# modelstreaming/ams

Measured on AMD Instinct MI355X. Metric: frames/sec student infer (DeeplabV3+MobileNetV2, 512x1024) + distill-steps/sec, higher is better.
Workload: dtype f32 (2xfp16 split products)

## Files before the change

### ams_amd/csrc/api.hip

```cpp
#include "engine.hpp"

using namespace ams;

extern "C" {

const char* ams_last_error(void) { return ams::last_error(); }
int ams_abi_version(void) { return AMS_ABI_VERSION; }

int ams_device_info(char* name_out, size_t name_cap, int32_t* n_cu, int64_t* hbm_bytes) {
    int dev = 0;
    AMS_CHECK_HIP(hipGetDevice(&dev));
    hipDeviceProp_t p;
    AMS_CHECK_HIP(hipGetDeviceProperties(&p, dev));
    if (name_out && name_cap) { snprintf(name_out, name_cap, "%s (%s)", p.name, p.gcnArchName); }
    if (n_cu) *n_cu = p.multiProcessorCount;
    if (hbm_bytes) *hbm_bytes = (int64_t)p.totalGlobalMem;
    return AMS_OK;
}

int ams_student_arena_bytes(const ams_student_config* cfg, const ams_layer_desc* layers, size_t* bytes_out) {
    AMS_REQUIRE(bytes_out, "arena_bytes: null output");
    ams_student tmp;
    int rc = student_build(&tmp, cfg, layers);
    if (rc) return rc;
// ... 263 lines not shown
                                   int32_t Ws, uint8_t* labels_out_dev, int64_t out_stride, void* stream) {
    return launch_teacher_labels_from_logits(logits_dev, slot_stride, n, lh, lw, num_classes, Hs, Ws, labels_out_dev, out_stride, (hipStream_t)stream);
}

size_t ams_render_table_bytes(void) { return AMS_RENDER_TABLE_BYTES; }

int ams_render_views(const uint8_t* frames_dev, const void* student_dev, int32_t student_dtype, const uint8_t* teacher_dev, int32_t batch, int32_t H,
                     int32_t W, int32_t K, const uint8_t* tables_dev, const ams_render_out* out, void* stream) {
    return launch_render_views(frames_dev, student_dev, student_dtype, teacher_dev, batch, H, W, K, tables_dev, out, (hipStream_t)stream);
}

int ams_student_train_step_dp(ams_student* s, const void* frames_dev, int32_t frames_dtype, const uint8_t* teacher_dev,
                              int32_t batch, int32_t global_batch, float lr, const uint8_t* mask_dev, double* loss_dev,
                              ams_allreduce_cb cb, void* user, void* stream) {
    return train_step_impl(s, frames_dev, frames_dtype, teacher_dev, batch, global_batch, lr, mask_dev, loss_dev, cb, user, nullptr, stream);
}

int ams_student_train_step_rccl(ams_student* s, const void* frames_dev, int32_t frames_dtype, const uint8_t* teacher_dev,
                                int32_t batch, int32_t global_batch, float lr, const uint8_t* mask_dev, double* loss_dev,
                                ams_comm* comm, void* stream) {
    AMS_REQUIRE(comm, "train_step_rccl: null communicator");
    return train_step_impl(s, frames_dev, frames_dtype, teacher_dev, batch, global_batch, lr, mask_dev, loss_dev, nullptr, nullptr, comm, stream);
}

int ams_student_train_step(ams_student* s, const void* frames_dev, int32_t frames_dtype, const uint8_t* teacher_dev, int32_t batch,
                           float lr, const uint8_t* mask_dev, double* loss_dev, void* stream) {
    return train_step_impl(s, frames_dev, frames_dtype, teacher_dev, batch, batch, lr, mask_dev, loss_dev, nullptr, nullptr, nullptr, stream);
}

int ams_student_f16_fallback_layers(const ams_student* s, int32_t* n_layers) {
    AMS_REQUIRE(s && n_layers, "f16_fallback_layers: null pointer");
    *n_layers = s->f16_fallback_layers;
    return AMS_OK;
}

int ams_student_feed_teacher_logits_layout(ams_student* s, const float* teacher_logits_dev, int32_t th, int32_t tw, int32_t layout) {
    AMS_REQUIRE(s, "feed_teacher_logits: null student");
    AMS_REQUIRE(layout == AMS_TLOGITS_FULL || layout == AMS_TLOGITS_SELECTED, "feed_teacher_logits: unknown teacher-logit layout %d", layout);
    if (!teacher_logits_dev) { s->teacher_logits = nullptr; s->teacher_th = s->teacher_tw = 0; s->teacher_layout = AMS_TLOGITS_FULL; return AMS_OK; }
    AMS_REQUIRE(th >= 1 && tw >= 1 && th <= s->cfg.height && tw <= s->cfg.width, "feed_teacher_logits: %d x %d teacher logits for %d x %d labels", th, tw,
                s->cfg.height, s->cfg.width);
    s->teacher_logits = teacher_logits_dev; s->teacher_th = th; s->teacher_tw = tw; s->teacher_layout = layout;
    return AMS_OK;
}

int ams_student_feed_teacher_logits(ams_student* s, const float* teacher_logits_dev, int32_t th, int32_t tw) {
    return ams_student_feed_teacher_logits_layout(s, teacher_logits_dev, th, tw, AMS_TLOGITS_FULL);
}

int ams_student_set_regularizer(ams_student* s, const uint8_t* reg_mask_dev, int32_t n_vars, float coef) {
    AMS_REQUIRE(s, "set_regularizer: null student");
    if (!reg_mask_dev) { s->reg_mask = nullptr; s->reg_nvars = 0; s->reg_coef = 0.f; return AMS_OK; }
    AMS_REQUIRE(s->cfg.trainable, "set_regularizer: this student was created frozen");
    AMS_REQUIRE(n_vars > 0 && coef >= 0.f, "set_regularizer: n_vars=%d coef=%g", n_vars, (double)coef);
    s->reg_mask = reg_mask_dev; s->reg_nvars = n_vars; s->reg_coef = coef;
    return AMS_OK;
}

int ams_student_set_option(ams_student* s, int32_t option, int32_t value) {
    AMS_REQUIRE(s, "set_option: null student");
    s->dual_choice.clear();
    if (option == AMS_OPT_MATMUL) {
        AMS_REQUIRE(value == AMS_MATMUL_F32 || value == AMS_MATMUL_SPLIT_BF16 || value == AMS_MATMUL_SPLIT_BF16_X6 || value == AMS_MATMUL_BF16 ||
                        value == AMS_MATMUL_SPLIT_F16,
                    "set_option: unknown matmul mode %d", value);
        s->matmul_mode = value;
        return AMS_OK;
    }
    if (option == AMS_OPT_DUAL_AUTOTUNE) {
        s->dual_autotune = value != 0;
        return AMS_OK;
    }
    if (option == AMS_OPT_DUAL_PARTS) {
        AMS_REQUIRE(value >= 2 && value <= 4, "set_option: AMS_OPT_DUAL_PARTS must be 2 .. 4");
        s->dual_parts = value;
        return AMS_OK;
    }
    if (option == AMS_OPT_FUSE_FIRST_BLOCK) {
        s->fuse_first_block = value < 0 ? 0 : (value > 2 ? 2 : value);
        return AMS_OK;
    }
    if (option == AMS_OPT_FUSE_DW_PROJECT) {
        s->fuse_dw_project = value != 0;
        return AMS_OK;
    }
    if (option == AMS_OPT_FUSE_EXPAND_DW_STREAM) {
        s->fuse_expand_dw_stream = value < 0 ? 0 : (value > 2 ? 2 : value);
        return AMS_OK;
    }
    if (option == AMS_OPT_BLOCK_X6) {
        s->block_x6 = value != 0;
        return AMS_OK;
    }
    if (option == AMS_OPT_LATE_SUBBATCH) {
        s->late_subbatch = value < 0 ? 0 : value;
        return AMS_OK;
    }
    if (option == AMS_OPT_DUAL_STREAM) {
        s->dual_stream = value < 0 ? 0 : value;
        s->dual_choice.clear();
        return AMS_OK;
    }
    if (option == AMS_OPT_FUSE_BLOCK) {
        s->fuse_block = value != 0;
        return AMS_OK;
    }
    if (option == AMS_OPT_FUSE_EXPAND_DW) {
        s->fuse_expand_dw = value < 0 ? 0 : (value > 2 ? 2 : value);
        return AMS_OK;
    }
    if (option == AMS_OPT_EMULATE_BF16_STORAGE) {
        s->emulate_bf16_storage = value != 0;
        return AMS_OK;
    }
    if (option == AMS_OPT_FUSE_DGRAD_BN) {
        s->fuse_dgrad_bn = value < 0 ? 0 : (value > 3 ? 3 : value);
        return AMS_OK;
    }
    if (option == AMS_OPT_FUSE_GEMM_RED) {
        s->fuse_gemm_red = value & 3;
        return AMS_OK;
    }
    if (option == AMS_OPT_TRAIN_RECOMPUTE) {
        s->train_recompute = value < 0 ? 0 : (value > 2 ? 2 : value);
        return AMS_OK;
    }
    if (option == AMS_OPT_FUSE_OPERAND_BN) {
        s->fuse_operand_bn = value & 1;
        return AMS_OK;
    }
    if (option == AMS_OPT_WGRAD_FORK_EVERY) {
        AMS_REQUIRE(value >= 1 && value <= 64, "set_option: AMS_OPT_WGRAD_FORK_EVERY must be in 1 .. 64");
        s->wgrad_fork_every = value;
        return AMS_OK;
    }
    if (option == AMS_OPT_TRAIN_FWD_F16) {
        s->train_fwd_f16 = value != 0;
        return AMS_OK;
    }
    if (option == AMS_OPT_SOFT_TEACHER) {
        s->soft_teacher = value != 0;
        return AMS_OK;
    }
    if (option == AMS_OPT_NAN_GRADS) {
        s->nan_grads = value != 0;
        return AMS_OK;
    }
    if (option == AMS_OPT_OVERLAP_WGRAD) {
        s->overlap_wgrad = value < 0 ? 0 : (value > 3 ? 3 : value);
        return AMS_OK;
    }
    if (option == AMS_OPT_OVERLAP_HEAD) {
        s->overlap_head = value != 0;
        return AMS_OK;
    }
    if (option == AMS_OPT_STREAM_MIN_ROWS) {
        AMS_REQUIRE(value >= 0, "set_option: AMS_OPT_STREAM_MIN_ROWS must be >= 0");
        s->stream_min_rows = value;
        return AMS_OK;
    }
    set_error("set_option: unknown option %d", option);
    return AMS_E_INVALID;
}

int ams_student_profile(ams_student* s, int32_t enable) {
    AMS_REQUIRE(s, "profile: null student");
    AMS_CHECK_HIP(hipDeviceSynchronize());
    s->prof.clear();
    s->prof.on = enable != 0;
    return AMS_OK;
}

int ams_student_profile_read(ams_student* s, char* buf, size_t cap, size_t* needed) {
    AMS_REQUIRE(s && needed, "profile_read: null pointer");
    AMS_CHECK_HIP(hipDeviceSynchronize());
    std::string out;
    char line[256];
    for (auto& r : s->prof.recs) {
        float ms = 0.f;
        AMS_CHECK_HIP(hipEventElapsedTime(&ms, r.e0, r.e1));
        snprintf(line, sizeof(line), "%s\t%d\t%.6f\t%.0f\t%.0f\t%.0f\n", r.name.c_str(), r.layer, ms, r.bytes, r.flops, r.flops_x6);
        out += line;
    }
    *needed = out.size() + 1;
    if (buf && cap >= out.size() + 1) memcpy(buf, out.c_str(), out.size() + 1);
    return AMS_OK;
}

int ams_student_get_adam_step(const ams_student* s, int64_t* t) {
    AMS_REQUIRE(s && t, "get_adam_step: null pointer");
    *t = s->adam_t;
    return AMS_OK;
}
int ams_student_set_adam_step(ams_student* s, int64_t t) {
    AMS_REQUIRE(s && t >= 0, "set_adam_step: bad argument");
    s->adam_t = t;
    return AMS_OK;
}

size_t ams_pack_masked_fp16_scratch(int64_t n) { return n > 0 ? pack_fp16_scratch(n) : 0; }

int ams_pack_masked_fp16(const float* params_dev, const uint8_t* mask_dev, int64_t n, uint16_t* out_half_dev, int64_t* n_out_dev,
                         int64_t* scratch_dev, size_t scratch_elems, void* stream) {
    AMS_REQUIRE(params_dev && out_half_dev && n_out_dev && n > 0, "pack_masked_fp16: bad argument");
    AMS_REQUIRE(scratch_dev && scratch_elems >= pack_fp16_scratch(n), "pack_masked_fp16: scratch too small (need %zu int64)",
                pack_fp16_scratch(n));
    return launch_pack_fp16(params_dev, mask_dev, n, out_half_dev, n_out_dev, scratch_dev, (hipStream_t)stream);
}

static int64_t delta_mask_bytes(const ams_student* s, const ams_delta_var* vars, int32_t n_vars, const char* what = "apply_delta") {
    if (!vars || n_vars < 1 || n_vars > AMS_DELTA_MAX_VARS) { set_error("%s: %d variables (1 .. %d)", what, n_vars, AMS_DELTA_MAX_VARS); return -1; }
    int64_t mask = 0;
    for (int32_t i = 0; i < n_vars; ++i) {
        const ams_delta_var& d = vars[i];
        const int64_t n_region = d.region == AMS_REGION_PARAMS ? (int64_t)s->cfg.n_trainable : d.region == AMS_REGION_STATS ? (int64_t)s->cfg.n_stats : -1;
        if (n_region < 0) { set_error("%s: variable %d: region %d is neither params nor stats", what, i, d.region); return -1; }
        if (d.offset < 0 || d.count < 0 || d.offset > n_region - d.count) {
            set_error("%s: variable %d: elements [%lld, +%lld) outside its region of %lld", what, i, (long long)d.offset, (long long)d.count,
                      (long long)n_region);
            return -1;
        }
        if (d.mask_offset != mask) {
            set_error("%s: variable %d: mask at byte %lld, the masks before it end at %lld", what, i, (long long)d.mask_offset, (long long)mask);
            return -1;
        }
        mask += (d.count + 7) / 8;
    }
    return mask;
}

size_t ams_student_apply_delta_scratch(const ams_delta_var* vars_host, int32_t n_vars) {
    if (!vars_host || n_vars < 1 || n_vars > AMS_DELTA_MAX_VARS) return 0;
    int64_t mask = 0;
    for (int32_t i = 0; i < n_vars; ++i) mask += vars_host[i].count > 0 ? (vars_host[i].count + 7) / 8 : 0;
    return (size_t)(4 * (int64_t)n_vars + delta_segments(mask));
}

int ams_student_apply_delta(ams_student* s, const uint8_t* payload_dev, int64_t payload_bytes, const ams_delta_var* vars_host,
                            int32_t n_vars, int64_t* n_applied_dev, int32_t* status_dev, int64_t* scratch_dev, size_t scratch_elems,
                            void* stream) {
    AMS_REQUIRE(s && n_applied_dev && status_dev && scratch_dev, "apply_delta: null pointer");
    AMS_REQUIRE(payload_bytes >= 0 && (payload_dev || payload_bytes == 0), "apply_delta: %lld payload bytes at %p", (long long)payload_bytes,
                (const void*)payload_dev);
    static_assert(sizeof(ams_delta_var) == 4 * sizeof(int64_t), "ams_delta_var: four int64 words");
    const int64_t mask_bytes = delta_mask_bytes(s, vars_host, n_vars);
    if (mask_bytes < 0) return AMS_E_INVALID;
    const size_t need = 4 * (size_t)n_vars + (size_t)delta_segments(mask_bytes);
    AMS_REQUIRE(scratch_elems >= need, "apply_delta: scratch too small (need %zu int64)", need);
    hipStream_t st = (hipStream_t)stream;
    if (s->ev_delta) AMS_CHECK_HIP(hipEventSynchronize(s->ev_delta));
    else RUN(create_sync_event(&s->ev_delta));
    s->delta_vars.assign(vars_host, vars_host + n_vars);
    ams_delta_var* vars_dev = reinterpret_cast<ams_delta_var*>(scratch_dev);
    AMS_CHECK_HIP(hipMemcpyAsync(vars_dev, s->delta_vars.data(), n_vars * sizeof(ams_delta_var), hipMemcpyHostToDevice, st));
    AMS_CHECK_HIP(hipEventRecord(s->ev_delta, st));
    return launch_apply_delta(payload_dev, payload_bytes, vars_dev, n_vars, mask_bytes, s->params, (int64_t)s->cfg.n_trainable, s->stats,
                              (int64_t)s->cfg.n_stats, scratch_dev + 4 * n_vars, n_applied_dev, status_dev, st);
}

size_t ams_select_changed_scratch(int64_t n) { return n > 0 ? select_scratch() : 0; }

int ams_select_changed(const float* after_dev, const float* before_dev, int64_t n, int64_t k, ams_select_result* result_dev,
                       int64_t* scratch_dev, size_t scratch_elems, void* stream) {
    AMS_REQUIRE(after_dev && before_dev && result_dev && scratch_dev, "select_changed: null pointer");
    AMS_REQUIRE(n > 0 && n < ((int64_t)1 << 31) && k >= 0 && k < n, "select_changed: rank %lld of %lld elements (0 <= k < n < 2^31)", (long long)k,
                (long long)n);
    AMS_REQUIRE(((uintptr_t)result_dev & 7) == 0 && ((uintptr_t)after_dev & 3) == 0 && ((uintptr_t)before_dev & 3) == 0, "select_changed: misaligned pointer");
    AMS_REQUIRE(scratch_elems >= select_scratch(), "select_changed: scratch too small (need %zu int64)", select_scratch());
    return launch_select_changed(after_dev, before_dev, n, k, result_dev, scratch_dev, (hipStream_t)stream);
}

int ams_select_apply(float* params_dev, const float* before_dev, int64_t n, float cut, uint8_t* mask_dev, int64_t* n_kept_dev, void* stream) {
    AMS_REQUIRE(params_dev && before_dev && mask_dev && n_kept_dev && n > 0, "select_apply: bad argument");
    AMS_REQUIRE(((uintptr_t)n_kept_dev & 7) == 0 && ((uintptr_t)params_dev & 3) == 0 && ((uintptr_t)before_dev & 3) == 0, "select_apply: misaligned pointer");
    return launch_select_apply(params_dev, before_dev, n, cut, mask_dev, n_kept_dev, (hipStream_t)stream);
}

size_t ams_student_encode_delta_scratch(const ams_delta_var* vars_host, int32_t n_vars) {
    if (!vars_host || n_vars < 1 || n_vars > AMS_DELTA_MAX_VARS) return 0;
    int64_t mask = 0;
    for (int32_t i = 0; i < n_vars; ++i) mask += vars_host[i].count > 0 ? (vars_host[i].count + 7) / 8 : 0;
    return (size_t)(5 * (int64_t)n_vars + 2 + encode_segments(mask));
}

int ams_student_encode_delta(ams_student* s, const uint8_t* mask_dev, const ams_delta_var* vars_host, int32_t n_vars, uint8_t* payload_dev,
                             int64_t payload_cap, int64_t* payload_bytes_dev, int64_t* scratch_dev, size_t scratch_elems, void* stream) {
    AMS_REQUIRE(s && payload_dev && payload_bytes_dev && scratch_dev, "encode_delta: null pointer");
    const int64_t mask_bytes = delta_mask_bytes(s, vars_host, n_vars, "encode_delta");
    if (mask_bytes < 0) return AMS_E_INVALID;
    AMS_REQUIRE(payload_cap >= mask_bytes, "encode_delta: room for %lld bytes, the mask section alone has %lld", (long long)payload_cap,
                (long long)mask_bytes);
    const size_t table = 5 * (size_t)n_vars + 1;
    const size_t need = table + 1 + (size_t)encode_segments(mask_bytes);
    AMS_REQUIRE(scratch_elems >= need, "encode_delta: scratch too small (need %zu int64)", need);
    hipStream_t st = (hipStream_t)stream;
    if (s->ev_encode) AMS_CHECK_HIP(hipEventSynchronize(s->ev_encode));
    else RUN(create_sync_event(&s->ev_encode));
    s->encode_table.resize(table);
    memcpy(s->encode_table.data(), vars_host, n_vars * sizeof(ams_delta_var));
    int64_t first = 0;
    for (int32_t i = 0; i < n_vars; ++i) { s->encode_table[4 * (size_t)n_vars + i] = first; first += vars_host[i].count; }
    s->encode_table[table - 1] = first;
    AMS_CHECK_HIP(hipMemcpyAsync(scratch_dev, s->encode_table.data(), table * sizeof(int64_t), hipMemcpyHostToDevice, st));
    AMS_CHECK_HIP(hipEventRecord(s->ev_encode, st));
    return launch_encode_delta(mask_dev, scratch_dev, n_vars, mask_bytes, s->params, s->stats, scratch_dev + table, payload_dev, payload_cap,
                               payload_bytes_dev, st);
// ... 484 lines not shown
```

### ams_amd/csrc/engine.hpp

```cpp
#pragma once
#include <math.h>
#include <stdarg.h>

#include <string>
#include <map>
#include <vector>

#include "kernels.hpp"

namespace ams {

const char* last_error();

struct ProfRec { std::string name; int layer; double bytes, flops, flops_x6; hipEvent_t e0, e1; };
struct Profiler {
    bool on = false;
    std::vector<ProfRec> recs;
    std::vector<hipEvent_t> pool;
    hipEvent_t get() {
        if (!pool.empty()) { hipEvent_t e = pool.back(); pool.pop_back(); return e; }
        hipEvent_t e = nullptr;
        (void)hipEventCreate(&e);
        return e;
    }
    void clear() {
        for (auto& r : recs) { pool.push_back(r.e0); pool.push_back(r.e1); }
        recs.clear();
    }
    ~Profiler() {
        clear();
        for (auto e : pool) if (e) (void)hipEventDestroy(e);
    }
};

struct LayerRt {
    ams_layer_desc d;
    int Hin = 0, Win = 0, Hout = 0, Wout = 0;
    int64_t px_in = 0, px_out = 0;
    float *fscale = nullptr, *fshift = nullptr;
    float *scale = nullptr, *shift = nullptr, *mean = nullptr, *rstd = nullptr, *cA = nullptr, *cB = nullptr, *cC = nullptr;
    double *fsums = nullptr, *bsums = nullptr;
    float *z = nullptr, *a = nullptr, *da = nullptr;
    float* dzp = nullptr;
    float* dw_rows = nullptr; size_t dw_rows_floats = 0;
    uint16_t *whi = nullptr, *wlo = nullptr, *wlo3 = nullptr;
    uint16_t* whf_mem = nullptr;
    uint16_t* whf = nullptr;
    int Kp = 0, split_k0 = 0;
    float* blk_vecs = nullptr;
    double* xx64 = nullptr;
    float* xx_g0 = nullptr;
};

struct Carver {
    char* base;
    size_t off = 0;
    explicit Carver(void* b) : base((char*)b) {}
    template <typename T>
    T* take(size_t n) {
        off = (off + 255) & ~(size_t)255;
        T* p = base ? (T*)(base + off) : nullptr;
        off += n * sizeof(T);
        return p;
    }
};

}

struct ams_student {
    ams_student_config cfg;
    std::vector<ams::LayerRt> L;
    char* arena = nullptr;
    size_t arena_bytes = 0;
    int h = 0, w = 0;
    int n_backbone = 0;
    int iPool = 0, iAspp = 0, iProj = 0, iLogits = 0;
    float *params = nullptr, *stats = nullptr, *grads = nullptr, *adam_m = nullptr, *adam_v = nullptr;
    float *fparams = nullptr, *fstats = nullptr;
    double* bn_sync = nullptr; size_t bn_sync_doubles = 0;
    float* logits = nullptr;
    uint16_t* xsplit = nullptr; size_t xsplit_plane = 0;
    uint16_t* panel_scratch = nullptr; size_t panel_elems = 0;
    std::vector<ams::SplitJob> tp_jobs;
    std::map<std::pair<const float*, int>, int> tp_index;
    ams::SplitJob* tp_jobs_dev = nullptr;
    uint16_t* tp_panels = nullptr; size_t tp_elems = 0;
    int64_t tp_blocks = 0;
    bool tp_fresh = false;
    bool tp_wait = false;
    hipEvent_t ev_tp = nullptr;
    std::vector<ams_delta_var> delta_vars;
    hipEvent_t ev_delta = nullptr;
    std::vector<int64_t> encode_table;
    hipEvent_t ev_encode = nullptr;
    float* dlogits = nullptr;
    float* ce_scratch = nullptr;
    int emulate_bf16_storage = 0;
    int fuse_gemm_red = 3;
    int fuse_operand_bn = 1;
    int fuse_dgrad_bn = 3;
    int train_recompute = 2;
    double* xx_scratch = nullptr; size_t xx_scratch_doubles = 0;
    float* xt_scratch = nullptr; size_t xt_floats = 0;
    float *vec_ones = nullptr, *vec_zeros = nullptr;
    float* vec_inv_hw = nullptr;
    float* act[4] = {nullptr, nullptr, nullptr, nullptr};
    size_t act_elems = 0;
    float *pooled = nullptr, *pool_a = nullptr, *img_bias = nullptr;
    float *d_img_bias = nullptr, *d_pool_a = nullptr, *d_pool_z = nullptr, *d_pooled = nullptr;
    float* im2col = nullptr;
    float* scratch2 = nullptr;
    float* scratch3 = nullptr;
    hipStream_t side2 = nullptr;
    hipEvent_t ev_xt = nullptr;
    hipStream_t side = nullptr;
    hipEvent_t ev_fork = nullptr, ev_head = nullptr;
    int dual_stream = 1;
    int dual_parts = 2;
    int dual_autotune = 0;
    hipStream_t part_stream[3] = {nullptr, nullptr, nullptr};
    hipEvent_t part_done[3] = {nullptr, nullptr, nullptr};
    hipEvent_t ev_fork_dual = nullptr;
    std::map<int, int> dual_choice;
    int overlap_head = 0;
    int overlap_wgrad = 1;
    int wgrad_fork_every = 1;
    int train_fwd_f16 = 0;
    int f16_fallback_layers = 0;
    int soft_teacher = 0;
    const float* teacher_logits = nullptr; int teacher_th = 0, teacher_tw = 0, teacher_layout = AMS_TLOGITS_FULL;
    const uint8_t* reg_mask = nullptr; int reg_nvars = 0; float reg_coef = 0.f;
    int nan_grads = 0;
    ~ams_student() {
        if (ev_fork) (void)hipEventDestroy(ev_fork);
        if (ev_head) (void)hipEventDestroy(ev_head);
        for (auto& e : part_done) if (e) (void)hipEventDestroy(e);
        for (auto& t : part_stream) if (t) (void)hipStreamDestroy(t);
        if (ev_fork_dual) (void)hipEventDestroy(ev_fork_dual);
        if (side) (void)hipStreamDestroy(side);
        if (side2) (void)hipStreamDestroy(side2);
        if (ev_xt) (void)hipEventDestroy(ev_xt);
        if (ev_tp) (void)hipEventDestroy(ev_tp);
        if (ev_delta) (void)hipEventDestroy(ev_delta);
        if (ev_encode) (void)hipEventDestroy(ev_encode);
    }
    float* scratch = nullptr; size_t scratch_floats = 0;
    float* tmp_c = nullptr;
    double* loss_buf = nullptr;
    int64_t* conf_buf = nullptr;
    int64_t adam_t = 0;
    bool frozen_ready = false;
    int matmul_mode = AMS_MATMUL_SPLIT_F16;
    int fuse_dw_project = 0;
    int fuse_first_block = 1;
    int64_t stream_min_rows = 4096;
    int fuse_expand_dw_stream = 1;
    int block_x6 = 1;
    int late_subbatch = 0;
    int fuse_block = 1;
    int fuse_expand_dw = 1;
    ams::Profiler prof;
    hipEvent_t prof_e0 = nullptr;
    double prof_flops = 0.0;
    double prof_flops_x6 = 0.0;
};

namespace ams {

int student_build(ams_student* s, const ams_student_config* cfg, const ams_layer_desc* layers);
int student_layout(ams_student* s, void* arena, size_t* bytes_out);
void prof_begin(ams_student* s, hipStream_t st);
void prof_end(ams_student* s, hipStream_t st, int layer, double bytes);

static inline PwArgs pw_args(const float* x, int64_t M, int K, int ldx, const float* w, int N, float* y, int ldy) {
    PwArgs a;
    memset(&a, 0, sizeof(a));
    a.x = x; a.M = M; a.K = K; a.Kw = K; a.ldx = ldx; a.w = w; a.w_sk = N; a.w_sn = 1; a.N = N;
    a.rows_per_img = 1; a.act = AMS_ACT_NONE; a.y = y; a.ldy = ldy;
    return a;
}

#define RUN(expr) do { int _rc = (expr); if (_rc) return _rc; } while (0)

#define RUNK(LAYER, BYTES, expr)                                   \
    do {                                                           \
        prof_begin(s, st);                                         \
        int _rc = (expr);                                          \
        prof_end(s, st, (LAYER), (double)(BYTES));                 \
        if (_rc) return _rc;                                       \
    } while (0)

static inline double pw_bytes(const PwArgs& a) {
    return 4.0 * ((double)a.M * (a.K + a.N + (a.res ? a.N : 0)) + (double)a.Kw * a.N) + (a.ysplit ? 2.0 * a.ysplit_np * (double)a.M * a.N : 0.0);
}
static inline double dw_bytes(const LayerRt& l, int B) { return 4.0 * ((double)B * (l.px_in + l.px_out) * l.d.cin + 9.0 * l.d.cin); }

struct SyncCtx { ams_allreduce_cb cb; void* user; ams_student* s; ams_comm* comm; };

static inline int comm_as_cb(void*, size_t, size_t, int32_t) { return 0; }

static inline int sync_any(const SyncCtx* sc, void* p, size_t n, int dtype, hipStream_t st) {
    if (!sc || !sc->cb) return AMS_OK;
    if (sc->comm) return comm_allreduce(sc->comm, p, n, dtype, st);
    const int rc = sc->cb(sc->user, (size_t)((char*)p - sc->s->arena), n, dtype);
    if (rc) { set_error("all-reduce callback failed (%d)", rc); return AMS_E_STATE; }
    return AMS_OK;
}
static inline int sync_doubles(const SyncCtx* sc, double* p, size_t n, hipStream_t st) { return sync_any(sc, p, n, AMS_DT_F64, st); }

bool split_pays(const PwArgs& a);
int live_pointwise(ams_student* s, const PwArgs& a, hipStream_t st);
bool train_recompute_block(const ams_student* s, int i);
bool dw_fused_train(const ams_student* s, int i, int B);
bool stem_fused_train(const ams_student* s);
bool dw_fused_train_fwd(const ams_student* s, int i, int B);
bool operand_bn_act(const ams_student* s, int i);
size_t red_rows_bound(int64_t M);
int check_call(const ams_student* s, const void* frames, int dtype, int batch);
int run_forward(ams_student* s, const void* frames, int dtype, int batch, int mode, hipStream_t st);
int forward_live(ams_student* s, const void* frames, int dtype, int B, int global_B, bool update_ema, const SyncCtx* sc, hipStream_t st);

int loss_forward(ams_student* s, const uint8_t* teacher, int B, int32_t* labels, hipStream_t st);
int backward(ams_student* s, const void* frames, int dtype, const uint8_t* teacher, int B, int global_B, const SyncCtx* sc, hipStream_t st);
int train_step_impl(ams_student* s, const void* frames_dev, int32_t frames_dtype, const uint8_t* teacher_dev, int32_t batch, int32_t global_batch,
                    float lr, const uint8_t* mask_dev, double* loss_dev, ams_allreduce_cb cb, void* user, ams_comm* comm, void* stream);

}
```

### ams_amd/csrc/engine_forward.hip

```cpp
#include "engine.hpp"

namespace ams {

bool split_pays(const PwArgs& a) {
    if (a.K < 32 || a.K % 8 != 0 || a.M < 256) return false;
    return a.M < 32768 || !pointwise_stream_applies(a) || (int64_t)a.K * a.N >= 40 * (int64_t)(a.K + a.N);
}

int live_pointwise(ams_student* s, const PwArgs& a, hipStream_t st) {
    const bool split = s->matmul_mode != AMS_MATMUL_F32 && s->panel_scratch && split_pays(a) && a.Kw == a.K && a.ldx % 4 == 0;
    if (!split) return launch_pointwise(a, st);
    const int Kp = (a.K + 31) / 32 * 32;
    const size_t plane = (size_t)a.N * Kp;
    if (s->tp_fresh) {
        auto it = s->tp_index.find({a.w, a.w_sk == 1 ? 1 : 0});
        if (it != s->tp_index.end()) {
            const SplitJob& j = s->tp_jobs[it->second];
            if (j.K == a.K && j.N == a.N && j.sk == a.w_sk && j.sn == a.w_sn) {
                if (s->tp_wait) { AMS_CHECK_HIP(hipStreamWaitEvent(st, s->ev_tp, 0)); s->tp_wait = false; }
                if (s->matmul_mode == AMS_MATMUL_SPLIT_F16 && s->train_fwd_f16 && j.f16 && pointwise_f16_applies(a))
                    return launch_pointwise_split_f16(a, j.p0 + 3 * j.plane, j.plane, j.Kp, st);
                return launch_pointwise_split3(a, j.p0, j.p0 + j.plane, j.p0 + 2 * j.plane, j.Kp, st);
            }
        }
    }
    AMS_REQUIRE(3 * plane <= s->panel_elems, "live_pointwise: panel scratch too small");
    uint16_t* p0 = s->panel_scratch;
    int rc = launch_split_weights3(a.w, a.w_sk, a.w_sn, a.K, a.N, Kp, p0, p0 + plane, p0 + 2 * plane, st);
    if (rc) return rc;
    return launch_pointwise_split3(a, p0, p0 + plane, p0 + 2 * plane, Kp, st);
}

struct FrozenView {
    float* act[4];
    uint16_t* xsplit; size_t xsplit_plane;
    float *pooled, *pool_a, *img_bias, *logits, *scratch;
    const void* frames; int B;
    int reserved;
};
static FrozenView view_whole(const ams_student* s, const void* frames, int B) {
    return {{s->act[0], s->act[1], s->act[2], s->act[3]}, s->xsplit, s->xsplit_plane, s->pooled, s->pool_a, s->img_bias, s->logits, s->scratch, frames, B, -1};
}
static FrozenView view_late(const ams_student* s, FrozenView v, int b0, int bp, int input_i) {
    v.pooled += (size_t)b0 * s->L[s->iPool].d.cin;
    v.pool_a += (size_t)b0 * s->L[s->iPool].d.cout;
    v.img_bias += (size_t)b0 * s->L[s->iProj].d.cout;
    v.logits += (size_t)b0 * s->h * s->w * 32;
    v.B = bp; v.reserved = input_i;
    return v;
}
static FrozenView view_slice(const ams_student* s, const void* frames, int dtype, int b0, int bp) {
    const ams_student_config& c = s->cfg;
    FrozenView v = view_late(s, view_whole(s, (const char*)frames + (size_t)b0 * c.height * c.width * 3 * (dtype == AMS_DT_U8 ? 1 : 4), bp), b0, bp, -1);
    for (int k = 0; k < 4; ++k) v.act[k] += (size_t)b0 * (s->act_elems / c.max_batch);
    if (v.xsplit) { v.xsplit += 3 * (s->xsplit_plane / c.max_batch) * b0; v.xsplit_plane = (s->xsplit_plane / c.max_batch) * bp; }
    v.scratch += image_colsum_scratch(b0, s->L[s->iPool].d.cin);
    return v;
}

struct PartsFmt { int np = 0, fmt = 0; };
struct Cursor { int i; const float* cur; int cur_i; PartsFmt parts; };

static int other(const FrozenView& v, int avoid0, int avoid1) {
    for (int k = 0; k < 4; ++k) if (k != avoid0 && k != avoid1 && k != v.reserved) return k;
    return -1;
}

enum PwForm { PW_F32, PW_BF16_1, PW_BF16_2, PW_BF16_3, PW_F16 };
enum BlockForm { BLOCK_WHOLE,
                 BLOCK_TILED,
                 BLOCK_STREAM, BLOCK_WREG,
                 BLOCK_LAYERS };
struct BlockPlan {
    BlockForm form = BLOCK_LAYERS;
    bool expand = false;
    bool h16 = false, x6 = false;
    int np = 0; const uint16_t* wparts = nullptr; int64_t wplane = 0;
    PartsFmt in;
    PwForm expand_form = PW_F32;
    bool dw_project = false;
    bool d_h2i = false;
    PwForm project_form = PW_F32;
    PartsFmt out;
};

static PwArgs layer_args(const ams_student* s, int layer, int B, const float* x, float* y, const float* res) {
    const LayerRt& l = s->L[layer];
    PwArgs a = pw_args(x, (int64_t)B * l.px_in, l.d.cin, l.d.cin, s->fparams + l.d.w_off, l.d.cout, y, l.d.cout);
    a.scale = l.fscale; a.shift = l.fshift; a.act = l.d.act;
    if (l.d.role == AMS_ROLE_PROJECT && l.d.residual_from) { a.res = res; a.ldr = l.d.cout; }
    return a;
}

static PwForm pointwise_form(const ams_student* s, int layer, const PwArgs& a, bool streamable) {
    const LayerRt& l = s->L[layer];
    if (s->matmul_mode == AMS_MATMUL_F32 || !l.whi || !(split_pays(a) || (streamable && a.K % 8 == 0 && a.K >= 32))) return PW_F32;
    switch (s->matmul_mode) {
        case AMS_MATMUL_SPLIT_F16: return l.whf && pointwise_f16_applies(a) ? PW_F16 : PW_BF16_3;
        case AMS_MATMUL_SPLIT_BF16_X6: return PW_BF16_3;
        case AMS_MATMUL_BF16: return PW_BF16_1;
        default: return PW_BF16_2;
    }
}

static bool stream_ok(const ams_student* s, int B, int k) {
    if (!(s->fuse_expand_dw_stream && k + 1 <= s->n_backbone && s->L[k].d.role == AMS_ROLE_EXPAND && s->L[k + 1].d.role == AMS_ROLE_DEPTHWISE &&
          (int64_t)B * s->L[k].px_in >= s->stream_min_rows && (int64_t)s->L[k + 1].px_out * s->L[k + 1].d.cout * 4 < 0x7fffffffLL &&
          expand_dw_stream_supported(s->L[k].d.cin, s->L[k].d.cout, s->L[k + 1].d.stride, s->L[k + 1].d.rate)))
        return false;
    if (s->L[k + 1].d.stride != 1 && s->fuse_expand_dw_stream < 2) return false;
    if (s->L[k].d.cin <= 32) return true;
    return s->matmul_mode != AMS_MATMUL_F32 && s->L[k].whi && s->L[k].Kp == s->L[k].d.cin;
}
static int stream_np(const ams_student* s, int k) {
    if (s->matmul_mode == AMS_MATMUL_SPLIT_F16 && s->L[k].whf && s->L[k].d.cin > 32) return AMS_NP_F16;
    return s->matmul_mode == AMS_MATMUL_SPLIT_BF16_X6 || s->matmul_mode == AMS_MATMUL_SPLIT_F16 ? 3 : s->matmul_mode == AMS_MATMUL_BF16 ? 1 : 2;
}
static PartsFmt stream_parts(const ams_student* s, int k) {
    PartsFmt f;
    const int np = stream_np(s, k);
    if (np == AMS_NP_F16) { f.np = 2; f.fmt = 1; }
    else if (s->matmul_mode != AMS_MATMUL_SPLIT_F16) f.np = np;
    return f;
}

static BlockPlan plan_block(const ams_student* s, const FrozenView& v, int i, PartsFmt in) {
    BlockPlan p;
    const int B = v.B, nb = s->n_backbone;
    const auto role = [&](int k) { return k <= nb ? s->L[k].d.role : -1; };
    p.expand = role(i) == AMS_ROLE_EXPAND;
    const int id = i + (p.expand ? 1 : 0), ij = id + 1;
    const LayerRt& le = s->L[i];
    const LayerRt& ld = s->L[id];
    const LayerRt& lj = s->L[ij];
    if (s->fuse_block && p.expand && role(id) == AMS_ROLE_DEPTHWISE && role(ij) == AMS_ROLE_PROJECT &&
        (!lj.d.residual_from || lj.d.residual_from == i - 1) &&
        block_fused_supported(le.d.cin, le.d.cout, lj.d.cout, ld.d.stride, ld.d.rate, lj.d.residual_from != 0)) {
        p.form = BLOCK_WHOLE;
        p.h16 = s->block_x6 && s->matmul_mode == AMS_MATMUL_SPLIT_F16 && le.whf && lj.whf && le.Kp == 32;
        p.x6 = !p.h16 && s->block_x6 && s->matmul_mode != AMS_MATMUL_F32 && le.whi && le.Kp == 32 && le.d.cin > 16;
        return p;
    }
    if (stream_ok(s, B, i) && (le.d.cin <= 96 || in.np || s->fuse_expand_dw_stream >= 2)) {
        p.form = le.d.cin > 96 && in.np ? BLOCK_WREG : BLOCK_STREAM;
        p.in = in;
        p.np = stream_np(s, i);
        p.h16 = p.np == AMS_NP_F16;
        p.wparts = p.h16 ? le.whf : le.whi;
        p.wplane = p.h16 ? (int64_t)le.d.cout * le.Kp : (int64_t)(le.wlo - le.whi);
    } else if (s->fuse_expand_dw && p.expand && role(id) == AMS_ROLE_DEPTHWISE &&
               expand_dw_supported(le.d.cin, le.d.cout, ld.d.stride, ld.d.rate) &&
               (s->fuse_expand_dw >= 2 || le.d.cin <= 24 || ld.d.stride == 2)) {
        p.form = BLOCK_TILED;
    } else {
        if (p.expand) {
            const bool streamable = role(id) == AMS_ROLE_DEPTHWISE && le.Kp == le.d.cin && le.d.cin >= 64 &&
                                    expand_dw_stream_supported(le.d.cin, le.d.cout, ld.d.stride, ld.d.rate);
            p.expand_form = pointwise_form(s, i, layer_args(s, i, B, nullptr, nullptr, nullptr), streamable);
        }
        if (s->fuse_dw_project && s->matmul_mode == AMS_MATMUL_SPLIT_BF16 &&    role(id) == AMS_ROLE_DEPTHWISE &&
            role(ij) == AMS_ROLE_PROJECT && lj.whi && (int64_t)B * ld.px_out < 32768 && (int64_t)B * ld.px_out >= 256 &&
            lj.Kp == ld.d.cin && dw_project_supported(ld.d.cin, lj.d.cout, ld.d.stride, ld.d.rate)) {
            p.dw_project = true;
            return p;
        }
    }
    if (role(ij) != AMS_ROLE_PROJECT) return p;
    const PwArgs a = layer_args(s, ij, B, nullptr, nullptr, s->fparams);
    p.project_form = pointwise_form(s, ij, a, false);
    p.d_h2i = (p.form == BLOCK_STREAM || p.form == BLOCK_WREG) && p.h16 && p.project_form == PW_F16 && ld.d.cout % 8 == 0 && !s->emulate_bf16_storage;
    if (stream_ok(s, B, ij + 1) && v.xsplit && (size_t)a.M * a.N <= v.xsplit_plane && p.project_form != PW_F32 && pointwise_split_writes_parts(a) &&
        !(s->emulate_bf16_storage && lj.px_out == (int64_t)s->h * s->w))
        p.out = stream_parts(s, ij + 1);
    return p;
}

static int frozen_pointwise(ams_student* s, int layer, const PwArgs& a, PwForm form, hipStream_t st) {
    const LayerRt& l = s->L[layer];
    if (a.x_fmt != 0 && form != PW_F16) { set_error("frozen_pointwise: layer %d was handed fp16 pairs but does not run the fp16 product", layer); return AMS_E_STATE; }
    switch (form) {
        case PW_F16: RUNK(layer, pw_bytes(a), launch_pointwise_split_f16(a, l.whf, (int64_t)l.d.cout * l.Kp, l.Kp, st)); break;
        case PW_BF16_3: RUNK(layer, pw_bytes(a), launch_pointwise_split3(a, l.whi, l.wlo, l.wlo3, l.Kp, st)); break;
        case PW_BF16_2: RUNK(layer, pw_bytes(a), launch_pointwise_split(a, l.whi, l.wlo, l.Kp, st)); break;
        case PW_BF16_1: RUNK(layer, pw_bytes(a), launch_pointwise_split1(a, l.whi, l.Kp, st)); break;
        case PW_F32: RUNK(layer, pw_bytes(a), launch_pointwise(a, st)); break;
    }
    return AMS_OK;
}

static int run_first_block(ams_student* s, const FrozenView& v, int dtype, Cursor& c, hipStream_t st) {
    const ams_student_config& cf = s->cfg;
    const float* P = s->fparams;
    const int B = v.B;
    float* y = v.act[0];
    const LayerRt& l = s->L[1];
    const LayerRt& ld = s->L[2];
    const LayerRt& lj = s->L[3];
    const double in_bytes = (double)B * cf.height * cf.width * 3 * (dtype == AMS_DT_U8 ? 1 : 4);
    c.i = 2;
    if (s->fuse_first_block && s->n_backbone >= 3 && l.d.cout == 32 && ld.d.role == AMS_ROLE_DEPTHWISE && ld.d.cin == 32 &&
        ld.d.stride == 1 && ld.d.rate == 1 && lj.d.role == AMS_ROLE_PROJECT && lj.d.cin == 32 && lj.d.cout == 16 &&
        !lj.d.residual_from) {
        const double bytes = in_bytes + 4.0 * B * lj.px_out * lj.d.cout + 4.0 * (27 * 32 + 9 * 32 + 32 * 16);
        if (s->fuse_first_block >= 2)
            RUNK(3, bytes, launch_first_block_tiles(v.frames, dtype, B, cf.height, cf.width, cf.pixel_scale, P + l.d.w_off, l.fscale, l.fshift,
                                                    l.d.act, P + ld.d.w_off, ld.fscale, ld.fshift, ld.d.act, P + lj.d.w_off, lj.fscale,
                                                    lj.fshift, lj.d.act, y, st, l.blk_vecs));
        else {
            const bool h16 = s->block_x6 && s->matmul_mode == AMS_MATMUL_SPLIT_F16 && l.whf && lj.whf && lj.Kp == 32;
            const bool x6 = !h16 && s->block_x6 && s->matmul_mode != AMS_MATMUL_F32 && l.whi;
            RUNK(3, bytes, launch_first_block(v.frames, dtype, B, cf.height, cf.width, cf.pixel_scale, P + l.d.w_off, l.fscale, l.fshift,
                                              l.d.act, P + ld.d.w_off, ld.fscale, ld.fshift, ld.d.act, P + lj.d.w_off, lj.fscale,
                                              lj.fshift, lj.d.act, y, st, x6 ? l.whi : nullptr, 32 * 32, h16 ? l.whf : nullptr, 32 * 32,
                                              h16 ? lj.whf : nullptr, (int64_t)lj.d.cout * lj.Kp));
        }
        c.i = 4;
    } else {
        const double bytes = in_bytes + 4.0 * B * l.px_out * l.d.cout;
        RUNK(1, bytes, launch_stem(v.frames, dtype, B, cf.height, cf.width, P + l.d.w_off, l.d.cout, l.fscale, l.fshift, l.d.act,
                                   cf.pixel_scale, y, st));
    }
    c.cur = y; c.cur_i = 0; c.parts = PartsFmt();
    return AMS_OK;
}

static int run_project(ams_student* s, const FrozenView& v, Cursor& c, const BlockPlan& p, int ij, const float* d, int d_i, hipStream_t st) {
    const LayerRt& l = s->L[ij];
    AMS_REQUIRE(l.d.role == AMS_ROLE_PROJECT, "engine: expected project at layer %d", ij);
    const int o = other(v, c.cur_i, d_i);
    PwArgs a = layer_args(s, ij, v.B, d, v.act[o], c.cur);
    a.x_fmt = p.d_h2i ? 1 : 0;
    if (p.out.np) { a.ysplit = v.xsplit; a.ysplit_plane = a.M * a.N; a.ysplit_np = p.out.np; a.ysplit_fmt = p.out.fmt; }
    RUN(frozen_pointwise(s, ij, a, p.project_form, st));
    if (s->emulate_bf16_storage && l.px_out == (int64_t)s->h * s->w)
        RUN(launch_round_bf16(v.act[o], (int64_t)v.B * l.px_out * l.d.cout, st));
    c.cur = v.act[o]; c.cur_i = o; c.i = ij + 1; c.parts = p.out;
    return AMS_OK;
}

static int run_block_whole(ams_student* s, const FrozenView& v, Cursor& c, const BlockPlan& p, hipStream_t st) {
    const float* P = s->fparams;
    const int B = v.B, i = c.i;
    const LayerRt& le = s->L[i];
    const LayerRt& ld = s->L[i + 1];
    const LayerRt& lj = s->L[i + 2];
    const int o = other(v, c.cur_i, -1);
    const bool res = lj.d.residual_from != 0;
    const double bytes = 4.0 * ((double)B * (le.px_in * le.d.cin * (res ? 2 : 1) + lj.px_out * lj.d.cout) + (double)le.d.cin * le.d.cout +
                                9.0 * ld.d.cin + (double)lj.d.cin * lj.d.cout);
    const double fl_e = 2.0 * B * (double)le.px_in * le.d.cin * le.d.cout, fl_p = 2.0 * B * (double)lj.px_out * lj.d.cin * lj.d.cout;
    s->prof_flops = 2.0 * B * (double)ld.px_out * 9.0 * ld.d.cin + (p.h16 ? 0.0 : fl_p) + (p.x6 || p.h16 ? 0.0 : fl_e);
    s->prof_flops_x6 = p.h16 ? fl_e + fl_p : p.x6 ? fl_e : 0.0;
    RUNK(i + 2, bytes, launch_block_fused(c.cur, B, le.Hin, le.Win, le.d.cin, P + le.d.w_off, le.fscale, le.fshift, le.d.act, le.d.cout,
                                          P + ld.d.w_off, ld.d.stride, ld.fscale, ld.fshift, ld.d.act, P + lj.d.w_off, lj.fscale, lj.fshift,
                                          lj.d.act, lj.d.cout, res, v.act[o], st, le.blk_vecs, p.x6 ? le.whi : nullptr,
                                          (int64_t)(le.wlo - le.whi), p.h16 ? le.whf : nullptr, (int64_t)le.d.cout * le.Kp, p.h16 ? lj.whf : nullptr,
                                          (int64_t)lj.d.cout * lj.Kp, lj.Kp));
    c.cur = v.act[o]; c.cur_i = o; c.i = i + 3; c.parts = PartsFmt();
    return AMS_OK;
}

static int run_block_expand_dw(ams_student* s, const FrozenView& v, Cursor& c, const BlockPlan& p, hipStream_t st) {
    const float* P = s->fparams;
    const int B = v.B, i = c.i;
    const LayerRt& le = s->L[i];
    const LayerRt& ld = s->L[i + 1];
    const int o = other(v, c.cur_i, -1);
    const double bytes = 4.0 * ((double)B * (le.px_in * le.d.cin + ld.px_out * ld.d.cout) + (double)le.d.cin * le.d.cout + 9.0 * ld.d.cin);
    const uint16_t* x_parts = p.in.np ? v.xsplit : nullptr;
    const int64_t xplane = (int64_t)B * le.px_in * le.d.cin;
    if (p.form == BLOCK_TILED)
        RUNK(i + 1, bytes, launch_expand_dw(c.cur, B, le.Hin, le.Win, le.d.cin, P + le.d.w_off, le.fscale, le.fshift, le.d.act, le.d.cout,
                                            P + ld.d.w_off, ld.d.stride, ld.d.rate, ld.fscale, ld.fshift, ld.d.act, v.act[o], st));
    else if (p.form == BLOCK_WREG)
        RUNK(i + 1, bytes, launch_expand_dw_wreg(x_parts, xplane, B, le.Hin, le.Win, le.d.cin, p.wparts, p.wplane, p.np, le.fscale,
                                                 le.fshift, le.d.act, le.d.cout, P + ld.d.w_off, ld.d.rate, ld.fscale, ld.fshift, ld.d.act,
                                                 v.act[o], st, p.d_h2i ? 1 : 0));
    else
        RUNK(i + 1, bytes, launch_expand_dw_stream(c.cur, x_parts, xplane, B, le.Hin, le.Win, le.d.cin, P + le.d.w_off, p.wparts, p.wplane, p.np, le.fscale,
                                                   le.fshift, le.d.act, le.d.cout, P + ld.d.w_off, ld.d.stride, ld.d.rate, ld.fscale, ld.fshift, ld.d.act,
                                                   v.act[o], st, p.d_h2i ? 1 : 0));
    if (p.form != BLOCK_TILED && s->emulate_bf16_storage && ld.px_out == (int64_t)s->h * s->w)
        RUN(launch_round_bf16(v.act[o], (int64_t)B * ld.px_out * ld.d.cout, st));
    return run_project(s, v, c, p, i + 2, v.act[o], o, st);
}

static int run_block_layers(ams_student* s, const FrozenView& v, Cursor& c, const BlockPlan& p, hipStream_t st) {
    const float* P = s->fparams;
    const int B = v.B;
    int i = c.i;
    const float* x = c.cur;
    int x_i = c.cur_i;
    if (p.expand) {
        const int o = other(v, c.cur_i, -1);
        RUN(frozen_pointwise(s, i, layer_args(s, i, B, x, v.act[o], nullptr), p.expand_form, st));
        x = v.act[o]; x_i = o; ++i;
    }
    const LayerRt& l = s->L[i];
    AMS_REQUIRE(l.d.role == AMS_ROLE_DEPTHWISE, "engine: expected depthwise at layer %d", i);
    const int o = other(v, c.cur_i, x_i);
    if (p.dw_project) {
        const LayerRt& lpj = s->L[i + 1];
        const PwArgs a = layer_args(s, i + 1, B, nullptr, v.act[o], c.cur);
        const double bytes = 4.0 * ((double)B * (l.px_in * l.d.cin + lpj.px_out * lpj.d.cout * (a.res ? 2 : 1)) +
                                    (double)lpj.d.cin * lpj.d.cout + 9.0 * l.d.cin);
        RUNK(i + 1, bytes, launch_dw_project(x, B, l.Hin, l.Win, l.d.cin, P + l.d.w_off, l.d.rate, l.fscale, l.fshift, l.d.act, a,
                                             lpj.whi, lpj.wlo, lpj.Kp, st));
        c.cur = v.act[o]; c.cur_i = o; c.i = i + 2; c.parts = PartsFmt();
        return AMS_OK;
    }
    RUNK(i, dw_bytes(l, B), launch_depthwise(x, B, l.Hin, l.Win, l.d.cin, P + l.d.w_off, l.d.stride, l.d.rate, l.fscale,
                                             l.fshift, l.d.act, v.act[o], st));
    if (s->emulate_bf16_storage && l.px_out == (int64_t)s->h * s->w)
        RUN(launch_round_bf16(v.act[o], (int64_t)B * l.px_out * l.d.cout, st));
    return run_project(s, v, c, p, i + 1, v.act[o], o, st);
}

static int run_blocks(ams_student* s, const FrozenView& v, Cursor& c, int i_stop, hipStream_t st) {
    while (c.i <= s->n_backbone && c.i < i_stop) {
        const BlockPlan p = plan_block(s, v, c.i, c.parts);
        switch (p.form) {
            case BLOCK_WHOLE: RUN(run_block_whole(s, v, c, p, st)); break;
            case BLOCK_TILED: case BLOCK_STREAM: case BLOCK_WREG: RUN(run_block_expand_dw(s, v, c, p, st)); break;
            case BLOCK_LAYERS: RUN(run_block_layers(s, v, c, p, st)); break;
        }
    }
    return AMS_OK;
}

static int run_head(ams_student* s, const FrozenView& v, const Cursor& c, hipStream_t st) {
    const float* P = s->fparams;
    const LayerRt& lp = s->L[s->iPool]; const LayerRt& la = s->L[s->iAspp]; const LayerRt& lc = s->L[s->iProj]; const LayerRt& ll = s->L[s->iLogits];
    const int B = v.B;
    const int64_t HW = (int64_t)s->h * s->w, M = (int64_t)B * HW;
    const bool fork = s->overlap_head && !s->prof.on;
    hipStream_t ps = st;
    if (fork) {
        if (!s->side) RUN(create_side_stream(&s->side));
        if (!s->ev_fork) RUN(create_sync_event(&s->ev_fork));
        if (!s->ev_head) RUN(create_sync_event(&s->ev_head));
        AMS_CHECK_HIP(hipEventRecord(s->ev_fork, st));
        AMS_CHECK_HIP(hipStreamWaitEvent(s->side, s->ev_fork, 0));
        ps = s->side;
    }
    RUNK(s->iPool, 4.0 * M * lp.d.cin, launch_global_mean(c.cur, B, HW, lp.d.cin, v.pooled, v.scratch, ps));
    {
        PwArgs a = pw_args(v.pooled, B, lp.d.cin, lp.d.cin, P + lp.d.w_off, lp.d.cout, v.pool_a, lp.d.cout);
        a.scale = lp.fscale; a.shift = lp.fshift; a.act = lp.d.act;
        RUNK(s->iPool, pw_bytes(a), launch_pointwise(a, ps));
        PwArgs b = pw_args(v.pool_a, B, lp.d.cout, lp.d.cout, P + lc.d.w_off, lc.d.cout, v.img_bias, lc.d.cout);
        RUNK(s->iProj, pw_bytes(b), launch_pointwise(b, ps));
    }
    if (fork) AMS_CHECK_HIP(hipEventRecord(s->ev_head, s->side));
    const int o1 = other(v, c.cur_i, -1), o2 = other(v, c.cur_i, o1);
    PwArgs a = pw_args(c.cur, M, la.d.cin, la.d.cin, P + la.d.w_off, la.d.cout, v.act[o1], la.d.cout);
    a.scale = la.fscale; a.shift = la.fshift; a.act = la.d.act;
    RUN(frozen_pointwise(s, s->iAspp, a, pointwise_form(s, s->iAspp, a, false), st));
    if (fork) AMS_CHECK_HIP(hipStreamWaitEvent(st, s->ev_head, 0));
    PwArgs b = pw_args(v.act[o1], M, la.d.cout, la.d.cout, P + lc.d.w_off + (int64_t)lp.d.cout * lc.d.cout, lc.d.cout,
                       v.act[o2], lc.d.cout);
    b.img_bias = v.img_bias; b.rows_per_img = HW; b.scale = lc.fscale; b.shift = lc.fshift; b.act = lc.d.act;
    RUN(frozen_pointwise(s, s->iProj, b, pointwise_form(s, s->iProj, b, false), st));
    PwArgs d = pw_args(v.act[o2], M, lc.d.cout, lc.d.cout, P + ll.d.w_off, ll.d.cout, v.logits, 32);
    d.shift = P + ll.d.gamma_off;
    RUN(frozen_pointwise(s, s->iLogits, d, pointwise_form(s, s->iLogits, d, false), st));
    return AMS_OK;
}

static int forward_frozen(ams_student* s, const FrozenView& v, int dtype, hipStream_t st) {
    Cursor c;
    RUN(run_first_block(s, v, dtype, c, st));
    int i_late = s->n_backbone + 1;
    for (int k = 2; k <= s->n_backbone; ++k)
        if (s->L[k].d.role == AMS_ROLE_EXPAND && s->L[k].px_in == (int64_t)s->h * s->w) { i_late = k; break; }
    if (!(s->late_subbatch > 0 && v.B > s->late_subbatch && i_late <= s->n_backbone)) {
        RUN(run_blocks(s, v, c, s->n_backbone + 1, st));
        return run_head(s, v, c, st);
    }
    RUN(run_blocks(s, v, c, i_late, st));
    const int64_t late_in_frame = s->L[i_late].px_in * s->L[i_late].d.cin;
    for (int b0 = 0; b0 < v.B; b0 += s->late_subbatch) {
        const int bp = v.B - b0 < s->late_subbatch ? v.B - b0 : s->late_subbatch;
        const FrozenView lv = view_late(s, v, b0, bp, c.cur_i);
        Cursor lc = {i_late, c.cur + (int64_t)b0 * late_in_frame, c.cur_i, PartsFmt()};
        RUN(run_blocks(s, lv, lc, s->n_backbone + 1, st));
        RUN(run_head(s, lv, lc, st));
    }
    return AMS_OK;
}

bool train_recompute_block(const ams_student* s, int i) {
    if (!s->train_recompute || !s->xt_scratch || i < 2 || i + 1 > s->n_backbone) return false;
    const LayerRt& l = s->L[i];
    const LayerRt& ld = s->L[i + 1];
    return l.xx_g0 && l.d.role == AMS_ROLE_EXPAND && ld.d.role == AMS_ROLE_DEPTHWISE && xdw_train_supported(l.d.cin, l.d.cout, ld.d.stride, ld.d.rate) &&
           expand_dw_supported(l.d.cin, l.d.cout, ld.d.stride, ld.d.rate) && l.d.cout <= 1024 &&
           xdw_train_scratch(s->cfg.max_batch, l.Hin, l.Win, l.d.cin, l.d.cout) != (size_t)-1 &&
           xdw_train_scratch(s->cfg.max_batch, l.Hin, l.Win, l.d.cin, l.d.cout) <= s->xt_floats;
}

bool dw_fused_train(const ams_student* s, int i, int B) {
    if (i < 3 || i > s->n_backbone || !s->fuse_dgrad_bn || train_recompute_block(s, i - 1)) return false;
    const LayerRt& l = s->L[i];
    const LayerRt& prev = s->L[i - 1];
    return l.d.role == AMS_ROLE_DEPTHWISE && l.d.stride == 1 && prev.d.role == AMS_ROLE_EXPAND && prev.d.cout == l.d.cin && l.d.cin <= 1024 &&
           depthwise_dgrad_bn_scratch(B, l.Hin, l.Win, l.d.cin) <= s->scratch_floats;
}
bool stem_fused_train(const ams_student* s) {
    const ams_student_config& c = s->cfg;
    return s->n_backbone >= 2 && s->train_recompute && s->L[1].d.role == AMS_ROLE_STEM && s->L[1].d.cout == 32 && s->L[2].d.role == AMS_ROLE_DEPTHWISE &&
           s->L[2].d.stride == 1 && s->L[2].d.rate == 1 && s->xt_scratch && xdw_stem_scratch(c.max_batch, c.height, c.width) != (size_t)-1 &&
           xdw_stem_scratch(c.max_batch, c.height, c.width) <= s->xt_floats;
}
bool dw_fused_train_fwd(const ams_student* s, int i, int B) {
    if (s->fuse_dgrad_bn < 2 || i < 2 || i > s->n_backbone) return false;
    if (!(i == 2 ? stem_fused_train(s) : dw_fused_train(s, i, B))) return false;
    return depthwise_fwd_bn_scratch(B, s->L[i].Hin, s->L[i].Win, s->L[i].d.cin, s->L[i].d.rate) <= s->scratch_floats;
}

bool operand_bn_act(const ams_student* s, int i) {
    if (!(s->fuse_operand_bn & 1) || i < 2 || i + 1 > s->n_backbone) return false;
    const LayerRt& l = s->L[i];
    const LayerRt& lj = s->L[i + 1];
    return l.d.role == AMS_ROLE_DEPTHWISE && lj.d.role == AMS_ROLE_PROJECT && lj.d.cin == l.d.cout && l.d.cout % 4 == 0 && l.d.cout <= 1024;
}

size_t red_rows_bound(int64_t M) {
    const size_t tiled = (size_t)(M / 64 + 8), streaming = M >= 32768 ? 8 * 512 : 0;
    return tiled > streaming ? tiled : streaming;
}

struct BnEma { const float* center; float omd; float *mm, *mv; };
static BnEma bn_ema(const ams_student* s, const LayerRt& l, bool update_ema) {
    return {s->stats + l.d.mean_off, 1.0f - s->cfg.bn_decay, update_ema ? s->stats + l.d.mean_off : nullptr, update_ema ? s->stats + l.d.var_off : nullptr};
}
static int bn_from_partials(ams_student* s, LayerRt& l, const BnEma& e, const float* part, int rows, int64_t stride, double n_global,
                            const SyncCtx* sc, hipStream_t st) {
    const float *gamma = s->params + l.d.gamma_off, *beta = s->params + l.d.beta_off;
    if (!sc || !sc->cb)
        return launch_bn_fwd_finalize_partials(part, rows, stride, l.d.cout, l.fsums, n_global, e.center, gamma, beta, l.d.bn_eps, e.omd, e.mm, e.mv,
                                               l.scale, l.shift, l.mean, l.rstd, st);
    RUN(launch_partials_to_sums(part, rows, stride, l.d.cout, l.fsums, st));
    RUN(sync_doubles(sc, l.fsums, 2 * (size_t)l.d.cout, st));
    return launch_bn_finalize(l.fsums, n_global, l.d.cout, e.center, gamma, beta, l.d.bn_eps, e.omd, e.mm, e.mv, l.scale, l.shift, l.mean, l.rstd, st);
}

static int bn_train(ams_student* s, LayerRt& l, int64_t M_local, double n_global, bool update_ema, const SyncCtx* sc,
                    const float* res, hipStream_t st, int pre_rows = 0, bool act_pass = true) {
    const BnEma e = bn_ema(s, l, update_ema);
    if (pre_rows > 0) {
        RUN(bn_from_partials(s, l, e, s->scratch, pre_rows, 2 * (int64_t)l.d.cout, n_global, sc, st));
    } else if (!sc || !sc->cb) {
        RUNK(0, 4.0 * M_local * l.d.cout,
             launch_colstats_bn(l.z, M_local, l.d.cout, e.center, l.fsums, s->scratch, n_global, s->params + l.d.gamma_off,
                                s->params + l.d.beta_off, l.d.bn_eps, e.omd, e.mm, e.mv, l.scale, l.shift, l.mean, l.rstd, st));
    } else {
        RUNK(0, 4.0 * M_local * l.d.cout, launch_colstats(l.z, M_local, l.d.cout, e.center, l.fsums, s->scratch, st));
        RUN(sync_doubles(sc, l.fsums, 2 * (size_t)l.d.cout, st));
        RUN(launch_bn_finalize(l.fsums, n_global, l.d.cout, e.center, s->params + l.d.gamma_off, s->params + l.d.beta_off, l.d.bn_eps, e.omd,
                               e.mm, e.mv, l.scale, l.shift, l.mean, l.rstd, st));
    }
    if (!act_pass) return AMS_OK;
    RUNK(0, 4.0 * M_local * l.d.cout * (res ? 3 : 2), launch_bn_act(l.z, M_local, l.d.cout, l.scale, l.shift, l.d.act, res, l.a, st));
    return AMS_OK;
}

int forward_live(ams_student* s, const void* frames, int dtype, int B, int global_B, bool update_ema, const SyncCtx* sc,
                        hipStream_t st) {
    const ams_student_config& c = s->cfg;
    AMS_REQUIRE(c.trainable, "live forward needs a trainable student (activations are not allocated)");
    const float* P = s->params;
    s->tp_fresh = false;
    s->tp_wait = false;
    if (s->matmul_mode != AMS_MATMUL_F32 && !s->tp_jobs.empty()) {
        hipStream_t ts = st;
        if (s->overlap_wgrad && !s->prof.on && s->scratch2) {
            if (!s->side) RUN(create_side_stream(&s->side));
            if (!s->ev_fork) RUN(create_sync_event(&s->ev_fork));
            if (!s->ev_tp) RUN(create_sync_event(&s->ev_tp));
            AMS_CHECK_HIP(hipEventRecord(s->ev_fork, st));
            AMS_CHECK_HIP(hipStreamWaitEvent(s->side, s->ev_fork, 0));
            ts = s->side;
        }
        RUNK(0, 0.0, launch_split_batch(s->tp_jobs_dev, (int)s->tp_jobs.size(), s->tp_blocks, ts,
                                        s->train_fwd_f16 && s->matmul_mode == AMS_MATMUL_SPLIT_F16));
        if (ts != st) { AMS_CHECK_HIP(hipEventRecord(s->ev_tp, ts)); s->tp_wait = true; }
        s->tp_fresh = true;
    }
    {
        LayerRt& l = s->L[1];
        RUN(launch_stem(frames, dtype, B, c.height, c.width, P + l.d.w_off, l.d.cout, nullptr, nullptr, AMS_ACT_NONE,
                        c.pixel_scale, l.z, st));
        RUN(bn_train(s, l, (int64_t)B * l.px_out, (double)global_B * l.px_out, update_ema, sc, nullptr, st, 0, !dw_fused_train_fwd(s, 2, B)));
    }
    for (int i = 2; i <= s->n_backbone; ++i) {
        LayerRt& l = s->L[i];
        const float* x = s->L[i - 1].a;
        if (train_recompute_block(s, i)) {
            LayerRt& ld = s->L[i + 1];
            const BnEma e = bn_ema(s, l, update_ema);
            const double n_e = (double)global_B * l.px_out;
            if (s->train_recompute >= 2 && l.xx64 && s->xx_scratch && l.d.cin <= 32 &&
                xx_stats_scratch_doubles((int64_t)B * l.px_in, l.d.cin) <= s->xx_scratch_doubles) {
                const int KP = (l.d.cin + 15) / 16 * 16;
                RUNK(i, 4.0 * B * l.px_in * l.d.cin, launch_xx_gram(x, (int64_t)B * l.px_in, l.d.cin, s->xx_scratch, l.xx64, l.xx_g0, st));
                RUN(sync_doubles(sc, l.xx64, (size_t)KP * KP + KP, st));
                RUN(launch_expand_stats(l.xx64, l.d.cin, P + l.d.w_off, l.d.cout, n_e, e.center, s->params + l.d.gamma_off, s->params + l.d.beta_off,
                                        l.d.bn_eps, e.omd, e.mm, e.mv, l.scale, l.shift, l.mean, l.rstd, l.fsums, st));
            } else {
            int rows = 0;
            int64_t fstride = 0;
            RUNK(i, 4.0 * B * l.px_in * l.d.cin,
                 launch_xdw_fwd_stats(x, B, l.Hin, l.Win, l.d.cin, P + l.d.w_off, l.d.cout, e.center, s->xt_scratch, &rows, &fstride, st));
            {
                const int KP = (l.d.cin + 15) / 16 * 16;
                RUN(launch_reduce_splits(s->xt_scratch + 2 * (int64_t)l.d.cout, rows, (int64_t)KP * KP + KP, l.xx_g0, st, fstride));
            }
            RUN(bn_from_partials(s, l, e, s->xt_scratch, rows, fstride, n_e, sc, st));
            }
            int d_rows = 0;
            const bool d_stats = (s->fuse_gemm_red & 1) && expand_dw_stats_scratch(B, l.Hin, l.Win, l.d.cout, ld.d.stride) <= s->scratch_floats;
            RUNK(i + 1, 4.0 * ((double)B * (l.px_in * l.d.cin + ld.px_out * ld.d.cout)),
                 launch_expand_dw(x, B, l.Hin, l.Win, l.d.cin, P + l.d.w_off, l.scale, l.shift, l.d.act, l.d.cout, P + ld.d.w_off, ld.d.stride,
                                  ld.d.rate, s->vec_ones, s->vec_zeros, AMS_ACT_NONE, ld.z, st, d_stats ? s->stats + ld.d.mean_off : nullptr,
                                  d_stats ? s->scratch : nullptr, d_stats ? &d_rows : nullptr));
            RUN(bn_train(s, ld, (int64_t)B * ld.px_out, (double)global_B * ld.px_out, update_ema, sc, nullptr, st, d_rows, !operand_bn_act(s, i + 1)));
            ++i;
            continue;
        }
        int pre_rows = 0;
        if (l.d.role == AMS_ROLE_DEPTHWISE && dw_fused_train_fwd(s, i, B)) {
            const LayerRt& le = s->L[i - 1];
            if (s->fuse_dgrad_bn >= 3 && l.d.cin % 64 == 0 && depthwise_fwd_bn2_scratch(B, l.Hin, l.Win, l.d.cin, l.d.rate) <= s->scratch_floats)
                RUNK(i, dw_bytes(l, B), launch_depthwise_fwd_bn2(le.z, B, l.Hin, l.Win, l.d.cin, P + l.d.w_off, l.d.rate, le.scale, le.shift, le.d.act,
                                                                 s->stats + l.d.mean_off, l.z, s->scratch, &pre_rows, st));
            else
// ... 149 lines not shown
```

### ams_amd/csrc/kernels.hpp

```cpp
#pragma once
#include <vector>

#include "common.hpp"

struct ams_comm;

namespace ams {

int func_allow_lds(const void* fn, size_t lds);
int func_blocks_per_cu(const void* fn, int threads, size_t lds, int* per_cu);
int device_cus(int* cus);
bool launch_table_needs_attr(int device, const void* fn, size_t lds);
struct Knobs {
    int blk_th = 0, blk_tw = 0;
    int fb_walk = -1;
    int fb_abl = 0;
    int xwr_timed = 0;
    int blk_timed = 0;
    int blk_hp = -1;
    char pw_force = 0; int pw_rm = 0, pw_nt = 0;
    int pw_percu = 0;
    bool pwx_no_tail = false;
    int pwx_rm = 0, pwx_nt = 0;
    int xwr_abl = 0;
    int pwh_abl = 0;
    bool pwh_set = false; int pwh_nw = 4, pwh_d = 2;
    bool xds_set = false; int xds[6] = {0, 0, 0, 0, 0, 0};
    bool xwr_set = false; int xwr[5] = {0, 0, 0, 0, 0};
    bool wg6_eight_waves = false;
    int wg6_split_cap = 0;
    int event_flags = -1;
    unsigned side_cu_mask = 0;
};
const Knobs& knobs();
int blk_phase_cycles(unsigned long long* h);
int xwr_phase_cycles(unsigned long long* h);
int xds_phase_cycles(unsigned long long* h);
int create_side_stream(hipStream_t* out);
int create_sync_event(hipEvent_t* out);

int comm_allreduce(ams_comm* c, void* p, size_t n, int dtype, hipStream_t st);

struct PwArgs {
    const float* x;
    int64_t M;
    int K;
    int Kw;
    int ldx;
    const float* w;
    int64_t w_sk, w_sn;
    int N;
    const float* img_bias;
    int64_t rows_per_img;
    const float* scale;
    const float* shift;
    int act;
    const float* res;
    int ldr;
    float* y;
    int ldy;
    uint16_t* ysplit;
    int64_t ysplit_plane;
    int ysplit_np;
    int ysplit_fmt;
    int x_fmt;
    int red_mode;
    const float* red_center;
    const float* red_z; const float* red_scale; const float* red_shift; const float* red_mean; const float* red_rstd;
    int red_act;
    float* red_part;
    size_t red_part_floats;
    int* red_rows_out;
    const float* red_res; int red_ldr;
    int x_mode; int x_act;
    const float* x_v0; const float* x_v1; const float* x_v2; const float* x2;
    float* x_tmp;
};
int launch_pointwise(const PwArgs& a, hipStream_t st);
int pointwise_materialize_x(const PwArgs& a, PwArgs* b, hipStream_t st);
bool pointwise_stream_applies(const PwArgs& a);
bool pointwise_transforms_on_load(const PwArgs& a);
bool pointwise_split3_transforms_on_load(const PwArgs& a);

int launch_split_weights(const float* w, int64_t sk, int64_t sn, int K, int N, int Kp, uint16_t* hi, uint16_t* lo, hipStream_t st);
int launch_pointwise_split(const PwArgs& a, const uint16_t* whi, const uint16_t* wlo, int Kp, hipStream_t st);
int launch_split_weights3(const float* w, int64_t sk, int64_t sn, int K, int N, int Kp, uint16_t* hi, uint16_t* mid, uint16_t* lo,
                          hipStream_t st);
int launch_pointwise_split3(const PwArgs& a, const uint16_t* whi, const uint16_t* wmid, const uint16_t* wlo, int Kp, hipStream_t st);
struct SplitJob { const float* w; int64_t sk, sn; int K, N, Kp; uint16_t* p0; int64_t plane; int64_t first_block; int f16; };
int launch_split_batch(const SplitJob* jobs_dev, int njobs, int64_t total_blocks, hipStream_t st, int write_f16);
int launch_pointwise_split1(const PwArgs& a, const uint16_t* whi, int Kp, hipStream_t st);
int launch_split_weights_f16(const float* w, int64_t sk, int64_t sn, int K, int N, int Kp, uint16_t* hi, uint16_t* lo, hipStream_t st);
bool pointwise_f16_applies(const PwArgs& a);
int launch_pointwise_split_f16(const PwArgs& a, const uint16_t* whi, int64_t plane, int Kp, hipStream_t st);
int launch_pack_h2i(const float* x, int64_t M, int C, float* out, hipStream_t st);
bool pointwise_split_writes_parts(const PwArgs& a);

struct WgArgs {
    const float* x;  int ldx;  int K;
    const float* dy; int ldy;  int N;
    int64_t M;
    float* dw;
    float* scratch; size_t scratch_floats;
    int allow_split;
    int x_mode = 0, x_act = 0; const float* x_v0 = nullptr; const float* x_v1 = nullptr;
    int dy_mode = 0; const float* dy_v0 = nullptr; const float* dy_v1 = nullptr; const float* dy_v2 = nullptr; const float* dy2 = nullptr;
};
bool dw_project_supported(int C, int N, int stride, int rate);
int launch_dw_project(const float* e, int B, int H, int W, int C, const float* w_dw, int rate, const float* sc_d, const float* sh_d,
                      int act_d, const PwArgs& p, const uint16_t* whi, const uint16_t* wlo, int Kp, hipStream_t st);
bool pointwise_wgrad_x6_applies(int64_t M, int K, int N, int ldx, int ldy);
int wgrad_x6_splits(int64_t M, int K, int N);
int launch_pointwise_wgrad_x6(const WgArgs& a, int splits, hipStream_t st);
size_t pointwise_wgrad_scratch(int64_t M, int K, int N);
int launch_pointwise_wgrad(const WgArgs& a, hipStream_t st);

int launch_first_block(const void* frames, int dtype, int B, int H, int W, float pixel_scale, const float* w_stem,
                       const float* sc_s, const float* sh_s, int act_s, const float* w_dw, const float* sc_d, const float* sh_d,
                       int act_d, const float* w_pj, const float* sc_p, const float* sh_p, int act_p, float* y, hipStream_t st,
                       const uint16_t* w_parts = nullptr, int64_t w_plane = 0, const uint16_t* h_stem = nullptr, int64_t h_stem_plane = 0,
                       const uint16_t* h_pj = nullptr, int64_t h_pj_plane = 0);

int launch_resize_u8(const uint8_t* src, int Hs, int Ws, int C, int mode, int swap_rb, uint8_t* dst, int H, int W, hipStream_t st);

int launch_stem(const void* frames, int dtype, int B, int H, int W, const float* w, int cout, const float* scale,
                const float* shift, int act, float pixel_scale, float* y, hipStream_t st);
int launch_stem_im2col(const void* frames, int dtype, int B, int H, int W, float pixel_scale, float* out, hipStream_t st);
int launch_depthwise(const float* x, int B, int H, int W, int C, const float* w, int stride, int rate,
                     const float* scale, const float* shift, int act, float* y, hipStream_t st);
int launch_depthwise_dgrad(const float* dy, int B, int H, int W, int C, const float* w, int stride, int rate,
                           float* dx, hipStream_t st);
size_t depthwise_fwd_bn_scratch(int B, int H, int W, int C, int rate);
int launch_depthwise_fwd_bn(const float* ze, int B, int H, int W, int C, const float* w, int rate, const float* scale, const float* shift, int act,
                            const float* center, float* zd, float* scratch, int* rows_out, hipStream_t st);
size_t depthwise_dgrad_bn_scratch(int B, int H, int W, int C);
int launch_depthwise_dgrad_bn(const float* dy, int B, int H, int W, int C, const float* w, int rate, const float* z, const float* scale,
                              const float* shift, int act, const float* mean, const float* rstd, float* out, float* scratch, int* rows_out,
                              hipStream_t st);
size_t depthwise_dgrad_bn2_scratch(int B, int H, int W, int C, int rate);
int launch_depthwise_dgrad_bn2(const float* dy, const float* zd, const float* cA, const float* cB, const float* cC, int B, int H, int W, int C,
                               const float* w, int rate, const float* ze, const float* scale, const float* shift, int act, const float* mean,
                               const float* rstd, float* out, float* scratch, int* rows_out, hipStream_t st);
size_t depthwise_fwd_bn2_scratch(int B, int H, int W, int C, int rate);
int launch_depthwise_fwd_bn2(const float* ze, int B, int H, int W, int C, const float* w, int rate, const float* scale, const float* shift, int act,
                             const float* center, float* zd, float* scratch, int* rows_out, hipStream_t st);
size_t depthwise_wgrad_scratch(int B, int H, int W, int C, int stride, int rate);
int launch_depthwise_wgrad(const float* x, const float* dy, int B, int H, int W, int C, int stride, int rate,
                           float* dw, float* scratch, size_t scratch_floats, hipStream_t st);

bool expand_dw_supported(int Cin, int Cexp, int stride, int rate);
size_t expand_dw_stats_scratch(int B, int H, int W, int Cexp, int stride);
int launch_expand_dw(const float* x, int B, int H, int W, int Cin, const float* w_exp, const float* sc_e, const float* sh_e, int act_e,
                     int Cexp, const float* w_dw, int stride, int rate, const float* sc_d, const float* sh_d, int act_d, float* y,
                     hipStream_t st, const float* stats_center = nullptr, float* stats_part = nullptr, int* stats_rows = nullptr);

bool xdw_train_supported(int Cin, int Cexp, int stride, int rate);
size_t xdw_train_scratch(int B, int H, int W, int Cin, int Cexp);
int xdw_train_blocks(int B, int H, int W, int Cexp);
int launch_xdw_fwd_stats(const float* x, int B, int H, int W, int Cin, const float* w_exp, int Cexp, const float* center, float* scratch,
                         int* rows_out, int64_t* stride_out, hipStream_t st);
int launch_xdw_bwd_reduce(const float* x, int B, int H, int W, int Cin, const float* w_exp, int Cexp, const float* sc_e, const float* sh_e,
                          const float* mean_e, const float* rstd_e, int act_e, const float* w_dw, int stride, const float* dz_d, float* scratch,
                          int* rows_out, int64_t* stride_out, hipStream_t st);
size_t xdw_stem_scratch(int B, int fH, int fW);
int launch_xdw_bwd_reduce_stem(const void* frames, int dtype, int B, int fH, int fW, float pixel_scale, const float* w_stem, const float* sc_e,
                               const float* sh_e, const float* mean_e, const float* rstd_e, int act_e, const float* w_dw, const float* dz_d,
                               float* scratch, int* rows_out, int64_t* stride_out, hipStream_t st);
int launch_xdw_bwd_dx(const float* x, int B, int H, int W, int Cin, const float* w_exp, int Cexp, const float* sc_e, const float* sh_e,
                      int act_e, const float* w_dw, int stride, const float* dz_d, const float* cA, const float* cB, const float* cC,
                      const float* res, float* dx, hipStream_t st, const float* red_z = nullptr, const float* red_mean = nullptr,
                      const float* red_rstd = nullptr, float* red_part = nullptr, int* red_rows_out = nullptr);
int launch_xdw_dwe(const float* G1, const float* xx_g0, int Cin, int Cexp, const float* w_exp, const float* cA, const float* cB, const float* cC,
                   float* dw, hipStream_t st);

int xx_stats_blocks(int64_t M);
size_t xx_stats_scratch_doubles(int64_t M, int Cin);
int launch_xx_gram(const float* x, int64_t M, int Cin, double* scratch, double* xx64, float* xx32, hipStream_t st);
int launch_expand_stats(const double* xx64, int Cin, const float* w_exp, int Cexp, double n, const float* center, const float* gamma,
                        const float* beta, float eps, float one_minus_decay, float* moving_mean, float* moving_var, float* scale, float* shift,
                        float* save_mean, float* save_rstd, double* sums, hipStream_t st);

bool block_fused_supported(int Cin, int Cexp, int Cout, int stride, int rate, bool residual);
int launch_block_fused(const float* x, int B, int H, int W, int Cin, const float* w_exp, const float* sc_e, const float* sh_e, int act_e, int Cexp,
                       const float* w_dw, int stride, const float* sc_d, const float* sh_d, int act_d, const float* w_pj, const float* sc_p,
                       const float* sh_p, int act_p, int Cout, bool residual, float* y, hipStream_t st, const float* vecs = nullptr,
                       const uint16_t* wparts = nullptr, int64_t wplane = 0, const uint16_t* h_exp = nullptr, int64_t h_exp_plane = 0,
                       const uint16_t* h_pj = nullptr, int64_t h_pj_plane = 0, int h_pj_kp = 0);
int launch_first_block_tiles(const void* frames, int dtype, int B, int H, int W, float pixel_scale, const float* w_stem, const float* sc_s,
                             const float* sh_s, int act_s, const float* w_dw, const float* sc_d, const float* sh_d, int act_d, const float* w_pj,
                             const float* sc_p, const float* sh_p, int act_p, float* y, hipStream_t st, const float* vecs = nullptr);
int launch_block_pack(const float* sc_e, const float* sh_e, const float* sc_d, const float* sh_d, const float* w_dw, int Cexp, float* out, hipStream_t st);

constexpr int AMS_NP_F16 = 4;
bool expand_dw_stream_supported(int Cin, int Cexp, int stride, int rate);
int launch_expand_dw_stream(const float* x, const uint16_t* x_parts, int64_t x_plane, int B, int H, int W, int Cin, const float* w_f32,
                            const uint16_t* w_parts, int64_t plane, int np,
                            const float* sc_e, const float* sh_e, int act_e, int Cexp, const float* w_dw, int stride, int rate, const float* sc_d,
                            const float* sh_d, int act_d, float* y, hipStream_t st, int y_fmt = 0);

int launch_expand_dw_wreg(const uint16_t* x_parts, int64_t x_plane, int B, int H, int W, int Cin, const uint16_t* w_parts, int64_t plane,
                          int np, const float* sc_e, const float* sh_e, int act_e, int Cexp, const float* w_dw, int rate, const float* sc_d,
                          const float* sh_d, int act_d, float* y, hipStream_t st, int y_fmt = 0);


size_t image_colsum_scratch(int B, int C);
int launch_global_mean(const float* x, int B, int64_t HW, int C, float* y, float* scratch, hipStream_t st);
int launch_image_colsum(const float* x, int B, int64_t HW, int C, int ldx, float* out, float* scratch, hipStream_t st);

size_t colstats_scratch(int64_t M, int C);
int launch_colstats(const float* z, int64_t M, int C, const float* center, double* sums , float* scratch,
                    hipStream_t st);
int launch_bn_finalize(const double* sums, double n, int C, const float* center, const float* gamma, const float* beta,
                       float eps, float one_minus_decay, float* moving_mean, float* moving_var, float* scale,
                       float* shift, float* save_mean, float* save_rstd, hipStream_t st);
int launch_bn_fold(const float* gamma, const float* beta, const float* mean, const float* var, float eps, int C,
                   float* scale, float* shift, hipStream_t st);
int launch_bn_act(const float* z, int64_t M, int C, const float* scale, const float* shift, int act, const float* res,
                  float* a, hipStream_t st);
int launch_bn_bwd_reduce(const float* da, const float* z, int64_t M, int C, const float* scale, const float* shift,
                         int act, const float* mean, const float* rstd, double* sums, float* scratch, hipStream_t st);
int launch_bn_bwd_coef(const double* sums, double n, int C, const float* gamma, const float* mean, const float* rstd,
                       float* coefA, float* coefB, float* coefC, float* dgamma, float* dbeta, hipStream_t st);
int launch_bn_param_grads(const double* sums, int C, float* dgamma, float* dbeta, hipStream_t st);
int launch_colstats_bn(const float* z, int64_t M, int C, const float* center, double* sums, float* scratch, double n,
                       const float* gamma, const float* beta, float eps, float one_minus_decay, float* moving_mean,
                       float* moving_var, float* scale, float* shift, float* save_mean, float* save_rstd, hipStream_t st);
int launch_bn_bwd_reduce_coef(const float* da, const float* z, int64_t M, int C, const float* scale, const float* shift, int act,
                              const float* mean, const float* rstd, double* sums, float* scratch, double n, const float* gamma,
                              float* coefA, float* coefB, float* coefC, float* dgamma, float* dbeta, hipStream_t st);
int launch_bn_bwd_apply(const float* da, const float* z, int64_t M, int C, const float* scale, const float* shift, int act,
                        const float* coefA, const float* coefB, const float* coefC, float* dz, hipStream_t st);
int launch_colsum(const float* x, int64_t M, int C, int ldx, float* out, float* scratch, hipStream_t st);
int launch_adam(float* p, const float* g, float* m, float* v, const uint8_t* mask, int64_t n, float lr_t, float b1,
                float b2, float eps, hipStream_t st);
struct ReduceJobs {
    static constexpr int kMax = 32;
    int n = 0;
    const float* part[kMax]; float* out[kMax]; int splits[kMax]; int64_t count[kMax]; int64_t stride[kMax]; int first_block[kMax];
    bool add(const float* p, int splits_, int64_t count_, float* o, int64_t stride_) {
        if (n >= kMax) return false;
        part[n] = p; splits[n] = splits_; count[n] = count_; out[n] = o; stride[n] = stride_ > 0 ? stride_ : count_; ++n;
        return true;
    }
};
int launch_reduce_batch(ReduceJobs& jobs, hipStream_t st);
int launch_reduce_splits(const float* part, int splits, int64_t n, float* out, hipStream_t st, int64_t stride = 0);
int launch_bn_fwd_finalize_partials(const float* part, int rows, int64_t row_stride, int C, double* sums, double n, const float* center,
                                    const float* gamma, const float* beta, float eps, float one_minus_decay, float* moving_mean,
                                    float* moving_var, float* scale, float* shift, float* save_mean, float* save_rstd, hipStream_t st);
// ... 72 lines not shown
```

### ams_amd/csrc/pw_common.hpp

```cpp
#pragma once
#include <stdlib.h>

#include <string>

#include "kernels.hpp"
#include "split_bf16.hpp"

namespace ams {

template <int NT>
__device__ __forceinline__ void pw_stage_affine(const PwArgs& a, float* sSc, float* sSh, int n0, int tid, int nthreads) {
    for (int e = tid; e < 16 * NT; e += nthreads) {
        const int n = n0 + e;
        sSc[e] = (a.scale && n < a.N) ? a.scale[n] : 1.f;
        sSh[e] = (a.shift && n < a.N) ? a.shift[n] : 0.f;
    }
}

template <int RM, int NT>
__device__ __forceinline__ void pw_epilogue(const PwArgs& a, f32x4 (&acc)[RM][NT], int64_t m_base, int n0, int l15, int q,
                                            const float* sSc, const float* sSh, int nrg = RM) {
    const bool y_vec = (a.ldy & 3) == 0, r_vec = (a.ldr & 3) == 0, n_vec = (a.N & 3) == 0;
#pragma unroll
    for (int r = 0; r < RM; ++r) {
        const int64_t m = m_base + r * 16 + l15;
        if (m >= a.M || r >= nrg) continue;
        float4 add[NT];
        bool has_add = false;
        if (a.res || a.img_bias) {
            has_add = true;
            const float* rp = a.res ? a.res + m * a.ldr : nullptr;
            const float* bp = a.img_bias ? a.img_bias + (m / a.rows_per_img) * a.N : nullptr;
#pragma unroll
            for (int t = 0; t < NT; ++t) {
                const int n4 = n0 + 16 * t + 4 * q;
                float4 rv = make_float4(0.f, 0.f, 0.f, 0.f), bv = rv;
                if (n4 + 3 < a.N) {
                    if (rp) rv = r_vec ? ld4(rp + n4) : make_float4(rp[n4], rp[n4 + 1], rp[n4 + 2], rp[n4 + 3]);
                    if (bp) bv = n_vec ? ld4(bp + n4) : make_float4(bp[n4], bp[n4 + 1], bp[n4 + 2], bp[n4 + 3]);
                } else if (n4 < a.N) {
                    float tr[4] = {0.f, 0.f, 0.f, 0.f}, tb[4] = {0.f, 0.f, 0.f, 0.f};
#pragma unroll
                    for (int i = 0; i < 4; ++i)
                        if (n4 + i < a.N) { if (rp) tr[i] = rp[n4 + i]; if (bp) tb[i] = bp[n4 + i]; }
                    rv = make_float4(tr[0], tr[1], tr[2], tr[3]);
                    bv = make_float4(tb[0], tb[1], tb[2], tb[3]);
                }
                add[t] = rv;
                acc[r][t][0] += bv.x; acc[r][t][1] += bv.y; acc[r][t][2] += bv.z; acc[r][t][3] += bv.w;
            }
        }
#pragma unroll
        for (int t = 0; t < NT; ++t) {
            const int c4 = 16 * t + 4 * q, n4 = n0 + c4;
            if (n4 >= a.N) continue;
            const float4 sc = ld4(sSc + c4), sh = ld4(sSh + c4);
            float4 v;
            const float4 bn = muladd4_pk(make_float4(acc[r][t][0], acc[r][t][1], acc[r][t][2], acc[r][t][3]), sc, sh);
            v.x = apply_act(bn.x, a.act); v.y = apply_act(bn.y, a.act);
            v.z = apply_act(bn.z, a.act); v.w = apply_act(bn.w, a.act);
            if (has_add && a.res) { v.x += add[t].x; v.y += add[t].y; v.z += add[t].z; v.w += add[t].w; }
            float* yp = a.y + m * a.ldy + n4;
            if (n4 + 3 < a.N && y_vec) st4(yp, v);
            else {
                const float o[4] = {v.x, v.y, v.z, v.w};
#pragma unroll
                for (int i = 0; i < 4; ++i) if (n4 + i < a.N) yp[i] = o[i];
            }
        }
    }
}

enum { EPI_PLAIN = 0, EPI_RES = 1, EPI_BIAS = 2, EPI_GENERIC = 3 };

template <int RM, int NT, int EPI, bool SPLIT_OUT = false>
__device__ __forceinline__ void pw_epilogue_t(const PwArgs& a, f32x4 (&acc)[RM][NT], int64_t m_base, int n0, int lane,
                                              const float* sSc, const float* sSh, float* sOut, int nrg = RM) {
    constexpr int OP = 16 * NT + 4;
    constexpr int V4 = 4 * NT;
    const int l15 = lane & 15, q = lane >> 4;
#pragma unroll
    for (int r = 0; r < RM; ++r) {
        if (r >= nrg) break;
        const int64_t m0 = m_base + r * 16;
        if (EPI == EPI_BIAS) {
            int64_t m = m0 + l15;
            if (m > a.M - 1) m = a.M - 1;
            const float* bp = a.img_bias + (m / a.rows_per_img) * a.N;
            float4 bv[NT];
#pragma unroll
            for (int t = 0; t < NT; ++t) {
                int n4 = n0 + 16 * t + 4 * q;
                if (n4 > a.N - 4) n4 = a.N - 4;
                bv[t] = ld4(bp + n4);
            }
#pragma unroll
            for (int t = 0; t < NT; ++t) { acc[r][t][0] += bv[t].x; acc[r][t][1] += bv[t].y; acc[r][t][2] += bv[t].z; acc[r][t][3] += bv[t].w; }
        }
        const bool ident = !a.scale && !a.shift && a.act == AMS_ACT_NONE;
#pragma unroll
        for (int t = 0; t < NT; ++t) {
            const int c4 = 16 * t + 4 * q;
            float4 v = make_float4(acc[r][t][0], acc[r][t][1], acc[r][t][2], acc[r][t][3]);
            if (!ident) {
                const float4 sc = ld4(sSc + c4), sh = ld4(sSh + c4);
                const float4 bn = muladd4_pk(v, sc, sh);
                v.x = apply_act(bn.x, a.act); v.y = apply_act(bn.y, a.act);
                v.z = apply_act(bn.z, a.act); v.w = apply_act(bn.w, a.act);
            }
            st4(sOut + l15 * OP + c4, v);
        }
        __builtin_amdgcn_fence(__ATOMIC_RELEASE, "wavefront");
        __builtin_amdgcn_wave_barrier();
        __builtin_amdgcn_fence(__ATOMIC_ACQUIRE, "wavefront");
        constexpr int UG = NT > 6 ? (NT + 1) / 2 : NT;
#pragma unroll
        for (int u0 = 0; u0 < NT; u0 += UG) {
        float4 rv[UG];
        if (EPI == EPI_RES) {
#pragma unroll
            for (int uu = 0; uu < UG; ++uu) {
                const int u = u0 + uu < NT ? u0 + uu : NT - 1;
                const int f = lane + 64 * u;
                const int row = f / V4;
                int col = n0 + (f - row * V4) * 4;
                int64_t m = m0 + row;
                if (m > a.M - 1) m = a.M - 1;
                if (col > a.N - 4) col = a.N - 4;
                rv[uu] = ld4(a.res + m * a.ldr + col);
            }
        }
#pragma unroll
        for (int uu = 0; uu < UG; ++uu) {
            const int u = u0 + uu;
            if (u >= NT) break;
            const int f = lane + 64 * u;
            const int row = f / V4, c4 = (f - row * V4) * 4;
            const int64_t m = m0 + row;
            float4 v = ld4(sOut + row * OP + c4);
            if (EPI == EPI_RES) { v.x += rv[uu].x; v.y += rv[uu].y; v.z += rv[uu].z; v.w += rv[uu].w; }
            if (m < a.M && n0 + c4 < a.N) {
                if (SPLIT_OUT && a.ysplit) __builtin_nontemporal_store((f32x4){v.x, v.y, v.z, v.w}, reinterpret_cast<f32x4*>(a.y + m * a.ldy + n0 + c4));
                else st4(a.y + m * a.ldy + n0 + c4, v);
            }
            if (SPLIT_OUT && a.ysplit && a.ysplit_fmt == 1 && m < a.M && n0 + c4 < a.N) {
                unsigned h[2], l[2];
                split4_f16(v, h, l);
                uint16_t* sp = a.ysplit + m * (int64_t)a.N + n0 + c4;
                *reinterpret_cast<uint2*>(sp) = make_uint2(h[0], h[1]);
                *reinterpret_cast<uint2*>(sp + a.ysplit_plane) = make_uint2(l[0], l[1]);
            } else if (SPLIT_OUT && a.ysplit && m < a.M && n0 + c4 < a.N) {
                const float f[4] = {v.x, v.y, v.z, v.w};
                typedef __bf16 bf16x4 __attribute__((ext_vector_type(4)));
                bf16x4 p0, p1, p2;
#pragma unroll
                for (int j = 0; j < 4; ++j) {
                    const __bf16 h = (__bf16)f[j];
                    const float r1 = f[j] - (float)h;
                    const __bf16 md = (__bf16)r1;
                    p0[j] = h; p1[j] = md; p2[j] = (__bf16)(r1 - (float)md);
                }
                uint16_t* sp = a.ysplit + m * (int64_t)a.N + n0 + c4;
                *reinterpret_cast<bf16x4*>(sp) = p0;
                if (a.ysplit_np >= 2) *reinterpret_cast<bf16x4*>(sp + a.ysplit_plane) = p1;
                if (a.ysplit_np == 3) *reinterpret_cast<bf16x4*>(sp + 2 * a.ysplit_plane) = p2;
            }
        }
        }
        __builtin_amdgcn_fence(__ATOMIC_RELEASE, "wavefront");
        __builtin_amdgcn_wave_barrier();
        __builtin_amdgcn_fence(__ATOMIC_ACQUIRE, "wavefront");
    }
}

template <int NT>
__device__ __forceinline__ void pw_red_stage(const PwArgs& a, float* sRedVec, int n0, int tid, int nthreads) {
    for (int e = tid; e < 4 * 16 * NT; e += nthreads) {
        const int which = e / (16 * NT), n = n0 + e - which * (16 * NT);
        float v = which == 0 ? 1.f : 0.f;
        if (n < a.N) {
            if (a.red_mode == 2) v = (which == 0 ? a.red_scale : which == 1 ? a.red_shift : which == 2 ? a.red_mean : a.red_rstd)[n];
            else v = (which == 0 && a.red_center) ? a.red_center[n] : 0.f;
        }
        sRedVec[e] = v;
    }
}

template <int RM, int NT>
__device__ __forceinline__ void pw_red_rowgroups(const PwArgs& a, f32x4 (&acc)[RM][NT], int64_t m_base, int n0, int l15, int q,
                                                 const float* sRedVec, float4 (&s1)[NT], float4 (&s2)[NT], int nrg = RM) {
    const float lo = a.red_act == AMS_ACT_NONE ? -__builtin_huge_valf() : 0.f, hi = a.red_act == AMS_ACT_RELU6 ? 6.f : __builtin_huge_valf();
#pragma unroll
    for (int r = 0; r < RM; ++r) {
        if (r >= nrg) break;
        int64_t m = m_base + r * 16 + l15;
        const float w = m < a.M ? 1.f : 0.f;
        const bool whole = m_base + r * 16 + 16 <= a.M;
        if (m > a.M - 1) m = a.M - 1;
        if (a.red_mode == 2) {
            float4 zv[NT];
#pragma unroll
            for (int t = 0; t < NT; ++t) {
                int n4 = n0 + 16 * t + 4 * q;
                if (n4 > a.N - 4) n4 = a.N - 4;
                zv[t] = ld4(a.red_z + m * a.ldy + n4);
            }
            if (a.red_res) {
#pragma unroll
                for (int t = 0; t < NT; ++t) {
                    int n4 = n0 + 16 * t + 4 * q;
                    if (n4 > a.N - 4) n4 = a.N - 4;
                    const float4 rv = ld4(a.red_res + m * a.red_ldr + n4);
                    acc[r][t][0] += rv.x; acc[r][t][1] += rv.y; acc[r][t][2] += rv.z; acc[r][t][3] += rv.w;
                }
            }
#pragma unroll
            for (int t = 0; t < NT; ++t) {
                const int c4 = 16 * t + 4 * q;
                const float4 sc = ld4(sRedVec + c4), sh = ld4(sRedVec + 16 * NT + c4), mu = ld4(sRedVec + 32 * NT + c4), rs = ld4(sRedVec + 48 * NT + c4);
                const float4 y = muladd4_pk(zv[t], sc, sh);
                float4 d;
                d.x = (y.x > lo && y.x < hi) ? acc[r][t][0] : 0.f; d.y = (y.y > lo && y.y < hi) ? acc[r][t][1] : 0.f;
                d.z = (y.z > lo && y.z < hi) ? acc[r][t][2] : 0.f; d.w = (y.w > lo && y.w < hi) ? acc[r][t][3] : 0.f;
                acc[r][t][0] = d.x; acc[r][t][1] = d.y; acc[r][t][2] = d.z; acc[r][t][3] = d.w;
                if (n0 + c4 < a.N) {
                    const float4 dw = whole ? d : make_float4(d.x * w, d.y * w, d.z * w, d.w * w);
                    s1[t] = add4_pk(s1[t], dw);
                    s2[t] = add4_pk(s2[t], mul4_pk(mul4_pk(dw, sub4_pk(zv[t], mu)), rs));
                }
            }
        } else {
#pragma unroll
            for (int t = 0; t < NT; ++t) {
                const int c4 = 16 * t + 4 * q;
                if (n0 + c4 >= a.N) continue;
                const float4 ctr = ld4(sRedVec + c4);
                float4 d = sub4_pk(make_float4(acc[r][t][0], acc[r][t][1], acc[r][t][2], acc[r][t][3]), ctr);
                if (!whole) d = make_float4(d.x * w, d.y * w, d.z * w, d.w * w);
                s1[t] = add4_pk(s1[t], d);
                s2[t] = add4_pk(s2[t], mul4_pk(d, d));
            }
        }
    }
}

template <int NT>
__device__ __forceinline__ void pw_red_finish(const PwArgs& a, float4 (&s1)[NT], float4 (&s2)[NT], int lane, int wave, int nwaves, float* sRed,
                                              int64_t row, int n0, int tid, int nthreads) {
    const int l15 = lane & 15, q = lane >> 4;
#pragma unroll
    for (int t = 0; t < NT; ++t) {
        float4 u = s1[t], v = s2[t];
#pragma unroll
        for (int off = 8; off > 0; off >>= 1) {
            u.x += __shfl_xor(u.x, off, 64); u.y += __shfl_xor(u.y, off, 64); u.z += __shfl_xor(u.z, off, 64); u.w += __shfl_xor(u.w, off, 64);
            v.x += __shfl_xor(v.x, off, 64); v.y += __shfl_xor(v.y, off, 64); v.z += __shfl_xor(v.z, off, 64); v.w += __shfl_xor(v.w, off, 64);
        }
        if (l15 == 0) {
            st4(sRed + (wave * 2 + 0) * 16 * NT + 16 * t + 4 * q, u);
            st4(sRed + (wave * 2 + 1) * 16 * NT + 16 * t + 4 * q, v);
        }
    }
    __syncthreads();
    float* out = a.red_part + row * 2 * (int64_t)a.N;
    for (int e = tid; e < 2 * 16 * NT; e += nthreads) {
        const int which = e / (16 * NT), c = e - which * (16 * NT);
        if (n0 + c >= a.N) continue;
        float s = 0.f;
        for (int wv = 0; wv < nwaves; ++wv) s += sRed[(wv * 2 + which) * 16 * NT + c];
        out[(int64_t)which * a.N + n0 + c] = s;
    }
}

static inline bool pw_red_ok(const PwArgs& a, int64_t rows) {
    return a.red_mode != 0 && a.red_part && (size_t)rows * 2 * (size_t)a.N <= a.red_part_floats && !a.scale && !a.shift && !a.img_bias && !a.res && a.act == AMS_ACT_NONE && a.N % 4 == 0 && a.ldy % 4 == 0 &&
           a.N >= 4;
}

static inline int pw_pick_epi(const PwArgs& a) {
    const bool vec_ok = a.N >= 4 && (a.N & 3) == 0 && (a.ldy & 3) == 0 && (!a.res || (a.ldr & 3) == 0);
    if (!vec_ok || (a.res && a.img_bias)) return EPI_GENERIC;
    return a.res ? EPI_RES : a.img_bias ? EPI_BIAS : EPI_PLAIN;
}

static inline void pw_pick_tile(int64_t M, int N, int* rm_out, int* nt_out) {
    int nt;
    if (N % 64 == 0) nt = 4;
    else if (N % 80 == 0) nt = 5;
    else if (N % 48 == 0) nt = 3;
    else if (N % 32 == 0) nt = 2;
    else nt = N <= 16 ? 1 : N <= 32 ? 2 : N <= 48 ? 3 : 4;
    const int tiles_n = cdiv(N, 16 * nt);
    *rm_out = (cdiv64(M, 128) * tiles_n >= 512) ? 2 : 1;
    *nt_out = nt;
}
// ... 88 lines not shown
```

### ams_amd/engine.py

```python
from __future__ import annotations

import ctypes as C
import os
from typing import Dict, Optional, Sequence

import numpy as np
import torch

from . import coord_masks, hip
from .spec import (BN_DECAY, BN_EPS_FROZEN, PIXEL_SCALE, Layer, StudentSpec, build_spec)
from . import weights as W

_ACT = {"none": hip.ACT_NONE, "relu": hip.ACT_RELU, "relu6": hip.ACT_RELU6}

_ENV_OPTIONS = {
    "AMS_DUAL_STREAM": hip.OPT_DUAL_STREAM, "AMS_DUAL_PARTS": hip.OPT_DUAL_PARTS, "AMS_DUAL_AUTOTUNE": hip.OPT_DUAL_AUTOTUNE,
    "AMS_BLOCK_X6": hip.OPT_BLOCK_X6, "AMS_LATE_SUB": hip.OPT_LATE_SUBBATCH, "AMS_STREAM_MIN_ROWS": hip.OPT_STREAM_MIN_ROWS,
    "AMS_OVERLAP_HEAD": hip.OPT_OVERLAP_HEAD, "AMS_FUSE_BLOCK": hip.OPT_FUSE_BLOCK, "AMS_FUSE_XDS": hip.OPT_FUSE_EXPAND_DW_STREAM,
    "AMS_OVERLAP_WGRAD": hip.OPT_OVERLAP_WGRAD, "AMS_FUSE_DGRAD_BN": hip.OPT_FUSE_DGRAD_BN, "AMS_FUSE_GEMM_RED": hip.OPT_FUSE_GEMM_RED,
    "AMS_TRAIN_RECOMPUTE": hip.OPT_TRAIN_RECOMPUTE, "AMS_NAN_GRADS": hip.OPT_NAN_GRADS, "AMS_FUSE_OPERAND_BN": hip.OPT_FUSE_OPERAND_BN,
    "AMS_WGRAD_FORK_EVERY": hip.OPT_WGRAD_FORK_EVERY, "AMS_TRAIN_FWD_F16": hip.OPT_TRAIN_FWD_F16,
}


def _role(layer: Layer) -> int:
    s = layer.scope
    if s == "MobilenetV2/Conv":
        return hip.ROLE_STEM
    if s.endswith("/expand"):
        return hip.ROLE_EXPAND
    if s.endswith("/depthwise"):
        return hip.ROLE_DEPTHWISE
    if s.endswith("/project"):
        return hip.ROLE_PROJECT
    return {"image_pooling": hip.ROLE_POOL_CONV, "aspp0": hip.ROLE_ASPP, "concat_projection": hip.ROLE_CONCAT_PROJ,
            "logits/semantic": hip.ROLE_LOGITS}[s]


def layer_table(spec: StudentSpec):
    arr = (hip.LayerDesc * len(spec.layers))()
    for i, l in enumerate(spec.layers):
        d = arr[i]
        d.role = _role(l)
        d.cin, d.cout, d.stride, d.rate = l.cin, l.cout, l.stride, l.rate
        d.act = _ACT[l.act]
        d.residual_from = l.residual_from or 0
        d.w_off = spec.by_name[l.weight_name].offset
        if l.bn_eps is not None:
            d.bn_eps = l.bn_eps
            d.gamma_off = spec.by_name[l.scope + "/BatchNorm/gamma:0"].offset
            d.beta_off = spec.by_name[l.scope + "/BatchNorm/beta:0"].offset
            d.mean_off = spec.by_name[l.scope + "/BatchNorm/moving_mean:0"].offset
            d.var_off = spec.by_name[l.scope + "/BatchNorm/moving_variance:0"].offset
        else:
            d.bn_eps = -1.0
            d.gamma_off = spec.by_name[l.scope + "/biases:0"].offset
            d.beta_off = d.mean_off = d.var_off = 0
    return arr


class StudentEngine:

    def __init__(self, class_indices: Sequence[int], height: int, width: Optional[int] = None, max_batch: int = 1,
                 trainable: bool = False, num_classes: int = 19, device: str | torch.device = "cuda:0"):
        if not torch.cuda.is_available():
            raise hip.AmsHipError("no GPU visible: the AMS student runs only on MI355X (no CPU fallback)")
        self.lib = hip.lib()
        self.device = torch.device(device)
        self.spec = build_spec(num_classes)
        self.height, self.width = int(height), int(width if width is not None else 2 * height)
        self.max_batch = int(max_batch)
        self.trainable = bool(trainable)
        self.num_classes = int(num_classes)
        self.soft_teacher = False
        self._reg_mask = self._teacher_logits_dev = None
        self._frames_b, self._frames_u8, self._frames_metric = 0, False, False
        self.class_indices = [int(c) for c in class_indices]
        self.K = len(self.class_indices)
        cfg = hip.StudentConfig()
        cfg.abi_version = hip.ABI_VERSION
        cfg.height, cfg.width, cfg.max_batch = self.height, self.width, self.max_batch
        cfg.num_classes, cfg.n_selected = num_classes, self.K
        for i, c in enumerate(self.class_indices):
            cfg.class_indices[i] = c
        cfg.n_layers = len(self.spec.layers)
        cfg.trainable = 1 if trainable else 0
        cfg.act_dtype = hip.DT_F32
        cfg.n_trainable, cfg.n_stats = self.spec.n_trainable, self.spec.n_stats
        cfg.bn_decay, cfg.bn_eps_frozen, cfg.pixel_scale = BN_DECAY, BN_EPS_FROZEN, PIXEL_SCALE
        self._cfg = cfg
        self._layers = layer_table(self.spec)
        need = C.c_size_t(0)
        hip.check(self.lib.ams_student_arena_bytes(C.byref(cfg), self._layers, C.byref(need)), "ams_student_arena_bytes")
        self.arena_bytes = int(need.value)
        with torch.cuda.device(self.device):
            self.arena = torch.zeros(self.arena_bytes, dtype=torch.uint8, device=self.device)
            handle = C.c_void_p()
            hip.check(self.lib.ams_student_create(C.byref(cfg), self._layers, C.c_void_p(self.arena.data_ptr()),
                                                  self.arena_bytes, C.byref(handle)), "ams_student_create")
        self._h = handle
        self.params = self._view(hip.REGION_PARAMS, torch.float32)
        self.stats = self._view(hip.REGION_STATS, torch.float32)
        self.frozen_params = self._view(hip.REGION_FROZEN, torch.float32)
        self.logits_lowres = self._view(hip.REGION_LOGITS, torch.float32)
        self.bn_sync = self._view(hip.REGION_BN_SYNC, torch.float64)
        if trainable:
            self.grads = self._view(hip.REGION_GRADS, torch.float32)
            self.adam_m = self._view(hip.REGION_ADAM_M, torch.float32)
            self.adam_v = self._view(hip.REGION_ADAM_V, torch.float32)
        h, w = C.c_int32(), C.c_int32()
        hip.check(self.lib.ams_student_lowres_size(self._h, C.byref(h), C.byref(w)))
        self.lowres = (h.value, w.value)
        self._out_meta = (self.K * self.K + 2) * 8
        nbytes = self._out_meta * self.max_batch + self.max_batch * self.height * self.width * 4
        self._out_dev = torch.zeros(nbytes, dtype=torch.uint8, device=self.device)
        self._out_host = torch.zeros(nbytes, dtype=torch.uint8).pin_memory()
        self._in_frames = torch.zeros(self.max_batch * self.height * self.width * 3, dtype=torch.uint8).pin_memory()
        self._in_labels = torch.zeros(self.max_batch * self.height * self.width, dtype=torch.uint8).pin_memory()
        self._in_free = {}
        self._keepalive = []
        self._delta_host = self._delta_dev = self._delta_scratch = None
        self._delta_words = torch.zeros(2, dtype=torch.int64, device=self.device)
        self._updated_since_freeze = False
        self._fallback_layers = 0
        self._select_scratch = self._encode_scratch = None
        self._select_words = torch.zeros(4, dtype=torch.int64, device=self.device)
        self.generation = 0
        for name, opt in _ENV_OPTIONS.items():
            if name in os.environ:
                hip.check(self.lib.ams_student_set_option(self._h, opt, int(os.environ[name])), "ams_student_set_option(%s)" % name)

    def _view(self, region: int, dtype: torch.dtype) -> torch.Tensor:
        off, n = C.c_size_t(), C.c_size_t()
        hip.check(self.lib.ams_student_region(self._h, region, C.byref(off), C.byref(n)), "ams_student_region")
        item = torch.empty((), dtype=dtype).element_size()
        return self.arena[off.value:off.value + n.value * item].view(dtype)

    def _stream(self) -> C.c_void_p:
        return C.c_void_p(torch.cuda.current_stream(self.device).cuda_stream)

    def close(self) -> None:
        if getattr(self, "_h", None):
            torch.cuda.synchronize(self.device)
            self.lib.ams_student_destroy(self._h)
            self._h = None

    def __del__(self):
        try:
            self.close()
        except Exception:
            pass

    def _frames_to_device(self, frames) -> tuple:
        if isinstance(frames, torch.Tensor):
            t = frames
        else:
            a = np.asarray(frames)
            if a.dtype == np.uint8 and a.ndim == 4 and tuple(a.shape[1:]) == (self.height, self.width, 3) and 0 < a.shape[0] <= self.max_batch:
                return self._staged(a, self._in_frames), hip.DT_U8, int(a.shape[0])
            a = np.ascontiguousarray(a)
            if a.dtype != np.uint8:
                a = a.astype(np.float32, copy=False)
            t = torch.from_numpy(a)
        if t.dtype not in (torch.uint8, torch.float32):
            t = t.to(torch.float32)
        assert t.dim() == 4 and tuple(t.shape[1:]) == (self.height, self.width, 3), \
            "frames must be [B,%d,%d,3], got %s" % (self.height, self.width, tuple(t.shape))
        assert 0 < t.shape[0] <= self.max_batch, "batch %d outside 1..%d" % (t.shape[0], self.max_batch)
        t = t.to(self.device, non_blocking=True).contiguous()
        return t, (hip.DT_U8 if t.dtype == torch.uint8 else hip.DT_F32), int(t.shape[0])

    def _staged(self, a: np.ndarray, block: torch.Tensor) -> torch.Tensor:
        prev = self._in_free.get(id(block))
        if prev is not None:
            prev.synchronize()
        view = block[:a.size].view(a.shape)
        np.copyto(view.numpy(), a)
        t = view.to(self.device, non_blocking=True)
        ev = torch.cuda.Event()
        ev.record(torch.cuda.current_stream(self.device))
        self._in_free[id(block)] = ev
        return t

    def _labels_to_device(self, labels, batch: int) -> torch.Tensor:
        if isinstance(labels, torch.Tensor):
            t = labels
        else:
            a = np.asarray(labels)
            if a.dtype == np.uint8 and tuple(a.shape) == (batch, self.height, self.width) and a.size <= self._in_labels.numel():
                return self._staged(a, self._in_labels)
            if a.dtype != np.uint8:
                ai = a.astype(np.float32).astype(np.int64)
                a = np.where((ai >= 0) & (ai < 255), ai, 255).astype(np.uint8)
            t = torch.from_numpy(np.ascontiguousarray(a))
        if t.dtype != torch.uint8:
            ti = t.to(torch.int64)
            t = torch.where((ti >= 0) & (ti < 255), ti, torch.full_like(ti, 255)).to(torch.uint8)
        assert tuple(t.shape) == (batch, self.height, self.width), "labels must be [B,H,W], got %s" % (tuple(t.shape),)
        return t.to(self.device, non_blocking=True).contiguous()

    def load_variables(self, variables: Dict[str, np.ndarray]) -> None:
        tr = self.params.cpu().numpy()
        st = self.stats.cpu().numpy()
        W.fill_flat(tr, [v for v in self.spec.trainable if v.name in variables], variables)
        W.fill_flat(st, [v for v in self.spec.stats if v.name in variables], variables)
        self.params.copy_(torch.from_numpy(tr))
        self.stats.copy_(torch.from_numpy(st))

    def get_variables(self) -> Dict[str, np.ndarray]:
        return W.unpack(self.spec, self.params.cpu().numpy(), self.stats.cpu().numpy())

    def set_matmul_mode(self, mode: int) -> None:
        hip.check(self.lib.ams_student_set_option(self._h, hip.OPT_MATMUL, int(mode)), "ams_student_set_option")

    def pack_masked_fp16(self, mask: Optional[torch.Tensor] = None) -> torch.Tensor:
        n = self.spec.n_trainable
        if mask is not None:
            assert mask.dtype == torch.uint8 and mask.numel() == n and mask.device == self.arena.device
        out = torch.empty(n, dtype=torch.int16, device=self.device)
        cnt = torch.zeros(1, dtype=torch.int64, device=self.device)
        scratch = torch.empty(int(self.lib.ams_pack_masked_fp16_scratch(n)), dtype=torch.int64, device=self.device)
        hip.check(self.lib.ams_pack_masked_fp16(C.c_void_p(self.params.data_ptr()), C.c_void_p(mask.data_ptr()) if mask is not None else None,
                                                n, C.c_void_p(out.data_ptr()), C.c_void_p(cnt.data_ptr()),
                                                C.c_void_p(scratch.data_ptr()), scratch.numel(), self._stream()),
                  "ams_pack_masked_fp16")
        return out[:int(cnt.item())]

    def set_fuse_operand_bn(self, on: bool) -> None:
        hip.check(self.lib.ams_student_set_option(self._h, hip.OPT_FUSE_OPERAND_BN, int(bool(on))), "ams_student_set_option")

    def set_wgrad_fork_every(self, n: int) -> None:
        hip.check(self.lib.ams_student_set_option(self._h, hip.OPT_WGRAD_FORK_EVERY, int(n)), "ams_student_set_option")

    def set_train_recompute(self, on: bool, fuse_dgrad_bn: Optional[bool] = None, fuse_gemm_red: Optional[int] = None) -> None:
        hip.check(self.lib.ams_student_set_option(self._h, hip.OPT_TRAIN_RECOMPUTE, 2 if on is True else int(on)), "ams_student_set_option")
        if fuse_gemm_red is not None:
            hip.check(self.lib.ams_student_set_option(self._h, hip.OPT_FUSE_GEMM_RED, int(fuse_gemm_red)), "ams_student_set_option")
        if fuse_dgrad_bn is not None:
            hip.check(self.lib.ams_student_set_option(self._h, hip.OPT_FUSE_DGRAD_BN, 2 if fuse_dgrad_bn is True else int(fuse_dgrad_bn)), "ams_student_set_option")

    def set_soft_teacher(self, on: bool) -> None:
        hip.check(self.lib.ams_student_set_option(self._h, hip.OPT_SOFT_TEACHER, int(bool(on))), "ams_student_set_option")
        self.soft_teacher = bool(on)

    def set_regularizer(self, on: bool, biases_only: bool = False, coef: float = 0.01) -> None:
        if not on:
            hip.check(self.lib.ams_student_set_regularizer(self._h, None, 0, 0.0), "ams_student_set_regularizer")
            self._reg_mask = None
            return
        flat = np.zeros(self.spec.n_trainable, dtype=np.uint8)
        tvars = [v for v in self.spec.trainable if not (biases_only and 'weight' in v.name)]
        for part in W.split_flat(flat, tvars):
            part[...] = 1
        n_vars = len(tvars)
        self._reg_mask = torch.from_numpy(flat).to(self.device)
        hip.check(self.lib.ams_student_set_regularizer(self._h, C.c_void_p(self._reg_mask.data_ptr()), n_vars, float(coef)),
                  "ams_student_set_regularizer")

    def teacher_logits_layout(self, channels: int, layout: Optional[str] = None) -> int:
        channels = int(channels)
        if layout is None:
            assert channels in (self.num_classes, self.K), \
                "teacher logits must be [batch, th, tw, %d] (full) or [batch, th, tw, %d] (the selected classes), got %d channels" % (self.num_classes, self.K, channels)
            layout = "full" if channels == self.num_classes else "selected"
        assert layout in hip.TLOGITS_LAYOUTS, "layout is 'full' or 'selected', got %r" % (layout,)
        want = self.num_classes if layout == "full" else self.K
        assert channels == want, "teacher logits in the %s layout must be [batch, th, tw, %d], got %d channels" % (layout, want, channels)
        return hip.TLOGITS_LAYOUTS[layout]

    def _feed_teacher_logits(self, teacher_logits, b: int, layout: Optional[str] = None):
        if teacher_logits is None:
            assert not self.soft_teacher, "soft_teacher is on: teacher_logits must be fed (teacher_labels_logits_pl)"
            return None
        t = teacher_logits if isinstance(teacher_logits, torch.Tensor) else torch.from_numpy(np.ascontiguousarray(teacher_logits, dtype=np.float32))
        assert t.dim() == 4 and t.shape[0] == b, "teacher logits must be [batch, th, tw, %d]" % self.num_classes
        code = self.teacher_logits_layout(t.shape[3], layout)
        assert t.shape[1] <= self.height and t.shape[2] <= self.width
        t = t.to(self.device, dtype=torch.float32, non_blocking=True).contiguous()
        hip.check(self.lib.ams_student_feed_teacher_logits_layout(self._h, C.c_void_p(t.data_ptr()), int(t.shape[1]), int(t.shape[2]), code),
                  "ams_student_feed_teacher_logits_layout")
        return t

    def set_nan_grads(self, on: bool) -> None:
        hip.check(self.lib.ams_student_set_option(self._h, hip.OPT_NAN_GRADS, int(bool(on))), "ams_student_set_option")

    def set_fuse_first_block(self, on: int) -> None:
        hip.check(self.lib.ams_student_set_option(self._h, hip.OPT_FUSE_FIRST_BLOCK, int(on)), "ams_student_set_option")

    def set_fuse_dw_project(self, on: bool) -> None:
        hip.check(self.lib.ams_student_set_option(self._h, hip.OPT_FUSE_DW_PROJECT, int(bool(on))), "ams_student_set_option")

    def set_block_x6(self, on: bool) -> None:
        hip.check(self.lib.ams_student_set_option(self._h, hip.OPT_BLOCK_X6, int(bool(on))), "ams_student_set_option")

    def set_dual_stream(self, mode: int, parts: Optional[int] = None, autotune: Optional[bool] = None) -> None:
        hip.check(self.lib.ams_student_set_option(self._h, hip.OPT_DUAL_STREAM, int(mode)), "ams_student_set_option")
        if parts is not None:
            hip.check(self.lib.ams_student_set_option(self._h, hip.OPT_DUAL_PARTS, int(parts)), "ams_student_set_option")
        if autotune is not None:
            hip.check(self.lib.ams_student_set_option(self._h, hip.OPT_DUAL_AUTOTUNE, int(bool(autotune))), "ams_student_set_option")

    def set_late_subbatch(self, frames: int) -> None:
        hip.check(self.lib.ams_student_set_option(self._h, hip.OPT_LATE_SUBBATCH, int(frames)), "ams_student_set_option")

    def set_fuse_block(self, on: bool) -> None:
        hip.check(self.lib.ams_student_set_option(self._h, hip.OPT_FUSE_BLOCK, int(bool(on))), "ams_student_set_option")

    def set_fuse_expand_dw(self, on: int) -> None:
        hip.check(self.lib.ams_student_set_option(self._h, hip.OPT_FUSE_EXPAND_DW, int(on)), "ams_student_set_option")

    def set_fuse_expand_dw_stream(self, on: int) -> None:
        hip.check(self.lib.ams_student_set_option(self._h, hip.OPT_FUSE_EXPAND_DW_STREAM, int(on)), "ams_student_set_option")

    def freeze(self) -> None:
        hip.check(self.lib.ams_student_freeze(self._h, self._stream()), "ams_student_freeze")
        before, self._fallback_layers = self._fallback_layers, self.f16_fallback_layers()
        if self._updated_since_freeze and (before or self._fallback_layers):
            self.generation += 1
        self._updated_since_freeze = False

    def f16_fallback_layers(self) -> int:
        n = C.c_int32()
        hip.check(self.lib.ams_student_f16_fallback_layers(self._h, C.byref(n)), "ams_student_f16_fallback_layers")
        return int(n.value)

    def apply_delta(self, payload, layout) -> int:
        if isinstance(payload, torch.Tensor):
            assert payload.dtype == torch.uint8 and payload.device == self.arena.device, "payload: a uint8 tensor on the engine's device"
            dev = payload.contiguous().view(-1)
            n = int(dev.numel())
        else:
            a = np.frombuffer(payload, dtype=np.uint8) if isinstance(payload, (bytes, bytearray, memoryview)) else \
                np.ascontiguousarray(payload, dtype=np.uint8).reshape(-1)
            n = int(a.size)
            if n > layout.max_payload_bytes:
                raise hip.AmsHipError("delta payload rejected: %d bytes, the %s layout holds at most %d; the model is unchanged"
                                      % (n, layout.kind, layout.max_payload_bytes))
            if self._delta_host is None or self._delta_host.numel() < layout.max_payload_bytes:
                self._delta_host = torch.empty(layout.max_payload_bytes, dtype=torch.uint8).pin_memory()
                self._delta_dev = torch.empty(layout.max_payload_bytes, dtype=torch.uint8, device=self.device)
            np.copyto(self._delta_host[:n].numpy(), a)
            self._delta_dev[:n].copy_(self._delta_host[:n], non_blocking=True)
            dev = self._delta_dev
        table = layout.table()
        need = int(self.lib.ams_student_apply_delta_scratch(table, len(table)))
        if self._delta_scratch is None or self._delta_scratch.numel() < need:
            self._delta_scratch = torch.empty(need, dtype=torch.int64, device=self.device)
        words = self._delta_words.data_ptr()
        hip.check(self.lib.ams_student_apply_delta(self._h, C.c_void_p(dev.data_ptr()) if n else None, n, table, len(table),
                                                   C.c_void_p(words), C.c_void_p(words + 8), C.c_void_p(self._delta_scratch.data_ptr()),
                                                   self._delta_scratch.numel(), self._stream()), "ams_student_apply_delta")
        w = self._delta_words.cpu().numpy()
        applied, status = int(w[0]), int(w[1:].view(np.int32)[0])
        if status != hip.DELTA_OK:
            why = {hip.DELTA_BAD_SIZE: "its size does not match its mask (%d mask bytes + 2 per set bit): truncated, over-long or corrupted"
                   % layout.mask_bytes, hip.DELTA_BAD_PADDING: "a padding bit after a variable's last element is set"}.get(status, "status %d" % status)
            raise hip.AmsHipError("delta payload rejected (%d bytes, %s layout): %s; the model is unchanged" % (n, layout.kind, why))
        if applied:
            self._updated_since_freeze = True
        return applied

    def snapshot_params(self) -> torch.Tensor:
        return self.params.clone()

    def select_changed(self, before: torch.Tensor, frac: float):
        n = self.spec.n_trainable
        assert before.dtype == torch.float32 and before.numel() == n and before.device == self.arena.device
        q = 100 * (1 - frac)
        k = coord_masks.percentile_rank(n, q)
        if self._select_scratch is None:
            self._select_scratch = torch.empty(int(self.lib.ams_select_changed_scratch(n)), dtype=torch.int64, device=self.device)
        words = self._select_words
        hip.check(self.lib.ams_select_changed(C.c_void_p(self.params.data_ptr()), C.c_void_p(before.data_ptr()), n, k, C.c_void_p(words.data_ptr()),
                                              C.c_void_p(self._select_scratch.data_ptr()), self._select_scratch.numel(), self._stream()),
                  "ams_select_changed")
        w = words[:2].cpu().numpy()
        a, b = w[:1].view(np.float32)
        cut = coord_masks.percentile_cut(a, b, n, q, int(w[1]))
        mask = torch.empty(n, dtype=torch.uint8, device=self.device)
        hip.check(self.lib.ams_select_apply(C.c_void_p(self.params.data_ptr()), C.c_void_p(before.data_ptr()), n, float(cut),
                                            C.c_void_p(mask.data_ptr()), C.c_void_p(words.data_ptr() + 16), self._stream()), "ams_select_apply")
        return mask, words[2:3].clone()

    def encode_delta(self, layout, mask: Optional[torch.Tensor] = None, cap: Optional[int] = None) -> torch.Tensor:
        if mask is not None:
            assert mask.dtype == torch.uint8 and mask.numel() == layout.n_elements and mask.device == self.arena.device
        table = layout.table()
        need = int(self.lib.ams_student_encode_delta_scratch(table, len(table)))
        if self._encode_scratch is None or self._encode_scratch.numel() < need:
            self._encode_scratch = torch.empty(need, dtype=torch.int64, device=self.device)
        cap = layout.max_payload_bytes if cap is None else int(cap)
        out = torch.empty(cap, dtype=torch.uint8, device=self.device)
        size = self._select_words.data_ptr() + 24
        hip.check(self.lib.ams_student_encode_delta(self._h, C.c_void_p(mask.data_ptr()) if mask is not None else None, table, len(table),
                                                    C.c_void_p(out.data_ptr()), cap, C.c_void_p(size), C.c_void_p(self._encode_scratch.data_ptr()),
                                                    self._encode_scratch.numel(), self._stream()), "ams_student_encode_delta")
        nbytes = int(self._select_words[3].item())
        if nbytes > cap:
            raise hip.AmsHipError("encode_delta: the payload has %d bytes, the buffer %d; nothing was written" % (nbytes, cap))
        return out[:nbytes]

    def predict(self, frames, mode: int = hip.MODE_FROZEN) -> torch.Tensor:
        t, dt, b = self._frames_to_device(frames)
        out = torch.empty((b, self.height, self.width), dtype=torch.int32, device=self.device)
        hip.check(self.lib.ams_student_predict(self._h, C.c_void_p(t.data_ptr()), dt, b, mode, C.c_void_p(out.data_ptr()),
                                               self._stream()), "ams_student_predict")
        return out

    def graphed_predict(self, batch: int, mode: int = hip.MODE_FROZEN) -> "GraphedPredict":
        return GraphedPredict(self, batch, mode)

    def predict_with_metric(self, frames, labels_teacher, mode: int = hip.MODE_FROZEN):
        t, dt, b = self._frames_to_device(frames)
        lab = self._labels_to_device(labels_teacher, b)
        out = torch.empty((b, self.height, self.width), dtype=torch.int32, device=self.device)
        conf = torch.empty(self.K * self.K, dtype=torch.int64, device=self.device)
        loss = torch.empty(2, dtype=torch.float64, device=self.device)
        hip.check(self.lib.ams_student_predict_with_metric(
            self._h, C.c_void_p(t.data_ptr()), dt, b, mode, C.c_void_p(lab.data_ptr()), C.c_void_p(out.data_ptr()),
            C.c_void_p(conf.data_ptr()), C.c_void_p(loss.data_ptr()), self._stream()), "ams_student_predict_with_metric")
        return out, conf.view(self.K, self.K), loss

    def predict_host(self, frames, mode: int = hip.MODE_FROZEN) -> np.ndarray:
        self.predict_frames(frames, None, mode, u8=True)
        return self.fetch_frames(labels_only=True)[0]

    def predict_with_metric_host(self, frames, labels_teacher, mode: int = hip.MODE_FROZEN):
        self.predict_frames(frames, labels_teacher, mode, u8=True)
        labels, confs, losses = self.fetch_frames()
        return labels, confs.sum(axis=0), losses.sum(axis=0)

    def predict_frames(self, frames, labels_teacher=None, mode: int = hip.MODE_FROZEN, u8: bool = False):
        t, dt, b = self._frames_to_device(frames)
        lab = self._labels_to_device(labels_teacher, b) if labels_teacher is not None else None
        kk = self.K * self.K
        base = self._out_dev.data_ptr()
        meta = self._out_meta * b
        fn = self.lib.ams_student_predict_frames_u8 if u8 else self.lib.ams_student_predict_frames
        hip.check(fn(self._h, C.c_void_p(t.data_ptr()), dt, b, mode, C.c_void_p(lab.data_ptr()) if lab is not None else None, C.c_void_p(base + meta),
                     C.c_void_p(base), C.c_void_p(base + kk * 8 * b), self._stream()), "ams_student_predict_frames")
        self._keepalive = [t, lab]
        self._frames_b = b
        self._frames_u8 = bool(u8)
        self._frames_metric = lab is not None
        conf = self._out_dev[:kk * 8 * b].view(torch.int64).view(b, self.K, self.K)
        loss = self._out_dev[kk * 8 * b:meta].view(torch.float64).view(b, 2)
        px = b * self.height * self.width
        labels = (self._out_dev[meta:meta + px].view(b, self.height, self.width) if u8 else
                  self._out_dev[meta:meta + px * 4].view(torch.int32).view(b, self.height, self.width))
        return labels, conf, loss

    def last_inputs(self):
        return self._keepalive[0], self._keepalive[1]

    def fetch_frames(self, labels_only: bool = False):
        b = self._frames_b
        kk = self.K * self.K
        meta = self._out_meta * b
        px = b * self.height * self.width
        n = meta + (px if self._frames_u8 else px * 4)
# ... 131 lines not shown
```

### ams_amd/hip.py

```python
from __future__ import annotations

import ctypes as C
import os
from pathlib import Path

_HERE = Path(__file__).resolve().parent
LIB_PATH = _HERE / "libams_hip.so"

ABI_VERSION = 6

ROLE_STEM, ROLE_EXPAND, ROLE_DEPTHWISE, ROLE_PROJECT, ROLE_POOL_CONV, ROLE_ASPP, ROLE_CONCAT_PROJ, ROLE_LOGITS = range(8)
ACT_NONE, ACT_RELU, ACT_RELU6 = 0, 1, 2
DT_F32, DT_U8, DT_I32, DT_F64 = 0, 1, 3, 4
MODE_FROZEN, MODE_LIVE = 0, 1
OPT_MATMUL = 1
RESIZE_NEAREST, RESIZE_LINEAR = 0, 1
OPT_FUSE_EXPAND_DW = 2
OPT_FUSE_DW_PROJECT = 3
OPT_FUSE_FIRST_BLOCK = 4
OPT_FUSE_EXPAND_DW_STREAM = 5
OPT_FUSE_BLOCK = 6
OPT_LATE_SUBBATCH = 7
OPT_BLOCK_X6 = 8
OPT_DUAL_STREAM = 10
OPT_TRAIN_RECOMPUTE = 11
OPT_FUSE_DGRAD_BN = 16
OPT_FUSE_GEMM_RED = 17
OPT_EMULATE_BF16_STORAGE = 15
OPT_DUAL_AUTOTUNE = 12
OPT_DUAL_PARTS = 13
OPT_NAN_GRADS = 18
OPT_TRAIN_FWD_F16 = 24
OPT_SOFT_TEACHER = 25
TLOGITS_FULL, TLOGITS_SELECTED = 0, 1
TLOGITS_LAYOUTS = {"full": TLOGITS_FULL, "selected": TLOGITS_SELECTED}
OPT_OVERLAP_WGRAD = 19
OPT_OVERLAP_HEAD = 20
OPT_STREAM_MIN_ROWS = 21
OPT_FUSE_OPERAND_BN = 22
OPT_WGRAD_FORK_EVERY = 23
MATMUL_F32, MATMUL_SPLIT_BF16, MATMUL_SPLIT_BF16_X6, MATMUL_BF16, MATMUL_SPLIT_F16 = 0, 1, 2, 3, 4
MATMUL_DEFAULT = MATMUL_SPLIT_F16
(REGION_PARAMS, REGION_STATS, REGION_GRADS, REGION_ADAM_M, REGION_ADAM_V, REGION_FROZEN, REGION_BN_SYNC,
 REGION_LOGITS) = range(8)


class LayerDesc(C.Structure):
    _fields_ = [("role", C.c_int32), ("cin", C.c_int32), ("cout", C.c_int32), ("stride", C.c_int32),
                ("rate", C.c_int32), ("act", C.c_int32), ("residual_from", C.c_int32), ("bn_eps", C.c_float),
                ("w_off", C.c_int64), ("gamma_off", C.c_int64), ("beta_off", C.c_int64), ("mean_off", C.c_int64),
                ("var_off", C.c_int64)]


class StudentConfig(C.Structure):
    _fields_ = [("abi_version", C.c_int32), ("height", C.c_int32), ("width", C.c_int32), ("max_batch", C.c_int32),
                ("num_classes", C.c_int32), ("n_selected", C.c_int32), ("class_indices", C.c_int32 * 32),
                ("n_layers", C.c_int32), ("trainable", C.c_int32), ("act_dtype", C.c_int32),
                ("n_trainable", C.c_int64), ("n_stats", C.c_int64), ("bn_decay", C.c_float),
                ("bn_eps_frozen", C.c_float), ("pixel_scale", C.c_float)]


class DeltaVar(C.Structure):
    _fields_ = [("region", C.c_int32), ("reserved", C.c_int32), ("offset", C.c_int64), ("count", C.c_int64), ("mask_offset", C.c_int64)]


class RenderOut(C.Structure):
    _fields_ = [("colour_student", C.c_void_p), ("overlay_student", C.c_void_p), ("colour_teacher", C.c_void_p), ("overlay_teacher", C.c_void_p),
                ("ignore_mask", C.c_void_p), ("cross_mask", C.c_void_p)]


RENDER_VIEWS = tuple(f[0] for f in RenderOut._fields_)
RENDER_TABLE_BYTES = 1120
CONFIDENCE_BINS = 32

DELTA_OK, DELTA_BAD_SIZE, DELTA_BAD_PADDING = 0, 1, 2
DELTA_MAX_VARS = 1024

ALLREDUCE_CB = C.CFUNCTYPE(C.c_int, C.c_void_p, C.c_size_t, C.c_size_t, C.c_int32)

_vp, _i32, _i64, _f32, _sz = C.c_void_p, C.c_int32, C.c_int64, C.c_float, C.c_size_t

SIGNATURES = {
    "ams_last_error": (C.c_char_p, []),
    "ams_abi_version": (C.c_int, []),
    "ams_device_info": (C.c_int, [C.c_char_p, _sz, C.POINTER(_i32), C.POINTER(_i64)]),
    "ams_student_arena_bytes": (C.c_int, [C.POINTER(StudentConfig), C.POINTER(LayerDesc), C.POINTER(_sz)]),
    "ams_student_create": (C.c_int, [C.POINTER(StudentConfig), C.POINTER(LayerDesc), _vp, _sz, C.POINTER(_vp)]),
    "ams_student_destroy": (None, [_vp]),
    "ams_student_region": (C.c_int, [_vp, _i32, C.POINTER(_sz), C.POINTER(_sz)]),
    "ams_student_lowres_size": (C.c_int, [_vp, C.POINTER(_i32), C.POINTER(_i32)]),
    "ams_student_layer_tensor": (C.c_int, [_vp, _i32, _i32, C.POINTER(C.c_size_t), C.POINTER(C.c_size_t)]),
    "ams_student_freeze": (C.c_int, [_vp, _vp]),
    "ams_student_predict": (C.c_int, [_vp, _vp, _i32, _i32, _i32, _vp, _vp]),
    "ams_student_predict_with_metric": (C.c_int, [_vp, _vp, _i32, _i32, _i32, _vp, _vp, _vp, _vp, _vp]),
    "ams_student_predict_frames": (C.c_int, [_vp, _vp, _i32, _i32, _i32, _vp, _vp, _vp, _vp, _vp]),
    "ams_student_predict_frames_u8": (C.c_int, [_vp, _vp, _i32, _i32, _i32, _vp, _vp, _vp, _vp, _vp]),
    "ams_student_confidence": (C.c_int, [_vp, _i32, _vp, _vp, _vp, _vp, _vp]),
    "ams_student_soft_metric": (C.c_int, [_vp, _i32, _vp, _vp, _i32, _i32, _vp, _vp, _vp, _vp]),
    "ams_cross_confusion": (C.c_int, [_vp, _vp, _i64, _vp, _vp]),
    "ams_cross_confusion_pairs": (C.c_int, [_vp, _vp, _i64, _i32, _i64, _vp, _vp, _i32, _vp, _vp]),
    "ams_student_soft_metric_layout": (C.c_int, [_vp, _i32, _vp, _vp, _i32, _i32, _vp, _vp, _vp, _vp, _i32]),
    "ams_replay_pack_logits": (C.c_int, [_vp, _i32, _i32, _i32, C.POINTER(_i32), _i32, _i32, _vp, _vp]),
    "ams_replay_gather": (C.c_int, [_vp, _i64, _vp, _i64, _i32, _i32, _i32, _vp, _vp, _i32, _i32, _i32, _vp, _vp, _vp]),
    "ams_replay_gather_f32": (C.c_int, [_vp, _i64, _i32, _i32, _i32, _i32, _vp, _vp, _i32, _vp, _vp]),
    "ams_replay_gather_logits": (C.c_int, [_vp, _i64, _i32, _i32, _i32, _i32, _vp, _vp, _i32, _i32, _i32, _vp, _vp]),
    "ams_replay_gather_logits_lowres": (C.c_int, [_vp, _i64, _i32, _i32, _i32, _i32, _i32, _i32, _vp, _vp, _i32, _i32, _i32, _vp, _vp]),
    "ams_teacher_labels_from_logits": (C.c_int, [_vp, _i64, _i32, _i32, _i32, _i32, _i32, _i32, _vp, _i64, _vp]),
    "ams_render_table_bytes": (_sz, []),
    "ams_render_views": (C.c_int, [_vp, _vp, _i32, _vp, _i32, _i32, _i32, _i32, _vp, C.POINTER(RenderOut), _vp]),
    "ams_student_train_step": (C.c_int, [_vp, _vp, _i32, _vp, _i32, _f32, _vp, _vp, _vp]),
    "ams_student_train_step_dp": (C.c_int, [_vp, _vp, _i32, _vp, _i32, _i32, _f32, _vp, _vp, ALLREDUCE_CB, _vp, _vp]),
    "ams_comm_unique_id": (C.c_int, [_vp, _sz]),
    "ams_comm_create": (C.c_int, [_vp, _sz, _i32, _i32, C.POINTER(_vp)]),
    "ams_comm_destroy": (None, [_vp]),
    "ams_comm_stats": (C.c_int, [_vp, C.POINTER(_i32), C.POINTER(_i32), C.POINTER(_i64), C.POINTER(_i64)]),
    "ams_comm_set_timing": (C.c_int, [_vp, _i32]),
    "ams_comm_timing_read": (C.c_int, [_vp, C.POINTER(C.c_double), C.POINTER(C.c_double), C.POINTER(_i64)]),
    "ams_comm_allreduce": (C.c_int, [_vp, _vp, _sz, _i32, _vp]),
    "ams_student_train_step_rccl": (C.c_int, [_vp, _vp, _i32, _vp, _i32, _i32, _f32, _vp, _vp, _vp, _vp]),
    "ams_student_set_option": (C.c_int, [_vp, _i32, _i32]),
    "ams_student_feed_teacher_logits": (C.c_int, [_vp, _vp, _i32, _i32]),
    "ams_student_feed_teacher_logits_layout": (C.c_int, [_vp, _vp, _i32, _i32, _i32]),
    "ams_student_f16_fallback_layers": (C.c_int, [_vp, C.POINTER(_i32)]),
    "ams_student_set_regularizer": (C.c_int, [_vp, _vp, _i32, _f32]),
    "ams_student_profile": (C.c_int, [_vp, _i32]),
    "ams_student_profile_read": (C.c_int, [_vp, C.c_char_p, _sz, C.POINTER(_sz)]),
    "ams_student_get_adam_step": (C.c_int, [_vp, C.POINTER(_i64)]),
    "ams_student_set_adam_step": (C.c_int, [_vp, _i64]),
    "ams_pack_masked_fp16": (C.c_int, [_vp, _vp, _i64, _vp, _vp, _vp, _sz, _vp]),
    "ams_pack_masked_fp16_scratch": (_sz, [_i64]),
    "ams_student_apply_delta": (C.c_int, [_vp, _vp, _i64, C.POINTER(DeltaVar), _i32, _vp, _vp, _vp, _sz, _vp]),
    "ams_student_apply_delta_scratch": (_sz, [C.POINTER(DeltaVar), _i32]),
    "ams_select_changed": (C.c_int, [_vp, _vp, _i64, _i64, _vp, _vp, _sz, _vp]),
    "ams_select_changed_scratch": (_sz, [_i64]),
    "ams_select_apply": (C.c_int, [_vp, _vp, _i64, _f32, _vp, _vp, _vp]),
    "ams_student_encode_delta": (C.c_int, [_vp, _vp, C.POINTER(DeltaVar), _i32, _vp, _i64, _vp, _vp, _sz, _vp]),
    "ams_student_encode_delta_scratch": (_sz, [C.POINTER(DeltaVar), _i32]),
    "ams_k_stem_conv": (C.c_int, [_vp, _i32, _i32, _i32, _i32, _vp, _i32, _vp, _vp, _i32, _f32, _vp, _vp]),
    "ams_k_depthwise3x3": (C.c_int, [_vp, _i32, _i32, _i32, _i32, _vp, _i32, _i32, _vp, _vp, _i32, _vp, _vp]),
    "ams_k_pointwise": (C.c_int, [_vp, _i64, _i32, _vp, _i32, _i32, _vp, _i64, _vp, _vp, _i32, _vp, _vp, _vp]),
    "ams_k_pointwise_split": (C.c_int, [_vp, _i64, _i32, _vp, _i32, _vp, _vp, _i32, _vp, _vp, _vp, _sz, _vp]),
    "ams_k_pointwise_split3": (C.c_int, [_vp, _i64, _i32, _vp, _i32, _vp, _vp, _i32, _vp, _vp, _vp, _sz, _vp]),
    "ams_k_pack_h2i": (C.c_int, [_vp, _i64, _i32, _vp, _vp]),
    "ams_k_pointwise_split_f16": (C.c_int, [_vp, _i64, _i32, _vp, _i32, _vp, _vp, _i32, _vp, _vp, _vp, _sz, _vp, _vp, _vp]),
    "ams_k_expand_dw_stream_f16": (C.c_int, [_vp, _i32, _i32, _i32, _i32, _vp, _vp, _vp, _i32, _vp, _i32, _vp, _vp, _vp, _vp, _sz, _i32, _i32, _vp]),
    "ams_ingest_resize_u8": (C.c_int, [_vp, _i32, _i32, _i32, _i32, _i32, _vp, _i32, _i32, _vp]),
    "ams_k_dw_project": (C.c_int, [_vp, _i32, _i32, _i32, _i32, _vp, _i32, _vp, _vp, _vp, _i32, _vp, _vp, _vp, _vp, _vp, _sz, _vp]),
    "ams_k_block_fused": (C.c_int, [_vp, _i32, _i32, _i32, _i32, _vp, _vp, _vp, _i32, _vp, _i32, _vp, _vp, _vp, _i32, _vp, _vp, _i32, _vp, _vp, _sz, _vp]),
    "ams_k_block_fused_f16": (C.c_int, [_vp, _i32, _i32, _i32, _i32, _vp, _vp, _vp, _i32, _vp, _i32, _vp, _vp, _vp, _i32, _vp, _vp, _i32, _vp, _vp, _sz, _vp]),
    "ams_k_expand_dw": (C.c_int, [_vp, _i32, _i32, _i32, _i32, _vp, _vp, _vp, _i32, _vp, _i32, _i32, _vp, _vp, _vp, _vp]),
    "ams_k_expand_dw_stream": (C.c_int, [_vp, _i32, _i32, _i32, _i32, _vp, _vp, _vp, _i32, _vp, _i32, _vp, _vp, _vp, _vp, _sz, _i32, _i32, _vp]),
    "ams_k_global_mean": (C.c_int, [_vp, _i32, _i64, _i32, _vp, _vp, _sz, _vp]),
    "ams_k_global_mean_scratch": (_sz, [_i32, _i32]),
    "ams_k_upsample_argmax": (C.c_int, [_vp, _i32, _i32, _i32, _i32, C.POINTER(_i32), _i32, _i32, _i32, _vp, _vp, _vp,
                                        _vp, _vp]),
    "ams_k_upsample_confidence": (C.c_int, [_vp, _i32, _i32, _i32, _i32, C.POINTER(_i32), _i32, _i32, _i32, _vp, _vp, _vp, _vp, _vp]),
    "ams_confidence_stats_len": (_sz, []),
    "ams_k_upsample_soft_metric": (C.c_int, [_vp, _i32, _i32, _i32, _i32, C.POINTER(_i32), _i32, _i32, _i32, _vp, _vp, _i32, _i32, _vp, _vp, _vp, _vp]),
    "ams_k_upsample_soft_metric_layout": (C.c_int, [_vp, _i32, _i32, _i32, _i32, _i32, C.POINTER(_i32), _i32, _i32, _i32, _vp, _vp, _i32, _i32, _i32, _vp, _vp, _vp, _vp]),
    "ams_soft_metric_stats_len": (_sz, [_i32]),
    "ams_k_ce_grad": (C.c_int, [_vp, _i32, _i32, _i32, _i32, C.POINTER(_i32), _i32, _i32, _i32, _vp, _vp, _vp, _vp]),
    "ams_k_ce_loss_grad": (C.c_int, [_vp, _i32, _i32, _i32, _i32, C.POINTER(_i32), _i32, _i32, _i32, _vp, _vp, _vp, _vp, _sz, _vp]),
    "ams_k_ce_loss_grad_scratch": (_sz, [_i32, _i32, _i32, _i32]),
    "ams_k_ce_loss_grad_soft": (C.c_int, [_vp, _i32, _i32, _i32, _i32, C.POINTER(_i32), _i32, _i32, _i32, _vp, _vp, _i32, _i32, _vp, _vp, _vp, _sz, _vp]),
    "ams_k_ce_loss_grad_soft_layout": (C.c_int, [_vp, _i32, _i32, _i32, _i32, _i32, C.POINTER(_i32), _i32, _i32, _i32, _vp, _vp, _i32, _i32, _i32, _vp, _vp, _vp, _sz, _vp]),
    "ams_debug_launch_table_needs_attr": (C.c_int, [_i32, C.c_uint64, _sz]),
    "ams_debug_reload_knobs": (C.c_int, []),
    "ams_debug_phase_cycles": (C.c_int, [C.c_int32, C.POINTER(C.c_uint64), C.c_int32]),
    "ams_k_pointwise_wgrad": (C.c_int, [_vp, _vp, _i64, _i32, _i32, _vp, _vp, _sz, _vp]),
    "ams_k_pointwise_wgrad_scratch": (_sz, [_i64, _i32, _i32]),
    "ams_k_pointwise_wgrad_split": (C.c_int, [_vp, _vp, _i64, _i32, _i32, _vp, _vp, _sz, _vp]),
    "ams_k_depthwise3x3_dgrad": (C.c_int, [_vp, _i32, _i32, _i32, _i32, _vp, _i32, _i32, _vp, _vp]),
    "ams_k_depthwise3x3_wgrad": (C.c_int, [_vp, _vp, _i32, _i32, _i32, _i32, _i32, _i32, _vp, _vp, _sz, _vp]),
    "ams_k_pointwise_xform": (C.c_int, [_vp, _i64, _i32, _vp, _i32, _i32, _i32, _i32, _i32, _vp, _vp, _vp, _vp, _vp, _vp, _vp, _sz, _vp]),
    "ams_k_pointwise_wgrad_xform": (C.c_int, [_vp, _vp, _i64, _i32, _i32, _i32, _i32, _i32, _vp, _vp, _i32, _vp, _vp, _vp, _vp, _vp, _vp, _sz, _vp]),
    "ams_k_pointwise_red": (C.c_int, [_vp, _i64, _i32, _vp, _i32, _i32, _i32, _i32, _vp, _vp, _vp, _vp, _vp, _vp, _i32, _vp, _vp, _vp, _sz,
                                     C.POINTER(_i32), _vp, _sz, _vp]),
    "ams_k_depthwise3x3_fwd_bn_scratch": (_sz, [_i32, _i32, _i32, _i32, _i32]),
    "ams_k_depthwise3x3_fwd_bn": (C.c_int, [_vp, _i32, _i32, _i32, _i32, _vp, _i32, _vp, _vp, _i32, _vp, _vp, _vp, _sz, C.POINTER(_i32), _vp]),
    "ams_k_depthwise3x3_dgrad_bn_scratch": (_sz, [_i32, _i32, _i32, _i32]),
    "ams_k_depthwise3x3_dgrad_bn": (C.c_int, [_vp, _i32, _i32, _i32, _i32, _vp, _i32, _vp, _vp, _vp, _i32, _vp, _vp, _vp, _vp, _sz,
                                             C.POINTER(_i32), _vp]),
    "ams_k_depthwise3x3_fwd_bn_tiles_scratch": (_sz, [_i32, _i32, _i32, _i32, _i32]),
    "ams_k_depthwise3x3_fwd_bn_tiles": (C.c_int, [_vp, _i32, _i32, _i32, _i32, _vp, _i32, _vp, _vp, _i32, _vp, _vp, _vp, _sz, C.POINTER(_i32), _vp]),
    "ams_k_depthwise3x3_dgrad_bn_apply_scratch": (_sz, [_i32, _i32, _i32, _i32, _i32]),
    "ams_k_depthwise3x3_dgrad_bn_apply": (C.c_int, [_vp, _vp, _vp, _vp, _vp, _i32, _i32, _i32, _i32, _vp, _i32, _vp, _vp, _vp, _i32, _vp, _vp, _vp, _vp, _sz,
# ... 49 lines not shown
```

### include/ams_hip.h

```cpp
#ifndef AMS_HIP_H
#define AMS_HIP_H

#include <stddef.h>
#include <stdint.h>

#ifdef __cplusplus
extern "C" {
#endif

#define AMS_ABI_VERSION 6

enum {
    AMS_OK = 0,
    AMS_E_INVALID = -1,
    AMS_E_HIP = -2,
    AMS_E_STATE = -3,
    AMS_E_NOMEM = -4
};

enum {
    AMS_ROLE_STEM = 0,
    AMS_ROLE_EXPAND = 1,
    AMS_ROLE_DEPTHWISE = 2,
    AMS_ROLE_PROJECT = 3,
    AMS_ROLE_POOL_CONV = 4,
    AMS_ROLE_ASPP = 5,
    AMS_ROLE_CONCAT_PROJ = 6,
    AMS_ROLE_LOGITS = 7
};
enum { AMS_ACT_NONE = 0, AMS_ACT_RELU = 1, AMS_ACT_RELU6 = 2 };
enum { AMS_DT_F32 = 0, AMS_DT_U8 = 1,
       AMS_DT_I32 = 3, AMS_DT_F64 = 4 };
enum {
    AMS_MODE_FROZEN = 0,
    AMS_MODE_LIVE = 1
};

typedef struct ams_layer_desc {
    int32_t role;
    int32_t cin, cout;
    int32_t stride, rate;
    int32_t act;
    int32_t residual_from;
    float bn_eps;
    int64_t w_off;
    int64_t gamma_off;
    int64_t beta_off;
    int64_t mean_off;
    int64_t var_off;
} ams_layer_desc;

typedef struct ams_student_config {
    int32_t abi_version;
    int32_t height, width;
    int32_t max_batch;
    int32_t num_classes;
    int32_t n_selected;
    int32_t class_indices[32];
    int32_t n_layers;
    int32_t trainable;
    int32_t act_dtype;
    int64_t n_trainable;
    int64_t n_stats;
    float bn_decay;
    float bn_eps_frozen;
    float pixel_scale;
} ams_student_config;

typedef struct ams_student ams_student;

enum {
    AMS_REGION_PARAMS = 0,
    AMS_REGION_STATS = 1,
    AMS_REGION_GRADS = 2,
    AMS_REGION_ADAM_M = 3,
    AMS_REGION_ADAM_V = 4,
    AMS_REGION_FROZEN = 5,
    AMS_REGION_BN_SYNC = 6,
    AMS_REGION_LOGITS = 7
};

const char* ams_last_error(void);
int ams_abi_version(void);
int ams_device_info(char* name_out, size_t name_cap, int32_t* n_cu, int64_t* hbm_bytes);

int ams_student_arena_bytes(const ams_student_config* cfg, const ams_layer_desc* layers, size_t* bytes_out);
int ams_student_create(const ams_student_config* cfg, const ams_layer_desc* layers, void* arena_dev,
                       size_t arena_bytes, ams_student** out);
void ams_student_destroy(ams_student* s);
int ams_student_region(const ams_student* s, int32_t region, size_t* offset_bytes, size_t* n_elems);
int ams_student_lowres_size(const ams_student* s, int32_t* h, int32_t* w);
int ams_student_layer_tensor(const ams_student* s, int32_t layer, int32_t which, size_t* offset_bytes, size_t* n_elems);

int ams_student_freeze(ams_student* s, void* stream);

int ams_student_predict(ams_student* s, const void* frames_dev, int32_t frames_dtype, int32_t batch,
                        int32_t mode, int32_t* labels_out_dev, void* stream);

int ams_student_predict_with_metric(ams_student* s, const void* frames_dev, int32_t frames_dtype, int32_t batch,
                                    int32_t mode, const uint8_t* teacher_dev, int32_t* labels_out_dev,
                                    int64_t* conf_mat_dev, double* loss_dev, void* stream);

int ams_student_predict_frames(ams_student* s, const void* frames_dev, int32_t frames_dtype, int32_t batch, int32_t mode,
                               const uint8_t* teacher_dev, int32_t* labels_out_dev, int64_t* conf_mats_dev, double* losses_dev, void* stream);

int ams_student_predict_frames_u8(ams_student* s, const void* frames_dev, int32_t frames_dtype, int32_t batch, int32_t mode,
                                  const uint8_t* teacher_dev, uint8_t* labels_out_dev, int64_t* conf_mats_dev, double* losses_dev, void* stream);

int ams_student_confidence(ams_student* s, int32_t batch, const uint8_t* teacher_dev, uint8_t* conf_u8, float* conf_f32, int64_t* stats,
                           void* stream);

int ams_student_soft_metric(ams_student* s, int32_t batch, const uint8_t* teacher_dev, const float* teacher_logits_dev, int32_t th, int32_t tw,
                            int64_t* stats, float* p_f32, float* ce_f32, void* stream);
int ams_student_soft_metric_layout(ams_student* s, int32_t batch, const uint8_t* teacher_dev, const float* teacher_logits_dev, int32_t th, int32_t tw,
                                   int64_t* stats, float* p_f32, float* ce_f32, void* stream, int32_t layout);

int ams_cross_confusion(const ams_student* s, const uint8_t* labels_dev, int64_t n_pixels, int64_t* conf_mat_dev,
                        void* stream);

int ams_student_train_step(ams_student* s, const void* frames_dev, int32_t frames_dtype, const uint8_t* teacher_dev,
                           int32_t batch, float lr, const uint8_t* mask_dev, double* loss_dev, void* stream);

int ams_student_f16_fallback_layers(const ams_student* s, int32_t* n_layers);

int ams_student_feed_teacher_logits(ams_student* s, const float* teacher_logits_dev, int32_t th, int32_t tw);

enum { AMS_TLOGITS_FULL = 0, AMS_TLOGITS_SELECTED = 1 };

int ams_student_feed_teacher_logits_layout(ams_student* s, const float* teacher_logits_dev, int32_t th, int32_t tw, int32_t layout);
int ams_student_set_regularizer(ams_student* s, const uint8_t* reg_mask_dev, int32_t n_vars, float coef);

typedef int (*ams_allreduce_cb)(void* user, size_t offset_bytes, size_t count, int32_t dtype);
int ams_student_train_step_dp(ams_student* s, const void* frames_dev, int32_t frames_dtype,
                              const uint8_t* teacher_dev, int32_t batch, int32_t global_batch, float lr,
                              const uint8_t* mask_dev, double* loss_dev, ams_allreduce_cb cb, void* user,
                              void* stream);

typedef struct ams_comm ams_comm;
int ams_comm_unique_id(uint8_t* id_out, size_t cap);
int ams_comm_create(const uint8_t* id, size_t id_len, int32_t rank, int32_t world, ams_comm** out);
void ams_comm_destroy(ams_comm* c);
int ams_comm_stats(const ams_comm* c, int32_t* rank, int32_t* world, int64_t* calls, int64_t* bytes);
int ams_comm_set_timing(ams_comm* c, int32_t enable);
int ams_comm_timing_read(ams_comm* c, double* total_ms, double* max_ms, int64_t* spans);
int ams_comm_allreduce(ams_comm* c, void* buf_dev, size_t count, int32_t dtype, void* stream);
int ams_student_train_step_rccl(ams_student* s, const void* frames_dev, int32_t frames_dtype, const uint8_t* teacher_dev,
                                int32_t batch, int32_t global_batch, float lr, const uint8_t* mask_dev, double* loss_dev,
                                ams_comm* comm, void* stream);

enum { AMS_OPT_SOFT_TEACHER = 25 ,
       AMS_OPT_TRAIN_FWD_F16 = 24 ,
       AMS_OPT_WGRAD_FORK_EVERY = 23 ,
       AMS_OPT_FUSE_OPERAND_BN = 22 ,
       AMS_OPT_NAN_GRADS = 18 ,
       AMS_OPT_OVERLAP_WGRAD = 19 ,
       AMS_OPT_OVERLAP_HEAD = 20 ,
       AMS_OPT_STREAM_MIN_ROWS = 21 ,
       AMS_OPT_DUAL_AUTOTUNE = 12 ,
       AMS_OPT_DUAL_PARTS = 13 ,
       AMS_OPT_EMULATE_BF16_STORAGE = 15 ,
       AMS_OPT_FUSE_DGRAD_BN = 16 ,
       AMS_OPT_FUSE_GEMM_RED = 17 ,
       AMS_OPT_TRAIN_RECOMPUTE = 11 ,
       AMS_OPT_DUAL_STREAM = 10 ,
       AMS_OPT_BLOCK_X6 = 8 ,
       AMS_OPT_LATE_SUBBATCH = 7 ,
       AMS_OPT_FUSE_BLOCK = 6 ,
       AMS_OPT_FUSE_FIRST_BLOCK = 4 ,
       AMS_OPT_FUSE_DW_PROJECT = 3 ,
       AMS_OPT_FUSE_EXPAND_DW_STREAM = 5 ,
       AMS_OPT_MATMUL = 1, AMS_OPT_FUSE_EXPAND_DW = 2  };
enum { AMS_MATMUL_F32 = 0, AMS_MATMUL_SPLIT_BF16 = 1, AMS_MATMUL_SPLIT_BF16_X6 = 2,
       AMS_MATMUL_SPLIT_F16 = 4 ,
       AMS_MATMUL_BF16 = 3  };
int ams_student_set_option(ams_student* s, int32_t option, int32_t value);

int ams_student_profile(ams_student* s, int32_t enable);
int ams_student_profile_read(ams_student* s, char* buf, size_t cap, size_t* needed);

int ams_student_get_adam_step(const ams_student* s, int64_t* t);
int ams_student_set_adam_step(ams_student* s, int64_t t);

int ams_pack_masked_fp16(const float* params_dev, const uint8_t* mask_dev, int64_t n, uint16_t* out_half_dev,
                         int64_t* n_out_dev, int64_t* scratch_dev, size_t scratch_elems, void* stream);
size_t ams_pack_masked_fp16_scratch(int64_t n);

typedef struct ams_delta_var {
    int32_t region;
    int32_t reserved;
    int64_t offset;
    int64_t count;
    int64_t mask_offset;
} ams_delta_var;

#define AMS_DELTA_MAX_VARS 1024

enum {
    AMS_DELTA_OK = 0,
    AMS_DELTA_BAD_SIZE = 1,
    AMS_DELTA_BAD_PADDING = 2
};

int ams_student_apply_delta(ams_student* s, const uint8_t* payload_dev, int64_t payload_bytes, const ams_delta_var* vars_host,
                            int32_t n_vars, int64_t* n_applied_dev, int32_t* status_dev, int64_t* scratch_dev, size_t scratch_elems,
                            void* stream);
size_t ams_student_apply_delta_scratch(const ams_delta_var* vars_host, int32_t n_vars);

typedef struct ams_select_result {
    float a;
    float b;
    int64_t nan_count;
} ams_select_result;
int ams_select_changed(const float* after_dev, const float* before_dev, int64_t n, int64_t k, ams_select_result* result_dev,
                       int64_t* scratch_dev, size_t scratch_elems, void* stream);
size_t ams_select_changed_scratch(int64_t n);

int ams_select_apply(float* params_dev, const float* before_dev, int64_t n, float cut, uint8_t* mask_dev, int64_t* n_kept_dev, void* stream);

int ams_student_encode_delta(ams_student* s, const uint8_t* mask_dev, const ams_delta_var* vars_host, int32_t n_vars, uint8_t* payload_dev,
                             int64_t payload_cap, int64_t* payload_bytes_dev, int64_t* scratch_dev, size_t scratch_elems, void* stream);
size_t ams_student_encode_delta_scratch(const ams_delta_var* vars_host, int32_t n_vars);

typedef struct ams_replay_sample {
    int32_t slot;
    int32_t th, tw;
    int32_t top, left;
    int32_t flip;
} ams_replay_sample;

int ams_replay_gather(const uint8_t* frame_slots_dev, int64_t frame_slot_stride, const uint8_t* label_slots_dev, int64_t label_slot_stride,
                      int32_t capacity, int32_t src_h, int32_t src_w, const ams_replay_sample* samples_dev, const ams_replay_sample* samples_host,
                      int32_t batch, int32_t H, int32_t W, uint8_t* frames_out_dev, uint8_t* labels_out_dev, void* stream);

int ams_replay_gather_f32(const float* slots_dev, int64_t slot_stride, int32_t capacity, int32_t th, int32_t tw, int32_t channels,
                          const ams_replay_sample* samples_dev, const ams_replay_sample* samples_host, int32_t batch, float* out_dev, void* stream);

int ams_replay_gather_logits(const float* slots_dev, int64_t slot_stride, int32_t capacity, int32_t src_h, int32_t src_w, int32_t channels,
                             const ams_replay_sample* samples_dev, const ams_replay_sample* samples_host, int32_t batch, int32_t H, int32_t W,
                             float* out_dev, void* stream);

int ams_replay_gather_logits_lowres(const float* slots_dev, int64_t slot_stride, int32_t capacity, int32_t lh, int32_t lw, int32_t channels,
                                    int32_t src_h, int32_t src_w, const ams_replay_sample* samples_dev, const ams_replay_sample* samples_host,
                                    int32_t batch, int32_t H, int32_t W, float* out_dev, void* stream);

int ams_replay_pack_logits(const float* logits_dev, int32_t th, int32_t tw, int32_t num_classes, const int32_t* class_idx_host, int32_t K,
                           int32_t layout, float* slot_dev, void* stream);

int ams_teacher_labels_from_logits(const float* logits_dev, int64_t slot_stride, int32_t n, int32_t lh, int32_t lw, int32_t num_classes, int32_t Hs,
                                   int32_t Ws, uint8_t* labels_out_dev, int64_t out_stride, void* stream);

int ams_cross_confusion_pairs(const ams_student* s, const uint8_t* label_slots_dev, int64_t label_slot_stride, int32_t capacity, int64_t n_pixels,
                              const int32_t* pairs_dev, const int32_t* pairs_host, int32_t n_pairs, int64_t* conf_mats_dev, void* stream);

#define AMS_RENDER_TABLE_BYTES 1120

typedef struct ams_render_out {
    uint8_t* colour_student;
    uint8_t* overlay_student;
    uint8_t* colour_teacher;
    uint8_t* overlay_teacher;
    uint8_t* ignore_mask;
    uint8_t* cross_mask;
} ams_render_out;

size_t ams_render_table_bytes(void);

int ams_render_views(const uint8_t* frames_dev, const void* student_dev, int32_t student_dtype, const uint8_t* teacher_dev, int32_t batch, int32_t H,
                     int32_t W, int32_t K, const uint8_t* tables_dev, const ams_render_out* out, void* stream);


int ams_k_stem_conv(const void* frames, int32_t frames_dtype, int32_t B, int32_t H, int32_t W, const float* w ,
                    int32_t cout, const float* scale, const float* shift, int32_t act, float pixel_scale,
                    float* y , void* stream);

int ams_k_depthwise3x3(const float* x, int32_t B, int32_t H, int32_t W, int32_t C, const float* w ,
                       int32_t stride, int32_t rate, const float* scale, const float* shift, int32_t act,
                       float* y, void* stream);

int ams_k_pointwise(const float* x, int64_t M, int32_t K, const float* w, int32_t N, int32_t trans_w,
                    const float* img_bias, int64_t rows_per_img, const float* scale, const float* shift,
                    int32_t act, const float* res, float* y, void* stream);

int ams_k_pointwise_split(const float* x, int64_t M, int32_t K, const float* w, int32_t N, const float* scale,
                          const float* shift, int32_t act, const float* res, float* y, uint16_t* panels,
                          size_t panel_elems, void* stream);

int ams_k_pointwise_split3(const float* x, int64_t M, int32_t K, const float* w, int32_t N, const float* scale,
                           const float* shift, int32_t act, const float* res, float* y, uint16_t* panels,
                           size_t panel_elems, void* stream);

int ams_k_expand_dw(const float* x, int32_t B, int32_t H, int32_t W, int32_t Cin, const float* w_exp, const float* scale_e,
                    const float* shift_e, int32_t Cexp, const float* w_dw, int32_t stride, int32_t rate, const float* scale_d,
                    const float* shift_d, float* y, void* stream);

int ams_k_block_fused(const float* x, int32_t B, int32_t H, int32_t W, int32_t Cin, const float* w_exp, const float* scale_e, const float* shift_e,
                      int32_t Cexp, const float* w_dw, int32_t stride, const float* scale_d, const float* shift_d, const float* w_proj, int32_t Cout,
                      const float* scale_p, const float* shift_p, int32_t residual, float* y, uint16_t* panels, size_t panel_elems, void* stream);

int ams_k_expand_dw_stream(const float* x, int32_t B, int32_t H, int32_t W, int32_t Cin, const float* w_exp, const float* scale_e,
                           const float* shift_e, int32_t Cexp, const float* w_dw, int32_t rate, const float* scale_d,
                           const float* shift_d, float* y, uint16_t* panels, size_t panel_elems, int32_t parts, int32_t presplit,
                           void* stream);

// ... 136 lines not shown
```

Before: 12210.

## Fuse ASPP, projection and logits pointwise layers into one head-chain kernel

Adds a head_chain kernel that runs the three frozen head pointwise GEMMs (ASPP 1x1, concat projection with image-pool bias, logits) back to back in one launch. Intermediates stay in LDS as split f16 hi/lo planes instead of going through global f32 activations. It also lets project layers that feed a stream/wreg block skip writing the f32 output and keep only the part planes, which saves write bandwidth. Both paths are on by default (fuse_head=3) and are guarded by shape and mode checks, with new runtime asserts against reading f32 data that was never written.

Result: faster. 12380 (median of 6 runs) (+1.4%).

```diff
diff --git a/ams_amd/csrc/api.hip b/ams_amd/csrc/api.hip
--- a/ams_amd/csrc/api.hip
+++ b/ams_amd/csrc/api.hip
@@ -439,6 +439,10 @@
     }
     if (option == AMS_OPT_OVERLAP_HEAD) {
         s->overlap_head = value != 0;
+        return AMS_OK;
+    }
+    if (option == AMS_OPT_FUSE_HEAD) {
+        s->fuse_head = value < 0 ? 0 : value & 3;
         return AMS_OK;
     }
     if (option == AMS_OPT_STREAM_MIN_ROWS) {
diff --git a/ams_amd/csrc/engine.hpp b/ams_amd/csrc/engine.hpp
--- a/ams_amd/csrc/engine.hpp
+++ b/ams_amd/csrc/engine.hpp
@@ -123,6 +123,7 @@
     hipEvent_t ev_fork_dual = nullptr;
     std::map<int, int> dual_choice;
     int overlap_head = 0;
+    int fuse_head = 3;
     int overlap_wgrad = 1;
     int wgrad_fork_every = 1;
     int train_fwd_f16 = 0;
@@ -191,7 +192,8 @@
     } while (0)
 
 static inline double pw_bytes(const PwArgs& a) {
-    return 4.0 * ((double)a.M * (a.K + a.N + (a.res ? a.N : 0)) + (double)a.Kw * a.N) + (a.ysplit ? 2.0 * a.ysplit_np * (double)a.M * a.N : 0.0);
+    return 4.0 * ((double)a.M * (a.K + (a.ysplit && a.y_skip_f32 ? 0 : a.N) + (a.res ? a.N : 0)) + (double)a.Kw * a.N) +
+           (a.ysplit ? 2.0 * a.ysplit_np * (double)a.M * a.N : 0.0);
 }
 static inline double dw_bytes(const LayerRt& l, int B) { return 4.0 * ((double)B * (l.px_in + l.px_out) * l.d.cin + 9.0 * l.d.cin); }
 
diff --git a/ams_amd/csrc/engine_forward.hip b/ams_amd/csrc/engine_forward.hip
--- a/ams_amd/csrc/engine_forward.hip
+++ b/ams_amd/csrc/engine_forward.hip
@@ -59,7 +59,7 @@
 }
 
 struct PartsFmt { int np = 0, fmt = 0; };
-struct Cursor { int i; const float* cur; int cur_i; PartsFmt parts; };
+struct Cursor { int i; const float* cur; int cur_i; PartsFmt parts; bool cur_f32 = true; };
 
 static int other(const FrozenView& v, int avoid0, int avoid1) {
     for (int k = 0; k < 4; ++k) if (k != avoid0 && k != avoid1 && k != v.reserved) return k;
@@ -82,6 +82,7 @@
     bool d_h2i = false;
     PwForm project_form = PW_F32;
     PartsFmt out;
+    bool out_parts_only = false;
 };
 
 static PwArgs layer_args(const ams_student* s, int layer, int B, const float* x, float* y, const float* res) {
@@ -172,6 +173,10 @@
     if (stream_ok(s, B, ij + 1) && v.xsplit && (size_t)a.M * a.N <= v.xsplit_plane && p.project_form != PW_F32 && pointwise_split_writes_parts(a) &&
         !(s->emulate_bf16_storage && lj.px_out == (int64_t)s->h * s->w))
         p.out = stream_parts(s, ij + 1);
+    if ((s->fuse_head & 2) && p.out.np && p.project_form == PW_F16 && !s->emulate_bf16_storage && !(s->late_subbatch > 0 && B > s->late_subbatch) && ij + 3 <= nb && role(ij + 3) == AMS_ROLE_PROJECT &&
+        !s->L[ij + 3].d.residual_from && !(s->fuse_block && block_fused_supported(s->L[ij + 1].d.cin, s->L[ij + 1].d.cout, s->L[ij + 3].d.cout,
+                                                                                  s->L[ij + 2].d.stride, s->L[ij + 2].d.rate, false)))
+        p.out_parts_only = true;
     return p;
 }
 
@@ -230,11 +235,12 @@
     const int o = other(v, c.cur_i, d_i);
     PwArgs a = layer_args(s, ij, v.B, d, v.act[o], c.cur);
     a.x_fmt = p.d_h2i ? 1 : 0;
-    if (p.out.np) { a.ysplit = v.xsplit; a.ysplit_plane = a.M * a.N; a.ysplit_np = p.out.np; a.ysplit_fmt = p.out.fmt; }
+    AMS_REQUIRE(!a.res || c.cur_f32, "engine: layer %d adds a block input that was left as part planes only", ij);
+    if (p.out.np) { a.ysplit = v.xsplit; a.ysplit_plane = a.M * a.N; a.ysplit_np = p.out.np; a.ysplit_fmt = p.out.fmt; a.y_skip_f32 = p.out_parts_only ? 1 : 0; }
     RUN(frozen_pointwise(s, ij, a, p.project_form, st));
     if (s->emulate_bf16_storage && l.px_out == (int64_t)s->h * s->w)
         RUN(launch_round_bf16(v.act[o], (int64_t)v.B * l.px_out * l.d.cout, st));
-    c.cur = v.act[o]; c.cur_i = o; c.i = ij + 1; c.parts = p.out;
+    c.cur = v.act[o]; c.cur_i = o; c.i = ij + 1; c.parts = p.out; c.cur_f32 = !p.out_parts_only;
     return AMS_OK;
 }
 
@@ -269,6 +275,8 @@
     const double bytes = 4.0 * ((double)B * (le.px_in * le.d.cin + ld.px_out * ld.d.cout) + (double)le.d.cin * le.d.cout + 9.0 * ld.d.cin);
     const uint16_t* x_parts = p.in.np ? v.xsplit : nullptr;
     const int64_t xplane = (int64_t)B * le.px_in * le.d.cin;
+    AMS_REQUIRE(c.cur_f32 || (x_parts && (p.form == BLOCK_WREG || (p.form == BLOCK_STREAM && le.d.cin > 32))),
+                "engine: block at layer %d reads an f32 input that was left as part planes only", i);
     if (p.form == BLOCK_TILED)
         RUNK(i + 1, bytes, launch_expand_dw(c.cur, B, le.Hin, le.Win, le.d.cin, P + le.d.w_off, le.fscale, le.fshift, le.d.act, le.d.cout,
                                             P + ld.d.w_off, ld.d.stride, ld.d.rate, ld.fscale, ld.fshift, ld.d.act, v.act[o], st));
@@ -319,6 +327,7 @@
 static int run_blocks(ams_student* s, const FrozenView& v, Cursor& c, int i_stop, hipStream_t st) {
     while (c.i <= s->n_backbone && c.i < i_stop) {
         const BlockPlan p = plan_block(s, v, c.i, c.parts);
+        AMS_REQUIRE(c.cur_f32 || p.form == BLOCK_STREAM || p.form == BLOCK_WREG, "engine: block at layer %d reads an f32 input that was left as part planes only", c.i);
         switch (p.form) {
             case BLOCK_WHOLE: RUN(run_block_whole(s, v, c, p, st)); break;
             case BLOCK_TILED: case BLOCK_STREAM: case BLOCK_WREG: RUN(run_block_expand_dw(s, v, c, p, st)); break;
@@ -332,6 +341,7 @@
     const float* P = s->fparams;
     const LayerRt& lp = s->L[s->iPool]; const LayerRt& la = s->L[s->iAspp]; const LayerRt& lc = s->L[s->iProj]; const LayerRt& ll = s->L[s->iLogits];
     const int B = v.B;
+    AMS_REQUIRE(c.cur_f32, "engine: the head reads an f32 input that was left as part planes only");
     const int64_t HW = (int64_t)s->h * s->w, M = (int64_t)B * HW;
     const bool fork = s->overlap_head && !s->prof.on;
     hipStream_t ps = st;
@@ -355,15 +365,27 @@
     const int o1 = other(v, c.cur_i, -1), o2 = other(v, c.cur_i, o1);
     PwArgs a = pw_args(c.cur, M, la.d.cin, la.d.cin, P + la.d.w_off, la.d.cout, v.act[o1], la.d.cout);
     a.scale = la.fscale; a.shift = la.fshift; a.act = la.d.act;
-    RUN(frozen_pointwise(s, s->iAspp, a, pointwise_form(s, s->iAspp, a, false), st));
-    if (fork) AMS_CHECK_HIP(hipStreamWaitEvent(st, s->ev_head, 0));
     PwArgs b = pw_args(v.act[o1], M, la.d.cout, la.d.cout, P + lc.d.w_off + (int64_t)lp.d.cout * lc.d.cout, lc.d.cout,
                        v.act[o2], lc.d.cout);
     b.img_bias = v.img_bias; b.rows_per_img = HW; b.scale = lc.fscale; b.shift = lc.fshift; b.act = lc.d.act;
-    RUN(frozen_pointwise(s, s->iProj, b, pointwise_form(s, s->iProj, b, false), st));
     PwArgs d = pw_args(v.act[o2], M, lc.d.cout, lc.d.cout, P + ll.d.w_off, ll.d.cout, v.logits, 32);
     d.shift = P + ll.d.gamma_off;
-    RUN(frozen_pointwise(s, s->iLogits, d, pointwise_form(s, s->iLogits, d, false), st));
+    const PwForm fa = pointwise_form(s, s->iAspp, a, false), fb = pointwise_form(s, s->iProj, b, false), fd = pointwise_form(s, s->iLogits, d, false);
+    if ((s->fuse_head & 1) && !s->emulate_bf16_storage && !(s->late_subbatch > 0) && fa == PW_F16 && fb == PW_F16 && fd == PW_F16 && la.Kp == la.d.cin && lc.Kp == la.d.cout &&
+        ll.Kp == lc.d.cout && head_chain_supported(la.d.cin, la.d.cout, la.d.cout, lc.d.cout, lc.d.cout, ll.d.cout)) {
+        if (fork) AMS_CHECK_HIP(hipStreamWaitEvent(st, s->ev_head, 0));
+        const double bytes = 4.0 * M * (la.d.cin + 32) + 4.0 * ((double)la.Kp * la.d.cout + (double)lc.Kp * lc.d.cout + (double)ll.Kp * ll.d.cout) +
+                             4.0 * (2.0 * la.d.cout + 2.0 * lc.d.cout + ll.d.cout + (double)B * lc.d.cout);
+        s->prof_flops_x6 = 2.0 * M * ((double)la.d.cin * la.d.cout + (double)la.d.cout * lc.d.cout + (double)lc.d.cout * ll.d.cout);
+        RUNK(s->iLogits, bytes, launch_head_chain(c.cur, M, la.d.cin, la.whf, (int64_t)la.d.cout * la.Kp, la.fscale, la.fshift, la.d.act,
+                                                  lc.whf, (int64_t)lc.d.cout * lc.Kp, lc.fscale, lc.fshift, lc.d.act, v.img_bias, HW,
+                                                  ll.whf, (int64_t)ll.d.cout * ll.Kp, d.shift, d.act, ll.d.cout, v.logits, st));
+        return AMS_OK;
+    }
+    RUN(frozen_pointwise(s, s->iAspp, a, fa, st));
+    if (fork) AMS_CHECK_HIP(hipStreamWaitEvent(st, s->ev_head, 0));
+    RUN(frozen_pointwise(s, s->iProj, b, fb, st));
+    RUN(frozen_pointwise(s, s->iLogits, d, fd, st));
     return AMS_OK;
 }
 
@@ -382,6 +404,7 @@
     for (int b0 = 0; b0 < v.B; b0 += s->late_subbatch) {
         const int bp = v.B - b0 < s->late_subbatch ? v.B - b0 : s->late_subbatch;
         const FrozenView lv = view_late(s, v, b0, bp, c.cur_i);
+        AMS_REQUIRE(c.cur_f32, "engine: the late section's input was left as part planes only");
         Cursor lc = {i_late, c.cur + (int64_t)b0 * late_in_frame, c.cur_i, PartsFmt()};
         RUN(run_blocks(s, lv, lc, s->n_backbone + 1, st));
         RUN(run_head(s, lv, lc, st));
diff --git a/ams_amd/csrc/k_head_chain.hip b/ams_amd/csrc/k_head_chain.hip
--- /dev/null
+++ b/ams_amd/csrc/k_head_chain.hip
@@ -0,0 +1,273 @@
+#include "pw_common.hpp"
+#include "split_bf16.hpp"
+
+namespace ams {
+
+namespace {
+
+constexpr int HC_N = 256;
+constexpr int HC_NT = HC_N / 16;
+constexpr int HC_NW = 4, HC_NTH = 64 * HC_NW;
+constexpr int HC_STAGE_HALVES = 2 * HC_N * 32;
+constexpr int HC_KA_MAX = 352;
+static inline int hc_slab_pitch(int KA) { return (KA > HC_N ? KA : HC_N) * 4 + 16; }
+constexpr int HC_VEC_FLOATS = 4 * HC_N + 32;
+static inline size_t hc_lds(int KA) { return (size_t)2 * HC_STAGE_HALVES * 2 + (size_t)HC_NW * 16 * hc_slab_pitch(KA) + (size_t)HC_VEC_FLOATS * 4; }
+
+struct HeadChainArgs {
+    const float* x; int64_t M; int KA;
+    int pitch;
+    const unsigned short *wA, *wB, *wC;
+    int64_t planeA, planeB, planeC;
+    const float *scA, *shA, *scB, *shB, *biasC;
+    const float* img_bias; int64_t rows_per_img;
+    int actA, actB, actC, NC;
+    float* y;
+};
+
+__device__ __forceinline__ f32x4 hc_mma(const u32x4& a, const u32x4& b, const f32x4& c) {
+    return __builtin_amdgcn_mfma_f32_16x16x32_f16(__builtin_bit_cast(f16x8, a), __builtin_bit_cast(f16x8, b), c, 0, 0, 0);
+}
+
+constexpr int HC_G = 4;
+__device__ __forceinline__ void hc_load_frags(const unsigned short* bw, int t0, u32x4 (&qh)[HC_G], u32x4 (&ql)[HC_G]) {
+#pragma unroll
+    for (int g = 0; g < HC_G; ++g) {
+        qh[g] = *reinterpret_cast<const u32x4*>(bw + (t0 + g) * 16 * 32);
+        ql[g] = *reinterpret_cast<const u32x4*>(bw + HC_N * 32 + (t0 + g) * 16 * 32);
+    }
+}
+__device__ __forceinline__ void hc_stage_tiles(const unsigned short* bw, const u32x4& xh, const u32x4& xl, f32x4 (&acc)[HC_NT], f32x4 (&accx)[HC_NT]) {
+    u32x4 qh[2][HC_G], ql[2][HC_G];
+    hc_load_frags(bw, 0, qh[0], ql[0]);
+#pragma unroll
+    for (int grp = 0; grp < HC_NT / HC_G; ++grp) {
+        const int cur = grp & 1, t0 = grp * HC_G;
+        if (grp + 1 < HC_NT / HC_G) hc_load_frags(bw, t0 + HC_G, qh[cur ^ 1], ql[cur ^ 1]);
+        __builtin_amdgcn_sched_barrier(0);
+#pragma unroll
+        for (int g = 0; g < HC_G; ++g) accx[t0 + g] = hc_mma(ql[cur][g], xh, accx[t0 + g]);
+#pragma unroll
+        for (int g = 0; g < HC_G; ++g) accx[t0 + g] = hc_mma(qh[cur][g], xl, accx[t0 + g]);
+#pragma unroll
+        for (int g = 0; g < HC_G; ++g) acc[t0 + g] = hc_mma(qh[cur][g], xh, acc[t0 + g]);
+        __builtin_amdgcn_sched_barrier(0);
+    }
+}
+
+template <bool BIAS>
+__device__ __forceinline__ void hc_handover(f32x4 (&acc)[HC_NT], f32x4 (&accx)[HC_NT], const float* sSc, const float* sSh, int act, const float* bias_row,
+                                            unsigned char* slab, int pitch, int l15, int q) {
+    float4 bv[BIAS ? HC_NT : 1];
+    if constexpr (BIAS) {
+#pragma unroll
+        for (int t = 0; t < HC_NT; ++t) bv[t] = ld4(bias_row + 16 * t + 4 * q);
+    }
+#pragma unroll
+    for (int t = 0; t < HC_NT; ++t) {
+        const f32x4 j = combine_f16(acc[t], accx[t]);
+        float4 v = make_float4(j[0], j[1], j[2], j[3]);
+        if constexpr (BIAS) { v.x += bv[t].x; v.y += bv[t].y; v.z += bv[t].z; v.w += bv[t].w; }
+        const int c4 = 16 * t + 4 * q;
+        const float4 bn = muladd4_pk(v, ld4(sSc + c4), ld4(sSh + c4));
+        v = make_float4(apply_act(bn.x, act), apply_act(bn.y, act), apply_act(bn.z, act), apply_act(bn.w, act));
+        unsigned h[2], l[2];
+        split4_f16(v, h, l);
+        const int g = 2 * t + (q >> 1), pos = (g & 3) * 8 + (g >> 2);
+        unsigned char* p = slab + l15 * pitch + pos * 32 + (q & 1) * 8;
+        *reinterpret_cast<uint2*>(p) = make_uint2(h[0], h[1]);
+        *reinterpret_cast<uint2*>(p + 16) = make_uint2(l[0], l[1]);
+    }
+    __builtin_amdgcn_fence(__ATOMIC_RELEASE, "wavefront");
+    __builtin_amdgcn_wave_barrier();
+    __builtin_amdgcn_fence(__ATOMIC_ACQUIRE, "wavefront");
+}
+
+__global__ __launch_bounds__(HC_NTH, 1) void head_chain_kernel(HeadChainArgs a) {
+    extern __shared__ __attribute__((aligned(16))) unsigned char smem[];
+    unsigned short* sW = reinterpret_cast<unsigned short*>(smem);
+    const int tid = threadIdx.x, wave = tid >> 6, lane = tid & 63, l15 = lane & 15, q = lane >> 4;
+    const int pitch = a.pitch;
+    unsigned char* slab = smem + (size_t)2 * HC_STAGE_HALVES * 2 + wave * (16 * pitch);
+    float* sVec = reinterpret_cast<float*>(smem + (size_t)2 * HC_STAGE_HALVES * 2 + HC_NW * (16 * pitch));
+    const int nA = a.KA / 32, nB = HC_N / 32;
+
+    const int wn = tid >> 2, wp = tid & 3;
+    const int dstAB = wn * 32 + (wp ^ (((wn >> 3) & 1) << 1)) * 8;
+    const int cpart = tid >> 7, cn = (tid & 127) >> 2;
+    const int dstC = cpart * (32 * 32) + cn * 32 + (wp ^ (((cn >> 3) & 1) << 1)) * 8;
+    const unsigned short* srcA = a.wA + (int64_t)wn * a.KA + wp * 8;
+    const unsigned short* srcB = a.wB + (int64_t)wn * HC_N + wp * 8;
+    const unsigned short* srcC = a.wC + cpart * a.planeC + (int64_t)(cn < a.NC ? cn : a.NC - 1) * HC_N + wp * 8;
+    u32x4 wreg[8];
+    auto load_w = [&](int g) {
+        if (g < nA + nB) {
+            const bool isA = g < nA;
+            const unsigned short* src = isA ? srcA + g * 32 : srcB + (g - nA) * 32;
+            const int64_t plane = isA ? a.planeA : a.planeB, col64 = isA ? (int64_t)64 * a.KA : (int64_t)64 * HC_N;
+#pragma unroll
+            for (int u = 0; u < 8; ++u) wreg[u] = *reinterpret_cast<const u32x4*>(src + (u >> 2) * plane + (u & 3) * col64);
+        } else if (g == nA + nB) {
+#pragma unroll
+            for (int u = 0; u < 8; ++u) wreg[u] = *reinterpret_cast<const u32x4*>(srcC + u * 32);
+        }
+    };
+    auto store_w = [&](int g) {
+        unsigned short* base = sW + (g & 1) * HC_STAGE_HALVES;
+        if (g < nA + nB) {
+#pragma unroll
+            for (int u = 0; u < 8; ++u) *reinterpret_cast<u32x4*>(base + (u >> 2) * (HC_N * 32) + (u & 3) * (64 * 32) + dstAB) = wreg[u];
+        } else if (g == nA + nB) {
+#pragma unroll
+            for (int u = 0; u < 8; ++u) *reinterpret_cast<u32x4*>(base + u * (2 * 32 * 32) + dstC) = wreg[u];
+        }
+    };
+
+    const int64_t m0 = (int64_t)blockIdx.x * (16 * HC_NW) + wave * 16, m_lane = m0 + l15;
+    const int64_t m_ld = m_lane < a.M ? m_lane : a.M - 1;
+    load_w(0);
+    for (int it0 = 0; it0 < nA; it0 += 5) {
+        float4 u[5][2];
+#pragma unroll
+        for (int i = 0; i < 5; ++i) {
+            const int it = it0 + i < nA ? it0 + i : nA - 1;
+            const int gi = it * 64 + lane, row = gi / (4 * nA), grp = gi - row * (4 * nA);
+            const int64_t m = m0 + row < a.M ? m0 + row : a.M - 1;
+            const float* p = a.x + m * a.KA + grp * 8;
+            u[i][0] = ld4(p); u[i][1] = ld4(p + 4);
+        }
+#pragma unroll
+        for (int i = 0; i < 5; ++i) {
+            if (it0 + i < nA) {
+                const int gi = (it0 + i) * 64 + lane, row = gi / (4 * nA), grp = gi - row * (4 * nA);
+                f16x8 h, l;
+                split8_f16(u[i][0], u[i][1], h, l);
+                unsigned char* p = slab + row * pitch + grp * 32;
+                *reinterpret_cast<u32x4*>(p) = __builtin_bit_cast(u32x4, h);
+                *reinterpret_cast<u32x4*>(p + 16) = __builtin_bit_cast(u32x4, l);
+            }
+        }
+    }
+    __builtin_amdgcn_fence(__ATOMIC_RELEASE, "wavefront");
+    __builtin_amdgcn_wave_barrier();
+    __builtin_amdgcn_fence(__ATOMIC_ACQUIRE, "wavefront");
+    for (int e = tid; e < HC_VEC_FLOATS; e += HC_NTH) {
+        const int which = e >> 8, c = e & 255;
+        float v;
+        if (which == 0) v = a.scA ? a.scA[c] : 1.f;
+        else if (which == 1) v = a.shA ? a.shA[c] : 0.f;
+        else if (which == 2) v = a.scB ? a.scB[c] : 1.f;
+        else if (which == 3) v = a.shB ? a.shB[c] : 0.f;
+        else v = (a.biasC && c < a.NC) ? a.biasC[c] : 0.f;
+        sVec[e] = v;
+    }
+    f32x4 acc[HC_NT], accx[HC_NT];
+#pragma unroll
+    for (int t = 0; t < HC_NT; ++t) { acc[t] = (f32x4){0.f, 0.f, 0.f, 0.f}; accx[t] = (f32x4){0.f, 0.f, 0.f, 0.f}; }
+    store_w(0);
+    __syncthreads();
+
+    const int frag = l15 * 32 + 8 * (q ^ ((l15 >> 3) << 1));
+    {
+        const unsigned char* xa = slab + l15 * pitch + q * 32;
+        u32x4 xh = *reinterpret_cast<const u32x4*>(xa), xl = *reinterpret_cast<const u32x4*>(xa + 16);
+        for (int s = 0; s < nA; ++s) {
+            const int sn = s + 1 < nA ? s + 1 : s;
+            load_w(s + 1);
+            const u32x4 xh1 = *reinterpret_cast<const u32x4*>(xa + sn * 128), xl1 = *reinterpret_cast<const u32x4*>(xa + sn * 128 + 16);
+            hc_stage_tiles(sW + (s & 1) * HC_STAGE_HALVES + frag, xh, xl, acc, accx);
+            xh = xh1; xl = xl1;
+            store_w(s + 1);
+            __syncthreads();
+        }
+    }
+    hc_handover<false>(acc, accx, sVec, sVec + HC_N, a.actA, nullptr, slab, pitch, l15, q);
+
+#pragma unroll
+    for (int t = 0; t < HC_NT; ++t) { acc[t] = (f32x4){0.f, 0.f, 0.f, 0.f}; accx[t] = (f32x4){0.f, 0.f, 0.f, 0.f}; }
+    const unsigned char* xfrag = slab + l15 * pitch + q * 8 * 32;
+    u32x4 xh = *reinterpret_cast<const u32x4*>(xfrag), xl = *reinterpret_cast<const u32x4*>(xfrag + 16);
+    for (int s = 0; s < nB; ++s) {
+        const int g = nA + s, sn = s + 1 < nB ? s + 1 : s;
+        load_w(g + 1);
+        const u32x4 xh1 = *reinterpret_cast<const u32x4*>(xfrag + sn * 32), xl1 = *reinterpret_cast<const u32x4*>(xfrag + sn * 32 + 16);
+        hc_stage_tiles(sW + (g & 1) * HC_STAGE_HALVES + frag, xh, xl, acc, accx);
+        xh = xh1; xl = xl1;
+        store_w(g + 1);
+        __syncthreads();
+    }
+    hc_handover<true>(acc, accx, sVec + 2 * HC_N, sVec + 3 * HC_N, a.actB, a.img_bias + (m_ld / a.rows_per_img) * HC_N, slab, pitch, l15, q);
+
+    f32x4 c0 = {0.f, 0.f, 0.f, 0.f}, c1 = c0, cx0 = c0, cx1 = c0;
+    const unsigned short* cw = sW + ((nA + nB) & 1) * HC_STAGE_HALVES + frag;
+    constexpr int CS = 2, NCG = HC_N / 32 / CS;
+    u32x4 fx[2][CS][2], fw[2][CS][4];
+    auto load_c = [&](int grp, u32x4 (&x)[CS][2], u32x4 (&w)[CS][4]) {
+#pragma unroll
+        for (int i = 0; i < CS; ++i) {
+            const int s = grp * CS + i;
+            const unsigned short* bw = cw + s * (2 * 32 * 32);
+            x[i][0] = *reinterpret_cast<const u32x4*>(xfrag + s * 32); x[i][1] = *reinterpret_cast<const u32x4*>(xfrag + s * 32 + 16);
+            w[i][0] = *reinterpret_cast<const u32x4*>(bw); w[i][1] = *reinterpret_cast<const u32x4*>(bw + 16 * 32);
+            w[i][2] = *reinterpret_cast<const u32x4*>(bw + 32 * 32); w[i][3] = *reinterpret_cast<const u32x4*>(bw + 32 * 32 + 16 * 32);
+        }
+    };
+    load_c(0, fx[0], fw[0]);
+#pragma unroll
+    for (int grp = 0; grp < NCG; ++grp) {
+        const int cur = grp & 1;
+        if (grp + 1 < NCG) load_c(grp + 1, fx[cur ^ 1], fw[cur ^ 1]);
+        __builtin_amdgcn_sched_barrier(0);
+#pragma unroll
+        for (int i = 0; i < CS; ++i) {
+            cx0 = hc_mma(fw[cur][i][2], fx[cur][i][0], cx0); cx1 = hc_mma(fw[cur][i][3], fx[cur][i][0], cx1);
+            cx0 = hc_mma(fw[cur][i][0], fx[cur][i][1], cx0); cx1 = hc_mma(fw[cur][i][1], fx[cur][i][1], cx1);
+            c0 = hc_mma(fw[cur][i][0], fx[cur][i][0], c0); c1 = hc_mma(fw[cur][i][1], fx[cur][i][0], c1);
+        }
+        __builtin_amdgcn_sched_barrier(0);
+    }
+    if (m_lane < a.M) {
+        const float4 one = make_float4(1.f, 1.f, 1.f, 1.f);
+#pragma unroll
+        for (int t = 0; t < 2; ++t) {
+            const f32x4 j = combine_f16(t == 0 ? c0 : c1, t == 0 ? cx0 : cx1);
+            const int n4 = 16 * t + 4 * q;
+            const float4 bn = muladd4_pk(make_float4(j[0], j[1], j[2], j[3]), one, ld4(sVec + 4 * HC_N + n4));
+            const float o[4] = {apply_act(bn.x, a.actC), apply_act(bn.y, a.actC), apply_act(bn.z, a.actC), apply_act(bn.w, a.actC)};
+            float* yp = a.y + m_lane * 32 + n4;
+            if (n4 + 3 < a.NC) st4(yp, make_float4(o[0], o[1], o[2], o[3]));
+            else {
+#pragma unroll
+                for (int i = 0; i < 4; ++i) if (n4 + i < a.NC) yp[i] = o[i];
+            }
+        }
+    }
+}
+
+}
+
+bool head_chain_supported(int KA, int NA, int KB, int NB, int KC, int NC) {
+    return KA >= 32 && KA % 32 == 0 && KA <= HC_KA_MAX && NA == HC_N && KB == HC_N && NB == HC_N && KC == HC_N && NC >= 1 && NC <= 32;
+}
+
+int launch_head_chain(const float* x, int64_t M, int KA, const uint16_t* wA, int64_t planeA, const float* scA, const float* shA, int actA,
+                      const uint16_t* wB, int64_t planeB, const float* scB, const float* shB, int actB, const float* img_bias, int64_t rows_per_img,
+                      const uint16_t* wC, int64_t planeC, const float* biasC, int actC, int NC, float* y, hipStream_t st) {
+    AMS_REQUIRE(M > 0 && rows_per_img > 0 && x && wA && wB && wC && img_bias && y && head_chain_supported(KA, HC_N, HC_N, HC_N, HC_N, NC),
+                "head_chain: bad problem (M %lld KA %d NC %d)", (long long)M, KA, NC);
+    HeadChainArgs a;
+    a.x = x; a.M = M; a.KA = KA; a.pitch = hc_slab_pitch(KA);
+    const size_t lds = hc_lds(KA);
+    a.wA = wA; a.wB = wB; a.wC = wC; a.planeA = planeA; a.planeB = planeB; a.planeC = planeC;
+    a.scA = scA; a.shA = shA; a.scB = scB; a.shB = shB; a.biasC = biasC;
+    a.img_bias = img_bias; a.rows_per_img = rows_per_img;
+    a.actA = actA; a.actB = actB; a.actC = actC; a.NC = NC;
+    a.y = y;
+    RUN_RC(func_allow_lds((const void*)head_chain_kernel, lds));
+    note_kernel("head_chain_kernel");
+    hipLaunchKernelGGL(head_chain_kernel, dim3((unsigned)cdiv64(M, 16 * HC_NW)), dim3(HC_NTH), lds, st, a);
+    AMS_CHECK_LAUNCH();
+    return AMS_OK;
+}
+
+}
diff --git a/ams_amd/csrc/kernels.hpp b/ams_amd/csrc/kernels.hpp
--- a/ams_amd/csrc/kernels.hpp
+++ b/ams_amd/csrc/kernels.hpp
@@ -63,6 +63,7 @@
     int64_t ysplit_plane;
     int ysplit_np;
     int ysplit_fmt;
+    int y_skip_f32;
     int x_fmt;
     int red_mode;
     const float* red_center;
@@ -95,6 +96,10 @@
 int launch_pointwise_split_f16(const PwArgs& a, const uint16_t* whi, int64_t plane, int Kp, hipStream_t st);
 int launch_pack_h2i(const float* x, int64_t M, int C, float* out, hipStream_t st);
 bool pointwise_split_writes_parts(const PwArgs& a);
+bool head_chain_supported(int KA, int NA, int KB, int NB, int KC, int NC);
+int launch_head_chain(const float* x, int64_t M, int KA, const uint16_t* wA, int64_t planeA, const float* scA, const float* shA, int actA,
+                      const uint16_t* wB, int64_t planeB, const float* scB, const float* shB, int actB, const float* img_bias, int64_t rows_per_img,
+                      const uint16_t* wC, int64_t planeC, const float* biasC, int actC, int NC, float* y, hipStream_t st);
 
 struct WgArgs {
     const float* x;  int ldx;  int K;
diff --git a/ams_amd/csrc/pw_common.hpp b/ams_amd/csrc/pw_common.hpp
--- a/ams_amd/csrc/pw_common.hpp
+++ b/ams_amd/csrc/pw_common.hpp
@@ -140,7 +140,7 @@
             float4 v = ld4(sOut + row * OP + c4);
             if (EPI == EPI_RES) { v.x += rv[uu].x; v.y += rv[uu].y; v.z += rv[uu].z; v.w += rv[uu].w; }
             if (m < a.M && n0 + c4 < a.N) {
-                if (SPLIT_OUT && a.ysplit) __builtin_nontemporal_store((f32x4){v.x, v.y, v.z, v.w}, reinterpret_cast<f32x4*>(a.y + m * a.ldy + n0 + c4));
+                if (SPLIT_OUT && a.ysplit) { if (!a.y_skip_f32) __builtin_nontemporal_store((f32x4){v.x, v.y, v.z, v.w}, reinterpret_cast<f32x4*>(a.y + m * a.ldy + n0 + c4)); }
                 else st4(a.y + m * a.ldy + n0 + c4, v);
             }
             if (SPLIT_OUT && a.ysplit && a.ysplit_fmt == 1 && m < a.M && n0 + c4 < a.N) {
diff --git a/ams_amd/engine.py b/ams_amd/engine.py
--- a/ams_amd/engine.py
+++ b/ams_amd/engine.py
@@ -20,6 +20,7 @@
     "AMS_OVERLAP_WGRAD": hip.OPT_OVERLAP_WGRAD, "AMS_FUSE_DGRAD_BN": hip.OPT_FUSE_DGRAD_BN, "AMS_FUSE_GEMM_RED": hip.OPT_FUSE_GEMM_RED,
     "AMS_TRAIN_RECOMPUTE": hip.OPT_TRAIN_RECOMPUTE, "AMS_NAN_GRADS": hip.OPT_NAN_GRADS, "AMS_FUSE_OPERAND_BN": hip.OPT_FUSE_OPERAND_BN,
     "AMS_WGRAD_FORK_EVERY": hip.OPT_WGRAD_FORK_EVERY, "AMS_TRAIN_FWD_F16": hip.OPT_TRAIN_FWD_F16,
+    "AMS_FUSE_HEAD": hip.OPT_FUSE_HEAD,
 }
 
 
@@ -306,6 +307,9 @@
     def set_fuse_block(self, on: bool) -> None:
         hip.check(self.lib.ams_student_set_option(self._h, hip.OPT_FUSE_BLOCK, int(bool(on))), "ams_student_set_option")
 
+    def set_fuse_head(self, on) -> None:
+        hip.check(self.lib.ams_student_set_option(self._h, hip.OPT_FUSE_HEAD, 3 if on is True else int(on)), "ams_student_set_option")
+
     def set_fuse_expand_dw(self, on: int) -> None:
         hip.check(self.lib.ams_student_set_option(self._h, hip.OPT_FUSE_EXPAND_DW, int(on)), "ams_student_set_option")
 
diff --git a/ams_amd/hip.py b/ams_amd/hip.py
--- a/ams_amd/hip.py
+++ b/ams_amd/hip.py
@@ -32,6 +32,7 @@
 OPT_NAN_GRADS = 18
 OPT_TRAIN_FWD_F16 = 24
 OPT_SOFT_TEACHER = 25
+OPT_FUSE_HEAD = 26
 TLOGITS_FULL, TLOGITS_SELECTED = 0, 1
 TLOGITS_LAYOUTS = {"full": TLOGITS_FULL, "selected": TLOGITS_SELECTED}
 OPT_OVERLAP_WGRAD = 19
diff --git a/include/ams_hip.h b/include/ams_hip.h
--- a/include/ams_hip.h
+++ b/include/ams_hip.h
@@ -148,7 +148,8 @@
                                 int32_t batch, int32_t global_batch, float lr, const uint8_t* mask_dev, double* loss_dev,
                                 ams_comm* comm, void* stream);
 
-enum { AMS_OPT_SOFT_TEACHER = 25 ,
+enum { AMS_OPT_FUSE_HEAD = 26 ,
+       AMS_OPT_SOFT_TEACHER = 25 ,
        AMS_OPT_TRAIN_FWD_F16 = 24 ,
        AMS_OPT_WGRAD_FORK_EVERY = 23 ,
        AMS_OPT_FUSE_OPERAND_BN = 22 ,
```
